# piljoong-jeong/nerf_meets_mlx

Hardware: AMD Instinct MI355X
Metric: train+render rays/sec on Lego 800x800 (synthetic), coarse+fine 64+128 (higher is better)
Workload: dtype split16 (fp16x2 render / bf16x2 train MFMA operands ~ 22 / 16 significand bits; fp32 accumulate)

## Files before the change

### include/nerf_hip.h

```cpp
#ifndef NERF_HIP_H
#define NERF_HIP_H

#include <stddef.h>
#include <stdint.h>

#ifdef __cplusplus
extern "C" {
#endif

#define NERF_ABI_VERSION 3

#define NERF_OK 0
#define NERF_E_NULL (-1)
#define NERF_E_SHAPE (-2)
#define NERF_E_UNSUPPORTED (-3)
#define NERF_E_HIP (-4)
#define NERF_E_RCCL (-5)

int nerf_abi_version(void);
const char* nerf_last_error(void);

#define NERF_RAY_STRIDE 11

int nerf_pixel_permutation(int64_t* out_idx, int64_t n, int64_t domain, uint64_t seed, uint64_t offset,
                           void* stream);

int nerf_ray_gen(const int64_t* pixel_idx, int64_t n, int H, int W, const double* K_host, const float* c2w_host,
                 float near, float far, float* rays, int64_t* coords, void* stream);

int nerf_sample_batch(int64_t n, int H, int W, uint64_t seed, uint64_t offset, const double* K_host, const float* c2w_host,
                      float near, float far, const float* image, float* rays, float* target, int64_t* pixel_idx,
                      void* stream);

int nerf_sample_batch_rgba(int64_t n, int H, int W, uint64_t seed, uint64_t offset, const double* K_host, const float* c2w_host,
                           float near, float far, const float* image, float* rays, float* target, int64_t* pixel_idx,
                           void* stream);

int nerf_gather_rows(const float* src, int64_t n_src, const int64_t* idx, int64_t n, int channels, float* out,
                     void* stream);

int nerf_ndc_rays(float* rays, int64_t n, int H, int W, float focal, float near, void* stream);

int nerf_sample_coarse(const float* rays, int64_t B, int n, int lindisp, float perturb, const float* t_rand,
                       float* z, void* stream);

int nerf_add_noise_z(const float* z_in, const float* t_rand, int64_t B, int n, float strength, float* z_out,
                     void* stream);

int nerf_importance_sample(const float* z, const float* weights, const float* u, int64_t B, int n, int N, float eps,
                           float* z_new, float* z_merged, float* cdf, int64_t* inds, void* stream);

int nerf_encode_freq(const float* x, int64_t M, int D, int n_freqs, int freq_mode, float* out, void* stream);

int nerf_encode_sinusoidal(const float* x, int64_t M, int D, int n_freqs, const float* freqs_host,
                           int include_input, float* out, void* stream);

int nerf_sh_encode(const float* dirs, int64_t M, int degree, float* out, void* stream);

int nerf_hashgrid_forward(const float* x, int64_t M, const float* tables, int L, int log2_T, int F,
                          const int* resolutions_host, float* out, void* stream);
int nerf_hashgrid_backward(const float* x, int64_t M, const float* d_out, int L, int log2_T, int F,
                           const int* resolutions_host, float* d_tables, void* stream);

int nerf_ngp_encode(const float* rays, const float* z, int64_t B, int n, const float* tables, int L, int log2_T,
                    int F, const int* resolutions_host, int sh_degree, float pos_scale, float pos_offset, float* x_out,
                    float* pts_out, void* stream);
int nerf_hashgrid_backward_rays(const float* rays, const float* z, int64_t B, int n, const float* d_out, int L,
                                int log2_T, int F, const int* resolutions_host, float pos_scale, float pos_offset,
                                float* d_tables, void* stream);

int nerf_hashgrid_backward_ex(const float* x, int64_t M, const float* d_out, int L, int log2_T, int F,
                              const int* resolutions_host, int level_lo, int level_hi, int fixed_point, void* d_tables,
                              void* stream);
int nerf_hashgrid_backward_rays_ex(const float* rays, const float* z, int64_t B, int n, const float* d_out, int L,
                                   int log2_T, int F, const int* resolutions_host, float pos_scale, float pos_offset,
                                   int level_lo, int level_hi, int fixed_point, void* d_tables, void* stream);

int nerf_hashgrid_forward_lw(const float* x, int64_t M, const float* tables, int L, int log2_T, int F,
                             const int* resolutions_host, const float* level_weights_host, float* out, void* stream);
int nerf_ngp_encode_lw(const float* rays, const float* z, int64_t B, int n, const float* tables, int L, int log2_T,
                       int F, const int* resolutions_host, const float* level_weights_host, int sh_degree,
                       float pos_scale, float pos_offset, float* x_out, float* pts_out, void* stream);
int nerf_hashgrid_backward_ex_lw(const float* x, int64_t M, const float* d_out, int L, int log2_T, int F,
                                 const int* resolutions_host, const float* level_weights_host, int level_lo,
                                 int level_hi, int fixed_point, void* d_tables, void* stream);
int nerf_hashgrid_backward_rays_ex_lw(const float* rays, const float* z, int64_t B, int n, const float* d_out, int L,
                                      int log2_T, int F, const int* resolutions_host, const float* level_weights_host,
                                      float pos_scale, float pos_offset, int level_lo, int level_hi, int fixed_point,
                                      void* d_tables, void* stream);

int nerf_composite_forward(const float* raw, const float* z, const float* rays, int64_t B, int n,
                           float raw_noise_std, const float* noise, int white_bkgd, float* rgb, float* disp,
                           float* acc, float* weights, float* depth, void* stream);

int nerf_composite_backward(const float* raw, const float* z, const float* rays, int64_t B, int n,
                            float raw_noise_std, const float* noise, int white_bkgd, const float* d_rgb,
                            const float* d_acc, const float* d_depth, float* d_raw, void* stream);

int nerf_mse_loss_grad(const float* pred, const float* target, int64_t count, float grad_scale, float* loss_out,
                       float* d_pred, void* stream);

int nerf_composite_mse_backward(const float* raw, const float* z, const float* rays, int64_t B, int n, int white_bkgd,
                                const float* target, float grad_scale, float* loss_out, float* rgb, float* d_raw,
                                void* stream);

int nerf_ssim_sums(const float* pred, const float* gt, int N, int C, int H, int W, const float* window_host,
                   int w_size, float c1, float c2, double* sums, void* stream);

typedef struct nerf_mlp_arch {
  int n_layers;
  int width;
  int in_pos;
  int in_dir;
  int skip_layer;
  int use_viewdirs;
  int out_ch;
  int precision;
} nerf_mlp_arch;

int64_t nerf_mlp_param_count(const nerf_mlp_arch* arch);
int64_t nerf_mlp_packed_bytes(const nerf_mlp_arch* arch);
int nerf_mlp_pack(const nerf_mlp_arch* arch, const float* params, void* packed, void* stream);

int64_t nerf_mlp_acts_bytes(const nerf_mlp_arch* arch, int64_t M);
int64_t nerf_mlp_dz_bytes(const nerf_mlp_arch* arch, int64_t M);

int nerf_mlp_forward(const nerf_mlp_arch* arch, const void* packed, const float* x, int64_t M, float* out,
                     void* stream);
int nerf_mlp_forward_train(const nerf_mlp_arch* arch, const void* packed, const float* x, int64_t M, float* out,
                           void* acts, void* stream);

int nerf_query_fused(const nerf_mlp_arch* arch, const void* packed, const float* rays, const float* z, int64_t B,
                     int n, int freq_mode, float* raw, void* acts, void* stream);

int nerf_mlp_backward(const nerf_mlp_arch* arch, const void* packed, const void* acts, const float* d_raw,
                      int64_t M, void* dz, float* grads, void* stream);
int nerf_mlp_backward_inputs(const nerf_mlp_arch* arch, const void* packed, const void* acts, const float* d_raw,
                             int64_t M, void* dz, float* grads, float* d_x, void* stream);

int nerf_mlp_debug_width(const nerf_mlp_arch* arch, int kind, int layer);
int nerf_mlp_debug_read(const nerf_mlp_arch* arch, const void* store, int kind, int layer, int64_t M, float* out,
                        void* stream);

int nerf_ngp_query_fused(const nerf_mlp_arch* arch, const void* packed, const float* rays, const float* z, int64_t B,
                         int n, const float* tables, int L, int log2_T, int F, const int* resolutions_host,
                         int sh_degree, float pos_scale, float pos_offset, float* raw, void* acts, void* stream);
int nerf_ngp_query_fused_h(const nerf_mlp_arch* arch, const void* packed, const float* rays, const float* z, int64_t B,
                           int n, const float* tables, const void* tables_half, int L, int log2_T, int F,
                           const int* resolutions_host, int sh_degree, float pos_scale, float pos_offset, float* raw,
                           void* acts, void* stream);
int nerf_ngp_query_fused_lw(const nerf_mlp_arch* arch, const void* packed, const float* rays, const float* z, int64_t B,
                            int n, const float* tables, const void* tables_half, int L, int log2_T, int F,
                            const int* resolutions_host, const float* level_weights_host, int sh_degree, float pos_scale,
                            float pos_offset, float* raw, void* acts, void* stream);


int nerf_occ_points(int log2_res, int64_t cell0, int64_t count, uint64_t seed, uint64_t update, float pos_scale,
                    float pos_offset, float* rays_out, float* z_out, void* stream);
int nerf_occ_merge(float* density, const float* raw, int64_t count, float decay, void* stream);
int64_t nerf_occ_finalize_workspace_bytes(int log2_res);
int nerf_occ_finalize(const float* density, int log2_res, float thr_cap, void* workspace, float* thr_out, uint32_t* bits,
                      void* stream);
int64_t nerf_occ_cull_workspace_bytes(int64_t B, int n);
int nerf_occ_cull(const float* rays, const float* z, int64_t B, int n, const uint32_t* bits, int log2_res, float pos_scale,
                  float pos_offset, void* workspace, int64_t* idx_out, int64_t* count_out, float* rays_out, float* z_out,
                  float* raw_fill, void* stream);
int nerf_scatter_rows(const float* src, const int64_t* idx, int64_t n, int channels, float* dst, int64_t n_dst, void* stream);

#define NERF_MARCH_MAX_STEPS 1024
int64_t nerf_occ_march_workspace_bytes(int64_t B);
int nerf_occ_march_count(const float* rays, int64_t B, const float* jitter, float jitter_const, const uint32_t* bits, int log2_res,
                         float pos_scale, float pos_offset, float step_world, int march_steps, void* workspace, int64_t* offsets,
                         void* stream);
int nerf_occ_march_write(const float* rays, int64_t B, const float* jitter, float jitter_const, const uint32_t* bits, int log2_res,
                         float pos_scale, float pos_offset, float step_world, int march_steps, void* workspace, int64_t* offsets,
                         float* rows_out, float* z_out, void* stream);
#define NERF_OCC_RELU 0
#define NERF_OCC_EXP 1
int nerf_occ_merge_ex(float* density, const float* raw, int64_t count, float decay, int activation, void* stream);

int nerf_composite_packed_forward(const float* raw, const float* z, const int64_t* offsets, int64_t B, int64_t K, float step_world,
                                  int white_bkgd, float* rgb, float* acc, float* depth, void* stream);
int nerf_composite_packed_mse_backward(const float* raw, const int64_t* offsets, int64_t B, int64_t K, float step_world,
                                       int white_bkgd, const float* target, float grad_scale, float* loss_out, float* rgb,
                                       float* d_raw, void* stream);

int nerf_composite_packed_distortion(const float* raw, const float* z, const int64_t* offsets, const float* rays, int64_t B,
                                     int64_t K, float step_world, int march_steps, int white_bkgd, float* rgb, float* acc,
                                     float* depth, float* dist, void* stream);
int nerf_composite_packed_mse_dist_backward(const float* raw, const float* z, const int64_t* offsets, const float* rays, int64_t B,
                                            int64_t K, float step_world, int march_steps, int white_bkgd, const float* target,
                                            float grad_scale, float dist_weight, float* loss_out, float* dist_out, float* rgb,
                                            float* d_raw, void* stream);

int nerf_composite_packed_forward_bg(const float* raw, const float* z, const int64_t* offsets, int64_t B, int64_t K, float step_world,
                                     const float* bg, int bg_stride, float* rgb, float* acc, float* depth, void* stream);
int nerf_composite_packed_distortion_bg(const float* raw, const float* z, const int64_t* offsets, const float* rays, int64_t B,
                                        int64_t K, float step_world, int march_steps, const float* bg, int bg_stride, float* rgb,
                                        float* acc, float* depth, float* dist, void* stream);
int nerf_composite_packed_mse_backward_bg(const float* raw, const int64_t* offsets, int64_t B, int64_t K, float step_world,
                                          const float* target_rgba, const float* bg, float grad_scale, float* loss_out, float* rgb,
                                          float* d_raw, void* stream);
int nerf_composite_packed_mse_dist_backward_bg(const float* raw, const float* z, const int64_t* offsets, const float* rays, int64_t B,
                                               int64_t K, float step_world, int march_steps, const float* target_rgba,
                                               const float* bg, float grad_scale, float dist_weight, float* loss_out,
                                               float* dist_out, float* rgb, float* d_raw, void* stream);

#define NERF_ERT_TERMINATED 1
int64_t nerf_ert_march_workspace_bytes(int64_t B);
int nerf_ert_init(int64_t B, int32_t* istate, float* fstate, int32_t* live, void* stream);
int nerf_ert_march_count(const float* rays, int64_t B, const float* jitter, float jitter_const, const uint32_t* bits, int log2_res,
                         float pos_scale, float pos_offset, float step_world, int march_steps, const int32_t* live, int64_t A,
                         const int32_t* istate, int max_new, void* workspace, int64_t* totals, void* stream);
int nerf_ert_march_write(const float* rays, int64_t B, const float* jitter, float jitter_const, const uint32_t* bits, int log2_res,
                         float pos_scale, float pos_offset, float step_world, int march_steps, const int32_t* live, int64_t A,
                         int32_t* istate, int max_new, void* workspace, int64_t* offsets, int32_t* live_out, float* rows_out,
                         float* z_out, void* stream);
int nerf_ert_fold(const float* raw, const float* z, const int64_t* offsets, const int32_t* live, int64_t A, int64_t B, int64_t K,
                  float step_world, float min_transmittance, int32_t* istate, float* fstate, void* stream);
int nerf_ert_finish(const int32_t* istate, const float* fstate, int64_t B, int white_bkgd, float* rgb, float* acc, float* depth,
                    int32_t* samples, void* stream);
int nerf_ert_finish_bg(const int32_t* istate, const float* fstate, int64_t B, const float* bg, int bg_stride, float* rgb, float* acc,
                       float* depth, int32_t* samples, void* stream);

#define NERF_MESH_MAX_RES 512
int64_t nerf_mesh_workspace_bytes(int res);
int nerf_mesh_points(int res, const float* lo_host, const float* hi_host, int64_t p0, int64_t count, float* rays_out, float* z_out,
                     void* stream);
int nerf_mesh_count(const float* vol, int res, float iso, void* workspace, int64_t* totals, void* stream);
int nerf_mesh_write_vertices(const float* vol, int res, float iso, const float* lo_host, const float* hi_host, void* workspace,
                             int64_t V, float* verts, float* normals, float* color_rows, void* stream);
int nerf_mesh_write_faces(const float* vol, int res, float iso, void* workspace, int64_t F, int32_t* faces, void* stream);

int64_t nerf_ccl_workspace_bytes(int res);
int nerf_ccl_label(const float* vol, int res, float iso, void* workspace, int32_t* labels, void* stream);
int nerf_ccl_sizes(const int32_t* labels, int res, int32_t* sizes, int64_t* stats, void* stream);
int nerf_ccl_filter(const float* vol, const int32_t* labels, const int32_t* sizes, const int64_t* stats, int res, float iso,
                    int64_t min_voxels, int largest_only, float* out, void* stream);

#define NERF_MORPH_MAX_RADIUS 16
int64_t nerf_morph_workspace_bytes(int res);
int nerf_morph_erode(const float* vol, int res, float iso, int radius, void* workspace, float* core, int64_t* stats2, void* stream);
int nerf_morph_reconstruct(const float* vol, const float* kept, int res, float iso, int radius, void* workspace, float* out,
                           int64_t* stats2, void* stream);

#define NERF_TSDF_MAX_VIEWS 16
typedef struct nerf_tsdf_view {
  float c2w[12];
  float fx, fy, cx, cy;
} nerf_tsdf_view;
int nerf_tsdf_reset(float* D, float* Wt, uint8_t* flags, int res, void* stream);
int nerf_tsdf_integrate(float* D, float* Wt, uint8_t* flags, int res, const float* lo_host, const float* hi_host,
                        const nerf_tsdf_view* views_host, int n, int H, int W, const float* depth, const float* acc, float trunc,
                        float acc_min, float far, int carve, void* stream);
int nerf_tsdf_volume(const float* D, const float* Wt, const uint8_t* flags, int res, int min_views, float* vol_out, void* stream);

int64_t nerf_render_workspace_bytes(int64_t B, int n, int N);
int nerf_render_rays_fused(const nerf_mlp_arch* arch, const void* packed_coarse, const void* packed_fine,
                           const float* rays, int64_t B, int n, int N, const float* u, int freq_mode, int white_bkgd,
                           void* workspace, float* rgb, float* disp, float* acc, float* rgb_coarse, float* disp_coarse,
                           float* acc_coarse, float* z_vals, float* weights, void* stream);

#define NERF_COMM_ID_BYTES 128
int nerf_comm_unique_id(char* id_out_host);
int nerf_comm_init(void** comm_out, int nranks, int rank, const char* id_host);
int nerf_allreduce_grads(void* comm, float* grads, int64_t count, void* stream);
int nerf_comm_destroy(void* comm);

#define NERF_OPTION_UNKNOWN (-2147483647 - 1)
int nerf_set_option(const char* key, int value);
int nerf_get_option(const char* key);

int nerf_adam_step(float* params, const float* grads, float* m, float* v, int64_t count, float lr, float beta1,
                   float beta2, float eps, int bias_correction, int step, float grad_scale, void* stream);
int nerf_adam_step_ex(float* params, void* grads, float* m, float* v, int64_t count, float lr, float beta1, float beta2,
                      float eps, int bias_correction, int step, float grad_scale, int grads_fixed_point, int zero_grads,
                      void* stream);
int nerf_adam_step_shadow(float* params, void* grads, float* m, float* v, int64_t count, float lr, float beta1, float beta2,
                          float eps, int bias_correction, int step, float grad_scale, int grads_fixed_point, int zero_grads,
                          void* params_half, void* stream);

#ifdef __cplusplus
}
#endif
#endif
```

### nerf_meets_mlx_amd/_native.py

```python
import ctypes as C
import os

import torch

_HERE = os.path.dirname(os.path.abspath(__file__))
LIB_PATH = os.environ.get("NERF_HIP_LIB", os.path.join(_HERE, "libnerf_hip.so"))

_P, _I64, _I, _F, _U64 = C.c_void_p, C.c_int64, C.c_int, C.c_float, C.c_uint64
SIGNATURES = {
    "nerf_abi_version": (_I, []),
    "nerf_last_error": (C.c_char_p, []),
    "nerf_pixel_permutation": (_I, [_P, _I64, _I64, _U64, _U64, _P]),
    "nerf_ray_gen": (_I, [_P, _I64, _I, _I, C.POINTER(C.c_double), C.POINTER(C.c_float), _F, _F, _P, _P, _P]),
    "nerf_sample_batch": (_I, [_I64, _I, _I, _U64, _U64, C.POINTER(C.c_double), C.POINTER(C.c_float), _F, _F, _P, _P, _P, _P, _P]),
    "nerf_sample_batch_rgba": (_I, [_I64, _I, _I, _U64, _U64, C.POINTER(C.c_double), C.POINTER(C.c_float), _F, _F, _P, _P, _P, _P, _P]),
    "nerf_gather_rows": (_I, [_P, _I64, _P, _I64, _I, _P, _P]),
    "nerf_ndc_rays": (_I, [_P, _I64, _I, _I, _F, _F, _P]),
    "nerf_sample_coarse": (_I, [_P, _I64, _I, _I, _F, _P, _P, _P]),
    "nerf_add_noise_z": (_I, [_P, _P, _I64, _I, _F, _P, _P]),
    "nerf_importance_sample": (_I, [_P, _P, _P, _I64, _I, _I, _F, _P, _P, _P, _P, _P]),
    "nerf_encode_freq": (_I, [_P, _I64, _I, _I, _I, _P, _P]),
    "nerf_encode_sinusoidal": (_I, [_P, _I64, _I, _I, C.POINTER(C.c_float), _I, _P, _P]),
    "nerf_sh_encode": (_I, [_P, _I64, _I, _P, _P]),
    "nerf_hashgrid_forward": (_I, [_P, _I64, _P, _I, _I, _I, C.POINTER(C.c_int), _P, _P]),
    "nerf_hashgrid_backward": (_I, [_P, _I64, _P, _I, _I, _I, C.POINTER(C.c_int), _P, _P]),
    "nerf_ngp_encode": (_I, [_P, _P, _I64, _I, _P, _I, _I, _I, C.POINTER(C.c_int), _I, C.c_float, C.c_float, _P, _P, _P]),
    "nerf_ngp_query_fused": (_I, [_P, _P, _P, _P, _I64, _I, _P, _I, _I, _I, C.POINTER(C.c_int), _I, C.c_float, C.c_float, _P, _P, _P]),
    "nerf_ngp_query_fused_h": (_I, [_P, _P, _P, _P, _I64, _I, _P, _P, _I, _I, _I, C.POINTER(C.c_int), _I, C.c_float, C.c_float, _P, _P, _P]),
    "nerf_hashgrid_backward_rays": (_I, [_P, _P, _I64, _I, _P, _I, _I, _I, C.POINTER(C.c_int), C.c_float, C.c_float, _P, _P]),
    "nerf_hashgrid_backward_ex": (_I, [_P, _I64, _P, _I, _I, _I, C.POINTER(C.c_int), _I, _I, _I, _P, _P]),
    "nerf_hashgrid_backward_rays_ex": (_I, [_P, _P, _I64, _I, _P, _I, _I, _I, C.POINTER(C.c_int), C.c_float, C.c_float, _I, _I, _I, _P, _P]),
    "nerf_hashgrid_forward_lw": (_I, [_P, _I64, _P, _I, _I, _I, C.POINTER(C.c_int), C.POINTER(C.c_float), _P, _P]),
    "nerf_ngp_encode_lw": (_I, [_P, _P, _I64, _I, _P, _I, _I, _I, C.POINTER(C.c_int), C.POINTER(C.c_float), _I, C.c_float, C.c_float, _P, _P, _P]),
    "nerf_ngp_query_fused_lw": (_I, [_P, _P, _P, _P, _I64, _I, _P, _P, _I, _I, _I, C.POINTER(C.c_int), C.POINTER(C.c_float), _I, C.c_float, C.c_float, _P, _P, _P]),
    "nerf_hashgrid_backward_ex_lw": (_I, [_P, _I64, _P, _I, _I, _I, C.POINTER(C.c_int), C.POINTER(C.c_float), _I, _I, _I, _P, _P]),
    "nerf_hashgrid_backward_rays_ex_lw": (_I, [_P, _P, _I64, _I, _P, _I, _I, _I, C.POINTER(C.c_int), C.POINTER(C.c_float), C.c_float, C.c_float, _I, _I, _I, _P, _P]),
    "nerf_composite_forward": (_I, [_P, _P, _P, _I64, _I, _F, _P, _I, _P, _P, _P, _P, _P, _P]),
    "nerf_composite_backward": (_I, [_P, _P, _P, _I64, _I, _F, _P, _I, _P, _P, _P, _P, _P]),
    "nerf_mse_loss_grad": (_I, [_P, _P, _I64, _F, _P, _P, _P]),
    "nerf_composite_mse_backward": (_I, [_P, _P, _P, _I64, _I, _I, _P, _F, _P, _P, _P, _P]),
    "nerf_ssim_sums": (_I, [_P, _P, _I, _I, _I, _I, C.POINTER(C.c_float), _I, _F, _F, _P, _P]),
    "nerf_mlp_param_count": (_I64, [_P]),
    "nerf_mlp_packed_bytes": (_I64, [_P]),
    "nerf_mlp_pack": (_I, [_P, _P, _P, _P]),
    "nerf_mlp_acts_bytes": (_I64, [_P, _I64]),
    "nerf_mlp_dz_bytes": (_I64, [_P, _I64]),
    "nerf_mlp_forward": (_I, [_P, _P, _P, _I64, _P, _P]),
    "nerf_mlp_forward_train": (_I, [_P, _P, _P, _I64, _P, _P, _P]),
    "nerf_query_fused": (_I, [_P, _P, _P, _P, _I64, _I, _I, _P, _P, _P]),
    "nerf_mlp_backward": (_I, [_P, _P, _P, _P, _I64, _P, _P, _P]),
    "nerf_mlp_backward_inputs": (_I, [_P, _P, _P, _P, _I64, _P, _P, _P, _P]),
    "nerf_mlp_debug_width": (_I, [_P, _I, _I]),
    "nerf_mlp_debug_read": (_I, [_P, _P, _I, _I, _I64, _P, _P]),
    "nerf_render_workspace_bytes": (_I64, [_I64, _I, _I]),
    "nerf_render_rays_fused": (_I, [_P, _P, _P, _P, _I64, _I, _I, _P, _I, _I, _P, _P, _P, _P, _P, _P, _P, _P, _P, _P]),
    "nerf_comm_unique_id": (_I, [C.c_char_p]),
    "nerf_comm_init": (_I, [C.POINTER(C.c_void_p), _I, _I, C.c_char_p]),
    "nerf_allreduce_grads": (_I, [_P, _P, _I64, _P]),
    "nerf_comm_destroy": (_I, [_P]),
    "nerf_set_option": (_I, [C.c_char_p, _I]),
    "nerf_get_option": (_I, [C.c_char_p]),
    "nerf_adam_step": (_I, [_P, _P, _P, _P, _I64, _F, _F, _F, _F, _I, _I, _F, _P]),
    "nerf_adam_step_ex": (_I, [_P, _P, _P, _P, _I64, _F, _F, _F, _F, _I, _I, _F, _I, _I, _P]),
    "nerf_adam_step_shadow": (_I, [_P, _P, _P, _P, _I64, _F, _F, _F, _F, _I, _I, _F, _I, _I, _P, _P]),
    "nerf_occ_points": (_I, [_I, _I64, _I64, _U64, _U64, _F, _F, _P, _P, _P]),
    "nerf_occ_merge": (_I, [_P, _P, _I64, _F, _P]),
    "nerf_occ_finalize_workspace_bytes": (_I64, [_I]),
    "nerf_occ_finalize": (_I, [_P, _I, _F, _P, _P, _P, _P]),
    "nerf_occ_cull_workspace_bytes": (_I64, [_I64, _I]),
    "nerf_occ_cull": (_I, [_P, _P, _I64, _I, _P, _I, _F, _F, _P, _P, _P, _P, _P, _P, _P]),
    "nerf_scatter_rows": (_I, [_P, _P, _I64, _I, _P, _I64, _P]),
    "nerf_occ_merge_ex": (_I, [_P, _P, _I64, _F, _I, _P]),
    "nerf_occ_march_workspace_bytes": (_I64, [_I64]),
    "nerf_occ_march_count": (_I, [_P, _I64, _P, _F, _P, _I, _F, _F, _F, _I, _P, _P, _P]),
    "nerf_occ_march_write": (_I, [_P, _I64, _P, _F, _P, _I, _F, _F, _F, _I, _P, _P, _P, _P, _P]),
    "nerf_composite_packed_forward": (_I, [_P, _P, _P, _I64, _I64, _F, _I, _P, _P, _P, _P]),
    "nerf_composite_packed_mse_backward": (_I, [_P, _P, _I64, _I64, _F, _I, _P, _F, _P, _P, _P, _P]),
    "nerf_composite_packed_distortion": (_I, [_P, _P, _P, _P, _I64, _I64, _F, _I, _I, _P, _P, _P, _P, _P]),
    "nerf_composite_packed_mse_dist_backward": (_I, [_P, _P, _P, _P, _I64, _I64, _F, _I, _I, _P, _F, _F, _P, _P, _P, _P, _P]),
    "nerf_composite_packed_forward_bg": (_I, [_P, _P, _P, _I64, _I64, _F, _P, _I, _P, _P, _P, _P]),
    "nerf_composite_packed_distortion_bg": (_I, [_P, _P, _P, _P, _I64, _I64, _F, _I, _P, _I, _P, _P, _P, _P, _P]),
    "nerf_composite_packed_mse_backward_bg": (_I, [_P, _P, _I64, _I64, _F, _P, _P, _F, _P, _P, _P, _P]),
    "nerf_composite_packed_mse_dist_backward_bg": (_I, [_P, _P, _P, _P, _I64, _I64, _F, _I, _P, _P, _F, _F, _P, _P, _P, _P, _P]),
    "nerf_ert_march_workspace_bytes": (_I64, [_I64]),
    "nerf_ert_init": (_I, [_I64, _P, _P, _P, _P]),
    "nerf_ert_march_count": (_I, [_P, _I64, _P, _F, _P, _I, _F, _F, _F, _I, _P, _I64, _P, _I, _P, _P, _P]),
    "nerf_ert_march_write": (_I, [_P, _I64, _P, _F, _P, _I, _F, _F, _F, _I, _P, _I64, _P, _I, _P, _P, _P, _P, _P, _P]),
    "nerf_ert_fold": (_I, [_P, _P, _P, _P, _I64, _I64, _I64, _F, _F, _P, _P, _P]),
    "nerf_ert_finish": (_I, [_P, _P, _I64, _I, _P, _P, _P, _P, _P]),
    "nerf_ert_finish_bg": (_I, [_P, _P, _I64, _P, _I, _P, _P, _P, _P, _P]),
    "nerf_mesh_workspace_bytes": (_I64, [_I]),
    "nerf_mesh_points": (_I, [_I, C.POINTER(C.c_float), C.POINTER(C.c_float), _I64, _I64, _P, _P, _P]),
    "nerf_mesh_count": (_I, [_P, _I, _F, _P, _P, _P]),
    "nerf_mesh_write_vertices": (_I, [_P, _I, _F, C.POINTER(C.c_float), C.POINTER(C.c_float), _P, _I64, _P, _P, _P, _P]),
    "nerf_mesh_write_faces": (_I, [_P, _I, _F, _P, _I64, _P, _P]),
    "nerf_ccl_workspace_bytes": (_I64, [_I]),
    "nerf_ccl_label": (_I, [_P, _I, _F, _P, _P, _P]),
    "nerf_ccl_sizes": (_I, [_P, _I, _P, _P, _P]),
    "nerf_ccl_filter": (_I, [_P, _P, _P, _P, _I, _F, _I64, _I, _P, _P]),
    "nerf_morph_workspace_bytes": (_I64, [_I]),
    "nerf_morph_erode": (_I, [_P, _I, _F, _I, _P, _P, _P, _P]),
    "nerf_morph_reconstruct": (_I, [_P, _P, _I, _F, _I, _P, _P, _P, _P]),
    "nerf_tsdf_reset": (_I, [_P, _P, _P, _I, _P]),
    "nerf_tsdf_integrate": (_I, [_P, _P, _P, _I, C.POINTER(C.c_float), C.POINTER(C.c_float), C.POINTER(C.c_float), _I, _I, _I, _P, _P,
                                _F, _F, _F, _I, _P]),
    "nerf_tsdf_volume": (_I, [_P, _P, _P, _I, _I, _P, _P]),
}


class MlpArch(C.Structure):
    _fields_ = [("n_layers", _I), ("width", _I), ("in_pos", _I), ("in_dir", _I), ("skip_layer", _I),
                ("use_viewdirs", _I), ("out_ch", _I), ("precision", _I)]


class NerfHipError(RuntimeError):
    pass


_lib = None


def lib():
    global _lib
    if _lib is None:
        if not os.path.exists(LIB_PATH):
            raise NerfHipError(
                f"{LIB_PATH} not found: build it with `python -c 'import __graft_entry__ as g; g.build()'` "
                "(hipcc --offload-arch=gfx950).  There is no CPU fallback.")
        L = C.CDLL(LIB_PATH)
        for name, (res, args) in SIGNATURES.items():
            fn = getattr(L, name)
            fn.restype, fn.argtypes = res, args
        _lib = L
    return _lib


def check(rc: int):
    if rc != 0:
        msg = lib().nerf_last_error().decode(errors="replace")
        if rc in (-1, -2, -3):
            raise ValueError(f"libnerf_hip error {rc}: {msg}")
        raise NerfHipError(f"libnerf_hip error {rc}: {msg}")


def ptr(t):
    if t is None:
        return None
    if not t.is_cuda:
        raise ValueError("libnerf_hip kernels need tensors on the ROCm device (there is no CPU path)")
    if not t.is_contiguous():
        raise ValueError("libnerf_hip kernels need contiguous tensors")
    return C.c_void_p(t.data_ptr())


def stream():
    return C.c_void_p(torch.cuda.current_stream().cuda_stream)


def f32(t, device=None):
    if not torch.is_tensor(t):
        t = torch.as_tensor(t)
    if device is not None:
        t = t.to(device)
    return t.to(torch.float32).contiguous()
```

### nerf_meets_mlx_amd/csrc/dw_split.h

```cpp
#pragma once
#include <stdint.h>

namespace nerf {

constexpr int DW_SPLIT_MAX_JOBS = 16;
struct DwCost { int nf, kf; };

inline int dw_split(const DwCost* jobs, int nj, int bias, int target_wgs, int64_t max_splits, int* splits) {
  int64_t units[DW_SPLIT_MAX_JOBS], total_units = 0;
  for (int j = 0; j < nj; ++j) {
    units[j] = jobs[j].nf + jobs[j].kf + bias;
    total_units += units[j];
  }
  int nw = 0;
  double frac[DW_SPLIT_MAX_JOBS];
  for (int j = 0; j < DW_SPLIT_MAX_JOBS; ++j) splits[j] = 0;
  for (int j = 0; j < nj; ++j) {
    const double share = (double)units[j] * target_wgs / (double)total_units;
    int64_t sp = (int64_t)share;
    frac[j] = share - (double)sp;
    if (sp < 1) { sp = 1; frac[j] = 0.0; }
    if (sp > max_splits) { sp = max_splits; frac[j] = 0.0; }
    splits[j] = (int)sp;
    nw += (int)sp;
  }
  while (nw < target_wgs) {
    int best = -1;
    for (int j = 0; j < nj; ++j)
      if (splits[j] < max_splits && (best < 0 || frac[j] > frac[best])) best = j;
    if (best < 0 || frac[best] <= 0.0) break;
    splits[best] += 1; frac[best] = 0.0; nw += 1;
  }
  while (nw > target_wgs) {
    int big = 0;
    for (int j = 1; j < nj; ++j) if (splits[j] > splits[big]) big = j;
    if (splits[big] <= 1) break;
    splits[big] -= 1; nw -= 1;
  }
  return nw;
}

}
```

### nerf_meets_mlx_amd/csrc/mlp.hip

```cpp
#include "common.h"
#include "mlp_ring.h"
#include "mlp_layout.h"
#include "mlp_frag.h"
#include "mlp_arch2.h"
#include "hash_common.h"
#include "mlp_params.h"
#include "mlp_model.h"
#include "dw_split.h"
#include <limits.h>
#include <string.h>


namespace nerf {

extern int g_hash_combine_max_res;




constexpr int PACK_THREADS = (L::F_TOTAL + L::B_PADDED) * 64 + L::BI_TOTAL;
__device__ __forceinline__ void pack_part(int tid, const float* __restrict__ p, bf16x8* __restrict__ wf,
                                          bf16x8* __restrict__ wb, float* __restrict__ bias) {
  const int nf = L::F_TOTAL * 64, nb = L::B_PADDED * 64;
  if (tid < nf + nb) {
// ... 781 lines not shown
  const int wv = __builtin_amdgcn_readfirstlane(threadIdx.x >> 6);
  const int64_t ntiles = (a.M + 31) >> 5;
  const int64_t nsuper = (ntiles + NW - 1) / NW;
  RingW<(L::B_TOTAL + CHUNK - 1) / CHUNK, L::B_TOTAL, 4, NW, CHUNK> ws;
  ws.wsrc = reinterpret_cast<const char*>(a.wb);
  ws.lane16 = 16 * lane;
  ws.lds0 = __builtin_amdgcn_readfirstlane(lds_addr_of(ring_smem));
  ws.wv = wv;
  ws.start(lane);
  PassQueue pq;
  pq.init(a.queue, ws.lds0 + decltype(ws)::BIAS_OFF);
  for (int64_t sp = blockIdx.x; sp < nsuper;) {
    int ln = lane;
    asm volatile("" : "+v"(ln));
    ws.new_pass();
    bwd_tiles<1>(a, ws, sp * NW + wv, ntiles, ln, &pq);
    sp = pq.next(sp);
  }
  ws.drain();
  pq.leave();
}


constexpr int DW_FRAG_STRIDE = 1152;
constexpr int DW_STAGE_BYTES = 32 * DW_FRAG_STRIDE;
constexpr int DW_STAGES = 4;
constexpr int DW_LDS_BYTES = DW_STAGES * DW_STAGE_BYTES + 1024;

__device__ __forceinline__ bf16x8 tr_frag(const char* lds_frag, int u, int hq, int i16) {
  const int q = i16 >> 2, p = i16 & 3;
  const char* base = lds_frag + 16 * (p & 1) + 8 * (p >> 1) + 32 * (16 * u + 8 * hq + q);
  const s16x4 lo = __builtin_amdgcn_ds_read_tr16_b64_v4i16((__attribute__((address_space(3))) s16x4*)(base));
  const s16x4 hi = __builtin_amdgcn_ds_read_tr16_b64_v4i16((__attribute__((address_space(3))) s16x4*)(base + 128));
  union { struct { s16x4 a, b; } s; bf16x8 v; } cvt;
  cvt.s.a = lo; cvt.s.b = hi;
  return cvt.v;
}

#ifndef NERF_DW_WAVES
#define NERF_DW_WAVES 16
#endif
constexpr int DW_WAVES = NERF_DW_WAVES;
constexpr int DW_NPW = 32 / DW_WAVES;
__global__ void __launch_bounds__(64 * DW_WAVES) mlp_dw_kernel(DwArgs a) {
  char* smem = ring_smem;
  int bj = blockIdx.x, job_id = 0;
  while (bj >= a.splits[job_id]) { bj -= a.splits[job_id]; ++job_id; }
  const DwJob jb = a.jobs[job_id];
  const int tile_lo = (int)((int64_t)a.ntiles * bj / a.splits[job_id]);
  const int tile_hi = (int)((int64_t)a.ntiles * (bj + 1) / a.splits[job_id]);
  const int tid = threadIdx.x, lane = tid & 63;
  const int wv = __builtin_amdgcn_readfirstlane(tid >> 6);
  const int n_tiles = (jb.nf + 1) >> 1, k_tiles = (jb.kf + 1) >> 1;
  const bool col_major = DW_WAVES == 16 && k_tiles <= 2;
  const int wr = col_major ? (wv & 3) : (wv >> 2), wc = col_major ? (wv >> 2) : (wv & 3);
  const int nf_pad = n_tiles * 2;
  const int nfk = jb.nf + jb.kf;
  const bool active = (wr * DW_NPW < n_tiles) && (wc * 2 < k_tiles);
  f32x16 acc[DW_NPW][2];
#pragma unroll
  for (int i = 0; i < DW_NPW; ++i)
#pragma unroll
    for (int k = 0; k < 2; ++k)
#pragma unroll
      for (int e = 0; e < 16; ++e) acc[i][k][e] = 0.0f;
  float bsum[DW_NPW];
#pragma unroll
  for (int i = 0; i < DW_NPW; ++i) bsum[i] = 0.0f;
  const int g16 = lane >> 4, i16 = lane & 15, hq = g16 >> 1, fsel = g16 & 1;
  const bf16x8* dzp = reinterpret_cast<const bf16x8*>(a.dz) + lane;
  const bf16x8* acp = reinterpret_cast<const bf16x8*>(a.acts) + lane;
  const unsigned lds0 = __builtin_amdgcn_readfirstlane(lds_addr_of(smem));
  const unsigned sink = lds0 + DW_STAGES * DW_STAGE_BYTES;

  if (jb.nf & 1) {
    for (int c = tid; c < DW_STAGES * 64; c += 64 * DW_WAVES) {
      bf16x8 zv;
#pragma unroll
      for (int j = 0; j < 8; ++j) zv[j] = (__bf16)0.0f;
      *reinterpret_cast<bf16x8*>(smem + (c >> 6) * DW_STAGE_BYTES + jb.nf * DW_FRAG_STRIDE + (c & 63) * 16) = zv;
    }
  }
  auto issue = [&](int tile, int stage) {
    const unsigned st = lds0 + __builtin_amdgcn_readfirstlane(stage) * DW_STAGE_BYTES;
#pragma unroll
    for (int k = 0; k < DW_NPW; ++k) {
      const int i = wv + DW_WAVES * k;
      if (i < jb.nf) dma_frag_nt(dzp + (int64_t)tile * a.zstride + (jb.dz_slot + i) * 64, st + i * DW_FRAG_STRIDE);
      else if (i < nfk) dma_frag_nt(acp + (int64_t)tile * a.astride + (jb.act_slot + (i - jb.nf)) * 64,
                                 st + (nf_pad + i - jb.nf) * DW_FRAG_STRIDE);
      else dma_frag(dzp + (int64_t)tile * a.zstride + jb.dz_slot * 64, sink);
    }
  };
  __syncthreads();
#pragma unroll
  for (int s_ = 0; s_ < DW_STAGES - 1; ++s_)
    if (tile_lo + s_ < tile_hi) issue(tile_lo + s_, s_);

  for (int tile = tile_lo; tile < tile_hi; ++tile) {
    const int rem = tile_hi - 1 - tile;
    if (DW_NPW == 4) {
      if (rem >= 2) asm volatile("s_waitcnt vmcnt(8) lgkmcnt(0)" ::: "memory");
      else if (rem == 1) asm volatile("s_waitcnt vmcnt(4) lgkmcnt(0)" ::: "memory");
      else asm volatile("s_waitcnt vmcnt(0) lgkmcnt(0)" ::: "memory");
    } else {
      if (rem >= 2) asm volatile("s_waitcnt vmcnt(4) lgkmcnt(0)" ::: "memory");
      else if (rem == 1) asm volatile("s_waitcnt vmcnt(2) lgkmcnt(0)" ::: "memory");
      else asm volatile("s_waitcnt vmcnt(0) lgkmcnt(0)" ::: "memory");
    }
    __builtin_amdgcn_s_barrier();
    if (tile + DW_STAGES - 1 < tile_hi) issue(tile + DW_STAGES - 1, (tile - tile_lo + DW_STAGES - 1) % DW_STAGES);
    const char* st = smem + ((tile - tile_lo) % DW_STAGES) * DW_STAGE_BYTES;
#if NERF_ABLATE == 4
    if (false) {
#else
    if (active) {
#endif
#pragma unroll
      for (int u = 0; u < 2; ++u) {
        bf16x8 bfr[2];
#pragma unroll
        for (int k = 0; k < 2; ++k) {
          const int kt = wc * 2 + k;
          const int f = nf_pad + (kt < k_tiles ? 2 * kt : 0) + fsel;
          bfr[k] = tr_frag(st + f * DW_FRAG_STRIDE, u, hq, i16);
        }
#pragma unroll
        for (int i = 0; i < DW_NPW; ++i) {
          const int nt = wr * DW_NPW + i;
          const int f = (nt < n_tiles ? 2 * nt : 0) + fsel;
          const bf16x8 afr = tr_frag(st + f * DW_FRAG_STRIDE, u, hq, i16);
#if NERF_ABLATE != 5
          if (wc == 0) {
            typedef __bf16 bf16x2_t __attribute__((ext_vector_type(2)));
            const bf16x2_t ones = {(__bf16)1.0f, (__bf16)1.0f};
#pragma unroll
            for (int j = 0; j < 8; j += 2) {
              const bf16x2_t pr = {afr[j], afr[j + 1]};
              bsum[i] = __builtin_amdgcn_fdot2_f32_bf16(pr, ones, bsum[i], false);
            }
          }
#endif
#pragma unroll
          for (int k = 0; k < 2; ++k) acc[i][k] = __builtin_amdgcn_mfma_f32_32x32x16_bf16(afr, bfr[k], acc[i][k], 0, 0, 0);
        }
      }
    }
  }
  if (!active) return;
#if NERF_ABLATE == 6
  if (a.ntiles > 0) return;
#endif
  const int rr = lane & 31, hh = lane >> 5;
  float* slot = a.partial + (size_t)blockIdx.x * DW_SLOT_FLOATS;
#pragma unroll
  for (int i = 0; i < DW_NPW; ++i) {
    const int nt = wr * DW_NPW + i;
    if (nt >= n_tiles) continue;
#pragma unroll
    for (int k = 0; k < 2; ++k) {
      const int kt = wc * 2 + k;
      if (kt >= k_tiles) continue;
      float* tile = slot + (8 * nt + kt) * 1024;
#pragma unroll
      for (int e = 0; e < 16; ++e) tile[((e & 3) + 8 * (e >> 2) + 4 * hh) * 32 + rr] = acc[i][k][e];
    }
    if (wc == 0 && jb.b_off >= 0) {
      const float tot = bsum[i] + __shfl_xor(bsum[i], 32, 64);
      if (hh == 0) slot[64 * 1024 + 32 * nt + rr] = tot;
    }
  }
}

__global__ void __launch_bounds__(256) mlp_dw_reduce_kernel(DwArgs a) {
  const int j = blockIdx.y;
  const DwJob jb = a.jobs[j];
  int first = 0;
  for (int q = 0; q < j; ++q) first += a.splits[q];
  const int S = a.splits[j];
  const int nw = jb.n_valid * jb.k_valid, nb = jb.b_off >= 0 ? jb.n_valid : 0;
  const float* base = a.partial + (size_t)first * DW_SLOT_FLOATS;
  for (int t = blockIdx.x * 256 + threadIdx.x; t < nw + nb; t += gridDim.x * 256) {
    const float* src;
    float* dst;
    if (t < nw) {
      const int n = t / jb.k_valid, k = t - n * jb.k_valid;
      src = base + (8 * (n >> 5) + (k >> 5)) * 1024 + (n & 31) * 32 + (k & 31);
      dst = a.grads + jb.w_off + (int64_t)n * jb.ldw + jb.col0 + k;
    } else {
      src = base + 64 * 1024 + (t - nw);
      dst = a.grads + jb.b_off + (t - nw);
    }
    float sum = 0.0f;
    int sidx = 0;
    for (; sidx + 8 <= S; sidx += 8) {
      float v[8];
#pragma unroll
      for (int q = 0; q < 8; ++q) v[q] = __builtin_nontemporal_load(src + (size_t)(sidx + q) * DW_SLOT_FLOATS);
#pragma unroll
      for (int q = 0; q < 8; ++q) sum += v[q];
    }
    for (; sidx < S; ++sidx) sum += __builtin_nontemporal_load(src + (size_t)sidx * DW_SLOT_FLOATS);
    *dst = sum;
  }
}



__global__ void __launch_bounds__(256) pack_img_kernel(const float* __restrict__ p, bf16x8* __restrict__ wf,
                                                       bf16x8* __restrict__ wb, float* __restrict__ bias, int out_ch) {
  const int tid = blockIdx.x * 256 + threadIdx.x;
  const int nf = LI::F_TOTAL * 64, nb = LI::B_PADDED * 64;
  if (tid < nf + nb) {
    const bool fw = tid < nf;
    const int t = fw ? tid : tid - nf;
    const int f = t >> 6, lane = t & 63, r = lane & 31, h = lane >> 5;
    bf16x8 v;
#pragma unroll
    for (int j = 0; j < 8; ++j)
      v[j] = (__bf16)(fw ? fwd_src_img(p, f, r, h, j, out_ch) : (f < LI::B_TOTAL ? bwd_src_img(p, f, r, h, j, out_ch) : 0.0f));
    (fw ? wf : wb)[t] = v;
  } else if (tid < nf + nb + LI::BI_TOTAL) {
    const int s = tid - nf - nb;
    bias[s] = s < 2048 ? p[LI::pb(s >> 8) + (s & 255)] : ((s - LI::BI_OUT) < out_ch ? p[LI::P_WO + out_ch * 256 + (s - LI::BI_OUT)] : 0.0f);
  }
}

struct ImgArgs {
  const bf16x8* wf; const bf16x8* wb; const float* bias;
  const float* x;
  const float* d_out;
  int64_t M; int out_ch;
  float* out;
  void* acts; void* dz;
  int64_t astride, zstride;
};

template <bool STORE, class WS>
__device__ __forceinline__ void fwd_tiles_img(const ImgArgs& a, WS& ws, int64_t tile0, int64_t ntiles, int lane) {
  constexpr int ST = 1;
  const int r = lane & 31, h = lane >> 5;
  int64_t tile = tile0 < ntiles ? tile0 : ntiles - 1;
  int64_t m = tile * 32 + r; if (m >= a.M) m = a.M - 1;
  bf16x8 xin[ST][3];
#pragma unroll
  for (int ks = 0; ks < 3; ++ks) xin[0][ks] = row_frag(a.x + m * LI::CIN, ks, h, LI::CIN);
  int bad = nonfinite_flags<32>(nonfinite_bits(xin[0][0]) | nonfinite_bits(xin[0][1]) | nonfinite_bits(xin[0][2]), 0u);
  asm volatile("" : "+v"(bad));
  if (STORE) { store_frags<3>(a.acts, tile0, a.astride, LI::A_X, xin[0], r, h); ws.note_stores(3); }
  bf16x8 ha[ST][16], hb[ST][16];
  u32x4 mk[ST];
#define IMG_LAYER(KS, FB, BS, IN, OUT, LYR)                                                        \
  do { mk[0] = u32x4{0u, 0u, 0u, 0u};                                                              \
       layer_fwd<ST, KS, 8, true, STORE>(ws, FB, BS, IN, OUT, mk, lane);                           \
       if (STORE) { store_frags<16>(a.acts, tile0, a.astride, LI::A_H0 + 16 * (LYR), OUT[0], r, h); \
                    *reinterpret_cast<u32x4*>(frag_ptr(a.acts, tile0, a.astride, LI::A_MASK + (LYR), r, h)) = mk[0]; ws.note_stores(17); } } while (0)
  IMG_LAYER(3, LI::F_L0, 0, xin, ha, 0);
  IMG_LAYER(16, LI::F_L1 + 0 * 128, 256, ha, hb, 1);
  IMG_LAYER(16, LI::F_L1 + 1 * 128, 512, hb, ha, 2);
  IMG_LAYER(16, LI::F_L1 + 2 * 128, 768, ha, hb, 3);
  IMG_LAYER(16, LI::F_L1 + 3 * 128, 1024, hb, ha, 4);
  {
    bf16x8 cat[ST][19];
    if (STORE) {
#pragma unroll
      for (int k = 0; k < 3; ++k) xin[0][k] = *frag_ptr(a.acts, tile0, a.astride, LI::A_X + k, r, h);
    }
#pragma unroll
    for (int k = 0; k < 3; ++k) cat[0][k] = xin[0][k];
#pragma unroll
    for (int k = 0; k < 16; ++k) cat[0][3 + k] = ha[0][k];
    IMG_LAYER(19, LI::F_L5, 1280, cat, hb, 5);
  }
  IMG_LAYER(16, LI::F_L6, 1536, hb, ha, 6);
  IMG_LAYER(16, LI::F_L7, 1792, ha, hb, 7);
#undef IMG_LAYER
  f32x16 acc;
  acc_init_bias(acc, ws, LI::BI_OUT, h);
#pragma unroll
  for (int ks = 0; ks < 16; ++ks) {
    const bf16x8 wo = next_frag(ws, LI::F_OUT + ks, lane);
    acc = __builtin_amdgcn_mfma_f32_32x32x16_bf16(wo, hb[0][ks], acc, 0, 0, 0);
  }
  const int64_t mo = tile0 * 32 + r;
  if (h == 0 && tile0 < ntiles && mo < a.M) {
#pragma unroll
    for (int c = 0; c < 4; ++c)
      if (c < a.out_ch) a.out[mo * a.out_ch + c] = bad ? __builtin_nanf("") : acc[c];
  }
}

template <bool STORE>
__global__ void __launch_bounds__(512, 2) mlp_img_fwd_ring_kernel(ImgArgs a) {
  const int lane = threadIdx.x & 63;
  const int wv = __builtin_amdgcn_readfirstlane(threadIdx.x >> 6);
  const int64_t ntiles = (a.M + 31) >> 5, nsuper = (ntiles + 7) >> 3;
  RingW<LI::F_CHUNKS, LI::F_TOTAL, (STORE ? 2 : 4)> ws;
  ws.wsrc = reinterpret_cast<const char*>(a.wf);
  ws.lane16 = 16 * lane;
  ws.lds0 = __builtin_amdgcn_readfirstlane(lds_addr_of(ring_smem));
  ws.wv = wv;
  ws.start(lane);
  ring_load_bias(a.bias, LI::BI_TOTAL);
  __syncthreads();
  for (int64_t sp = blockIdx.x; sp < nsuper; sp += gridDim.x) {
    int ln = lane;
    asm volatile("" : "+v"(ln));
    ws.new_pass();
    fwd_tiles_img<STORE>(a, ws, sp * 8 + wv, ntiles, ln);
  }
  ws.drain();
}

__global__ void __launch_bounds__(512, 2) mlp_img_bwd_ring_kernel(ImgArgs a) {
  constexpr int ST = 1;
  const int lane0 = threadIdx.x & 63;
  const int wv = __builtin_amdgcn_readfirstlane(threadIdx.x >> 6);
  const int64_t ntiles = (a.M + 31) >> 5, nsuper = (ntiles + 7) >> 3;
  RingW<LI::B_CHUNKS, LI::B_TOTAL> ws;
  ws.wsrc = reinterpret_cast<const char*>(a.wb);
  ws.lane16 = 16 * lane0;
  ws.lds0 = __builtin_amdgcn_readfirstlane(lds_addr_of(ring_smem));
  ws.wv = wv;
  ws.start(lane0);
  for (int64_t sp = blockIdx.x; sp < nsuper; sp += gridDim.x) {
    int lane = lane0;
    asm volatile("" : "+v"(lane));
    ws.new_pass();
    const int r = lane & 31, h = lane >> 5;
    const int64_t tile0 = sp * 8 + wv;
    const int64_t tile = tile0 < ntiles ? tile0 : ntiles - 1;
    const int64_t m = tile * 32 + r;
    bf16x8 zo[ST][1];
#pragma unroll
    for (int j = 0; j < 8; ++j) zo[0][0][j] = (__bf16)0.0f;
    if (tile0 < ntiles && m < a.M && h == 0) {
#pragma unroll
      for (int c = 0; c < 4; ++c)
        if (c < a.out_ch) zo[0][0][c] = (__bf16)a.d_out[m * a.out_ch + c];
    }
    u32x4 mk[8][ST];
#pragma unroll
    for (int l = 0; l < 8; ++l)
      mk[l][0] = *reinterpret_cast<const u32x4*>(frag_ptr(a.acts, tile, a.astride, LI::A_MASK + l, r, h));
    store_frags<1>(a.dz, tile0, a.zstride, LI::Z_OUT, zo[0], r, h); ws.note_stores(1);
    bf16x8 za[ST][16], zb[ST][16];
    layer_bwd<ST, 1, 8, true>(ws, LI::B_OUT, zo, zb, mk[7], lane);
    store_frags<16>(a.dz, tile0, a.zstride, LI::Z_L0 + 112, zb[0], r, h); ws.note_stores(16);
    layer_bwd<ST, 16, 8, true>(ws, LI::B_L7 + 0 * 128, zb, za, mk[6], lane);
    store_frags<16>(a.dz, tile0, a.zstride, LI::Z_L0 + 96, za[0], r, h); ws.note_stores(16);
    layer_bwd<ST, 16, 8, true>(ws, LI::B_L7 + 1 * 128, za, zb, mk[5], lane);
    store_frags<16>(a.dz, tile0, a.zstride, LI::Z_L0 + 80, zb[0], r, h); ws.note_stores(16);
    layer_bwd<ST, 16, 8, true>(ws, LI::B_L7 + 2 * 128, zb, za, mk[4], lane);
    store_frags<16>(a.dz, tile0, a.zstride, LI::Z_L0 + 64, za[0], r, h); ws.note_stores(16);
    layer_bwd<ST, 16, 8, true>(ws, LI::B_L7 + 3 * 128, za, zb, mk[3], lane);
// ... 76 lines not shown
        const int l = 8 * ks + 4 * q + 2 * h + e;
        const Corners c = corners_of(px, py, pz, a.rt.res[l], mask);
        if (LW) {
          const float w = h ? a.lw.w[8 * ks + 4 * q + 2 + e] : a.lw.w[8 * ks + 4 * q + e];
          const FeatVec<2> fv = hash_level_lw<HALF>(a.tables + (size_t)l * a.T * 2, a.tables_h + (size_t)l * a.T, c, w);
          xin[0][ks][4 * q + 2 * e] = (__bf16)fv.v[0];
          xin[0][ks][4 * q + 2 * e + 1] = (__bf16)fv.v[1];
        } else {
          const FeatVec<2> fv = HALF ? hash_level_h(a.tables_h + (size_t)l * a.T, c) : hash_level<2>(a.tables + (size_t)l * a.T * 2, c);
          xin[0][ks][4 * q + 2 * e] = (__bf16)fv.v[0];
          xin[0][ks][4 * q + 2 * e + 1] = (__bf16)fv.v[1];
        }
      }
  float sh[16];
  sh_eval(rr[8], rr[9], rr[10], 3, sh);
#pragma unroll
  for (int j = 0; j < 8; ++j) din[0][0][j] = (__bf16)(h == 0 ? sh[8 * (j >> 2) + (j & 3)] : sh[8 * (j >> 2) + 4 + (j & 3)]);
}

template <bool STORE, bool FUSED, bool LW = false>
__global__ void __launch_bounds__(512) mlp_small_fwd_kernel(SmallArgs a) {
  constexpr int ST = 1;
  lds_load_stream(a.wf, a.bias);
  const int lane0 = threadIdx.x & 63, wv = threadIdx.x >> 6;
  const bool rmaj = FUSED && !STORE && a.ray_major;
  const int64_t ntiles = rmaj ? ((a.B + 31) >> 5) * a.n : (a.M + 31) >> 5;
  LdsW ws;
  for (int64_t tile0 = (int64_t)blockIdx.x * 8 + wv; tile0 < ntiles; tile0 += (int64_t)gridDim.x * 8) {
    int lane = lane0;
    asm volatile("" : "+v"(lane));
    const int r = lane & 31, h = lane >> 5;
    int64_t m = tile0 * 32 + r;
    bool valid = m < a.M;
    if (rmaj) {
      const int64_t rb = tile0 / a.n;
      const int depth = (int)(tile0 - rb * a.n);
      int64_t ray = rb * 32 + r;
      valid = ray < a.B;
      if (!valid) ray = a.B - 1;
      m = ray * a.n + depth;
    }
    if (m >= a.M) m = a.M - 1;
    bf16x8 xin[ST][2], din[ST][1];
    if (FUSED) {
      if (a.tables_h) ngp_row_frags<true, LW>(a, m, h, xin, din);
      else ngp_row_frags<false, LW>(a, m, h, xin, din);
    } else {
      const float* row = a.x + m * LN::CIN;
      xin[0][0] = row_frag(row, 0, h, LN::CPOS); xin[0][1] = row_frag(row, 1, h, LN::CPOS);
      din[0][0] = row_frag(row + LN::CPOS, 0, h, LN::CDIR);
    }
    int bad = nonfinite_flags<32>(nonfinite_bits(xin[0][0]) | nonfinite_bits(xin[0][1]), nonfinite_bits(din[0][0]));
    asm volatile("" : "+v"(bad));
#define SINK(slot0) FragSink<STORE>{a.acts, tile0, a.astride, slot0, r, h}
#define MASK_STORE(layer) do { if (STORE) *reinterpret_cast<u32x4*>(frag_ptr(a.acts, tile0, a.astride, LN::A_MASK + (layer), r, h)) = mk[0]; } while (0)
    if (STORE) { store_frags<2>(a.acts, tile0, a.astride, LN::A_X, xin[0], r, h); store_frags<1>(a.acts, tile0, a.astride, LN::A_DX, din[0], r, h); }
    u32x4 mk[ST];
    bf16x8 h0[ST][4], h1[ST][4], ft[ST][4];
    mk[0] = u32x4{0u, 0u, 0u, 0u};
    layer_fwd<ST, 2, 2, true, STORE>(ws, LN::F_L0, LN::BI_L0, xin, h0, mk, lane, SINK(LN::A_H0));
    MASK_STORE(0);
    mk[0] = u32x4{0u, 0u, 0u, 0u};
    layer_fwd<ST, 4, 2, true, STORE>(ws, LN::F_L1, LN::BI_L1, h0, h1, mk, lane, SINK(LN::A_H1));
    MASK_STORE(1);
    layer_fwd<ST, 4, 2, false, false>(ws, LN::F_FA, LN::BI_FEAT, h1, ft, mk, lane, SINK(LN::A_FEAT));
    float alpha;
    {
      f32x16 acc;
      acc_init_bias(acc, ws, LN::BI_ALPHA, h);
#pragma unroll
      for (int ks = 0; ks < 4; ++ks) acc = __builtin_amdgcn_mfma_f32_32x32x16_bf16(ws.frag(LN::F_FA + 8 + ks, lane), h1[0][ks], acc, 0, 0, 0);
      alpha = acc[0];
    }
    bf16x8 hd[ST][2];
    {
      bf16x8 cat[ST][5];
#pragma unroll
      for (int k = 0; k < 4; ++k) cat[0][k] = ft[0][k];
      cat[0][4] = din[0][0];
      mk[0] = u32x4{0u, 0u, 0u, 0u};
      layer_fwd<ST, 5, 1, true, STORE>(ws, LN::F_DIR, LN::BI_DIR, cat, hd, mk, lane, SINK(LN::A_HD));
      MASK_STORE(2);
    }
    {
      f32x16 acc;
      acc_init_bias(acc, ws, LN::BI_RGB, h);
#pragma unroll
      for (int ks = 0; ks < 2; ++ks) acc = __builtin_amdgcn_mfma_f32_32x32x16_bf16(ws.frag(LN::F_RGB + ks, lane), hd[0][ks], acc, 0, 0, 0);
      if (h == 0 && valid) {
        float4 o; o.x = acc[0]; o.y = acc[1]; o.z = acc[2]; o.w = alpha;
        *reinterpret_cast<float4*>(a.out + m * 4) = poison_raw(o, bad);
      }
    }
#undef SINK
#undef MASK_STORE
  }
}

__global__ void __launch_bounds__(512) mlp_small_bwd_kernel(SmallArgs a) {
  constexpr int ST = 1;
  lds_load_stream(a.wb, nullptr);
  const int lane0 = threadIdx.x & 63, wv = threadIdx.x >> 6;
  const int64_t ntiles = (a.M + 31) >> 5;
  LdsW ws;
  for (int64_t tile0 = (int64_t)blockIdx.x * 8 + wv; tile0 < ntiles; tile0 += (int64_t)gridDim.x * 8) {
    int lane = lane0;
    asm volatile("" : "+v"(lane));
    const int r = lane & 31, h = lane >> 5;
    const int64_t m = tile0 * 32 + r;
    float4 g = make_float4(0.f, 0.f, 0.f, 0.f);
    if (m < a.M && h == 0) g = *reinterpret_cast<const float4*>(a.d_raw + m * 4);
    bf16x8 zrgb[ST][1], zal[ST][1];
#pragma unroll
    for (int j = 0; j < 8; ++j) { zrgb[0][0][j] = (__bf16)0.0f; zal[0][0][j] = (__bf16)0.0f; }
    zrgb[0][0][0] = (__bf16)g.x; zrgb[0][0][1] = (__bf16)g.y; zrgb[0][0][2] = (__bf16)g.z;
    zal[0][0][0] = (__bf16)g.w;
    u32x4 mk[3][ST];
#pragma unroll
    for (int l = 0; l < 3; ++l)
      mk[l][0] = *reinterpret_cast<const u32x4*>(frag_ptr(const_cast<void*>(a.acts), tile0, a.astride, LN::A_MASK + l, r, h));
    store_frags<1>(a.dz, tile0, a.zstride, LN::Z_RGB, zrgb[0], r, h);
    store_frags<1>(a.dz, tile0, a.zstride, LN::Z_A, zal[0], r, h);
#define ZSINK(slot0) FragSink<true>{a.dz, tile0, a.zstride, slot0, r, h}
    bf16x8 zd[ST][2], zf[ST][4], z1[ST][4], z0[ST][4];
    layer_bwd<ST, 1, 1, true>(ws, LN::B_RGB, zrgb, zd, mk[2], lane, ZSINK(LN::Z_D));
    layer_bwd<ST, 2, 2, false>(ws, LN::B_DIR, zd, zf, mk[2], lane, ZSINK(LN::Z_F));
    {
      bf16x8 cat[ST][5];
#pragma unroll
      for (int k = 0; k < 4; ++k) cat[0][k] = zf[0][k];
      cat[0][4] = zal[0][0];
      layer_bwd<ST, 5, 2, true>(ws, LN::B_FA, cat, z1, mk[1], lane, ZSINK(LN::Z_L1));
    }
    layer_bwd<ST, 4, 2, true>(ws, LN::B_L1, z1, z0, mk[0], lane, ZSINK(LN::Z_L0));
#undef ZSINK
    if (a.d_x) {
      f32x16 acc;
#pragma unroll
      for (int i = 0; i < 16; ++i) acc[i] = 0.0f;
#pragma unroll
      for (int ns = 0; ns < 4; ++ns) acc = __builtin_amdgcn_mfma_f32_32x32x16_bf16(ws.frag(LN::B_L0 + ns, lane), z0[0][ns], acc, 0, 0, 0);
      if (m < a.M) {
#pragma unroll
        for (int q = 0; q < 4; ++q) {
          float4 o; o.x = acc[4 * q]; o.y = acc[4 * q + 1]; o.z = acc[4 * q + 2]; o.w = acc[4 * q + 3];
          *reinterpret_cast<float4*>(a.d_x + m * LN::CPOS + 8 * q + 4 * h) = o;
        }
      }
    }
  }
}

static int g_dw_wgs = 0;
static int g_dw_bias = -1;
static int g_bwd_stage = 0;
static int g_dw_ring_cap = 8;
static int g_dw_private = 4;
static int g_dw16_variant = 1;
static int g_dw_narrow_first = 1;
static int g_dw_job_mask = 0;
static int g_mlp_variant = 0;
static int g_ring_wgs = 0;
static int g_ngp_ray_major = 1;
int g_pass_queue = 1;
static int g_ring_split = 1;

static int cu_count() {
  constexpr int MAX_DEVICES = 64;
  static int n[MAX_DEVICES] = {};
  int dev = 0;
  if (hipGetDevice(&dev) != hipSuccess || dev < 0 || dev >= MAX_DEVICES) dev = 0;
  if (n[dev] == 0) {
    int v = 0;
    n[dev] = (hipDeviceGetAttribute(&v, hipDeviceAttributeMultiprocessorCount, dev) == hipSuccess && v > 0) ? v : 256;
  }
  return n[dev];
}
static inline int ring_wgs() { return g_ring_wgs > 0 ? g_ring_wgs : cu_count(); }
static inline unsigned ring_grid(int64_t ntiles) { return persistent_grid((ntiles + 7) / 8, ring_wgs()); }

struct Option { const char* key; int* var; bool (*rule)(int& v); const char* refusal; };
static bool opt_any(int&) { return true; }
static bool opt_flag(int& v) { v = v ? 1 : 0; return true; }
template <int LO, int HI> static bool opt_clamp(int& v) { v = v < LO ? LO : v > HI ? HI : v; return true; }
static const Option OPTIONS[] = {
    {"mlp_variant", &g_mlp_variant, opt_any, nullptr},
    {"ring_split", &g_ring_split, [](int& v) { return v == 1 || v == 2; }, "nerf_set_option: ring_split must be 1 or 2"},
    {"ring_workgroups", &g_ring_wgs, opt_clamp<0, INT_MAX>, nullptr},
    {"tile_pad16", &g_tile_pad16, opt_clamp<0, INT_MAX>, nullptr},
    {"dw_workgroups", &g_dw_wgs, opt_clamp<0, INT_MAX>, nullptr},
    {"dw_unit_bias", &g_dw_bias, opt_clamp<-1, INT_MAX>, nullptr},
    {"bwd_stage", &g_bwd_stage, opt_any, nullptr},
    {"dw_job_mask", &g_dw_job_mask, opt_any, nullptr},
    {"hash_combine_max_res", &g_hash_combine_max_res, opt_clamp<0, INT_MAX>, nullptr},
    {"ngp_ray_major", &g_ngp_ray_major, opt_flag, nullptr},
    {"dw22_variant", &s16::g_dw_variant, opt_flag, nullptr},
    {"dw16_variant", &g_dw16_variant, opt_clamp<0, 3>, nullptr},
    {"dw_private_tiles", &g_dw_private, opt_clamp<0, 4>, nullptr},
    {"dw_ring_cap", &g_dw_ring_cap, opt_clamp<2, 16>, nullptr},
    {"pass_queue", &g_pass_queue, opt_flag, nullptr},
    {"dw_narrow_first", &g_dw_narrow_first, opt_flag, nullptr},
    {"f22_tiles", &f22::g_tiles, [](int& v) { return v == 0 || v == 2 || v == 3; }, "nerf_set_option: f22_tiles must be 0 (automatic), 2 or 3"},
};

}

using namespace nerf;

extern "C" int nerf_set_option(const char* key, int value) {
  NERF_REQUIRE(key, NERF_E_NULL, "nerf_set_option: key is NULL");
  NERF_REQUIRE(strcmp(key, "mlp_precision") != 0, NERF_E_UNSUPPORTED,
               "nerf_set_option: \"mlp_precision\" is gone (ABI 3): set nerf_mlp_arch.precision of the model instead");
  for (const Option& o : OPTIONS) {
    if (strcmp(key, o.key)) continue;
    if (!o.rule(value)) return fail(NERF_E_UNSUPPORTED, "%s", o.refusal);
    *o.var = value;
    return NERF_OK;
  }
  return fail(NERF_E_UNSUPPORTED, "nerf_set_option: unknown key '%s'", key);
}

extern "C" int nerf_get_option(const char* key) {
  if (!key) return NERF_OPTION_UNKNOWN;
  for (const Option& o : OPTIONS)
    if (!strcmp(key, o.key)) return *o.var;
  return NERF_OPTION_UNKNOWN;
}

extern "C" int64_t nerf_mlp_param_count(const nerf_mlp_arch* arch) { return resolve(arch).params; }
extern "C" int64_t nerf_mlp_packed_bytes(const nerf_mlp_arch* arch) { return resolve(arch).packed_bytes; }
extern "C" int64_t nerf_mlp_acts_bytes(const nerf_mlp_arch* arch, int64_t M) { return resolve(arch).acts_bytes(M); }
extern "C" int64_t nerf_mlp_dz_bytes(const nerf_mlp_arch* arch, int64_t M) { return resolve(arch).dz_bytes(M); }

#define NERF_ARCH_MSG ": HIP kernels exist for (8x256, skip 4) with in=63+27 view head, or in=40 / no view head / out_ch<=4, and for (2x64, no skip) with in=32+16 view head"
#define NERF_RESOLVE(who)        \
  const Model m = resolve(arch); \
  NERF_REQUIRE(m.ok, NERF_E_UNSUPPORTED, who NERF_ARCH_MSG)

extern "C" int nerf_mlp_pack(const nerf_mlp_arch* arch, const float* params, void* packed, void* stream) {
  NERF_RESOLVE("nerf_mlp_pack");
  NERF_REQUIRE(params && packed, NERF_E_NULL, "nerf_mlp_pack: params/packed is NULL");
  auto s = as_stream(stream);
  bf16x8* wf = m.stream<bf16x8>(packed, S_FWD);
  bf16x8* wb = m.stream<bf16x8>(packed, S_BWD);
  float* bias = m.stream<float>(packed, S_BIAS);
  int rc;
  if (m.shape == Shape::Small) {
    const int tot = (LN::F_PADDED + LN::B_PADDED) * 64 + LN::BI_TOTAL;
    rc = launch<pack_small_kernel>("nerf_mlp_pack (2x64 model)", dim3((tot + 255) / 256), dim3(256), 0, s, params, wf, wb, bias);
    if (!rc && m.split()) rc = s16x::small_pack(params, m.stream<void>(packed, S_S16), s);
  } else if (m.shape == Shape::Image) {
    const int tot = (LI::F_TOTAL + LI::B_PADDED) * 64 + LI::BI_TOTAL;
    rc = launch<pack_img_kernel>("nerf_mlp_pack (image model)", dim3((tot + 255) / 256), dim3(256), 0, s, params, wf, wb, bias, m.out_ch);
    if (!rc && m.split()) rc = s16x::img_pack(params, m.out_ch, m.stream<void>(packed, S_S16), s);
    if (!rc && m.prec == Prec::F32) rc = f32::pack(params, m.stream<void>(packed, S_F32), m.out_ch, s);
  } else {
    rc = launch<pack_kernel>("nerf_mlp_pack", dim3(PACK_BLOCKS + PACK16_BLOCKS), dim3(256), 0, s, params, wf, wb, bias,
                             m.stream<bf16x8>(packed, S_FWD16));
    if (!rc && m.prec == Prec::F32) rc = f32::pack(params, m.stream<void>(packed, S_F32), 0, s);
    if (!rc && m.split()) rc = f22::pack(params, m.stream<void>(packed, S_F22), s);
    if (!rc && m.split()) rc = s16::pack(params, m.stream<void>(packed, S_S16), s);
  }
  return rc;
}

template <int MODE>
static int launch_fwd(const Model& m, const void* packed, const float* x, const float* rays, const float* z, int64_t M, int n,
                      int freq_mode, float* out, void* acts, void* stream) {
  FwdArgs a;
  a.queue = nullptr;
  a.wf = m.stream<bf16x8>(packed, S_FWD);
  a.bias = m.stream<float>(packed, S_BIAS);
  a.x = x; a.rays = rays; a.z = z; a.M = M; a.n = n; a.out = out; a.acts = acts; a.astride = m.astride();
  fill_freqs(a.fr.pos, a.fr.dir, freq_mode);
  const int64_t ntiles = (M + 31) / 32;
  auto s = as_stream(stream);
  const int variant = (g_mlp_variant == 0) ? (MODE == 1 ? (acts ? 3 : 4) : 1) : g_mlp_variant;
  if ((variant == 4 || variant == 5) && MODE == 1 && !acts) {
    const dim3 g(persistent_grid((M + 255) / 256, ring_wgs()));
    FwdArgs a16 = a;
    a16.queue = passq_slot();
    a16.wf = m.stream<bf16x8>(packed, S_FWD16);
    const char* what = "mlp forward (ring, 16x16x32)";
    if (variant == 4) return launch<mlp_fwd_ring16_kernel<8, 2>, mlp_fwd_ring16_kernel<4, 4>>(what, g, dim3(512), RING16_LDS_BYTES, s, a16);
    return launch<mlp_fwd_ring16_kernel<4, 4>, mlp_fwd_ring16_kernel<8, 2>>(what, g, dim3(256), RING16_LDS_BYTES, s, a16);
  }
  if (variant >= 3 && MODE == 1) {
    a.queue = passq_slot();
    if (acts && g_ring_split == 2) {
      return launch<mlp_fwd_ring_kernel<1, true, SPLIT_NW, SPLIT_CHUNK>>(
          "mlp forward (ring, 2 workgroups per CU)", dim3(persistent_grid((ntiles + SPLIT_NW - 1) / SPLIT_NW, 2 * (int64_t)ring_wgs())),
          dim3(64 * SPLIT_NW), SPLIT_LDS_BYTES, s, a);
    }
    return with_bool(acts != nullptr, [&](auto store) {
      constexpr bool ST = decltype(store)::value;
      return launch<mlp_fwd_ring_kernel<1, ST>, mlp_fwd_ring_kernel<1, !ST>>("mlp forward (ring)", dim3(ring_grid(ntiles)), dim3(512),
                                                                              RING_LDS_BYTES, s, a);
    });
  }
  const int st = variant == 2 ? 2 : 1;
  const int64_t blocks = (ntiles + 4 * st - 1) / (4 * st);
  NERF_REQUIRE(blocks < (1ll << 31), NERF_E_SHAPE, "mlp forward: M too large");
  return with_bool(st == 1, [&](auto one) { return with_bool(acts != nullptr, [&](auto store) {
    return launch<mlp_fwd_kernel<decltype(one)::value ? 1 : 2, MODE, decltype(store)::value>>("mlp forward", dim3((unsigned)blocks), dim3(256),
                                                                                                0, s, a);
  }); });
}

static void img_args(ImgArgs& a, const Model& m, const void* packed) {
  a.wf = m.stream<bf16x8>(packed, S_FWD);
  a.wb = m.stream<bf16x8>(packed, S_BWD);
  a.bias = m.stream<float>(packed, S_BIAS);
  a.out_ch = m.out_ch; a.astride = m.astride(); a.zstride = m.zstride();
  a.x = nullptr; a.d_out = nullptr; a.out = nullptr; a.acts = nullptr; a.dz = nullptr; a.M = 0;
}

static void small_args(SmallArgs& a, const Model& m, const void* packed) {
  a.wf = m.stream<bf16x8>(packed, S_FWD);
  a.wb = m.stream<bf16x8>(packed, S_BWD);
  a.bias = m.stream<float>(packed, S_BIAS);
  a.x = nullptr; a.d_raw = nullptr; a.out = nullptr; a.d_x = nullptr; a.acts = nullptr; a.dz = nullptr; a.M = 0;
  a.astride = m.astride(); a.zstride = m.zstride();
  a.rays = nullptr; a.z = nullptr; a.n = 1; a.tables = nullptr; a.tables_h = nullptr; a.T = 0; a.pos_scale = 1.0f; a.pos_offset = 0.0f;
  a.ray_major = 0; a.B = 0;
  for (int l = 0; l < 32; ++l) a.lw.w[l] = 1.0f;
}

static int view_forward(const Model& m, const void* packed, const float* x, const float* rays, const float* z, int64_t M, int n,
                        int freq_mode, float* out, void* acts, void* stream);

extern "C" int nerf_mlp_forward_train(const nerf_mlp_arch* arch, const void* packed, const float* x, int64_t M,
                                      float* out, void* acts, void* stream) {
  NERF_RESOLVE("nerf_mlp_forward");
  if (M <= 0) return NERF_OK;
  NERF_REQUIRE(packed && x && out, NERF_E_NULL, "nerf_mlp_forward: NULL pointer");
  auto s = as_stream(stream);
  if (m.shape == Shape::Small) {
    if (m.split())
      return s16x::small_forward(m.stream<void>(packed, S_S16), m.stream<float>(packed, S_BIAS), x, M, out, acts, m.astride(),
                                 nullptr, s);
    SmallArgs a;
    small_args(a, m, packed);
    a.x = x; a.out = out; a.acts = acts; a.M = M;
    return with_bool(acts != nullptr, [&](auto store) {
      return launch<mlp_small_fwd_kernel<decltype(store)::value, false>>("mlp forward (2x64 model)", dim3(small_grid((M + 31) / 32)), dim3(512),
                                                                         LN::LDS_BYTES, s, a);
    });
  }
  if (m.shape == Shape::Image) {
    if (m.prec == Prec::F32)
      return f32::forward(m.stream<void>(packed, S_F32), x, nullptr, nullptr, M, 1, 0, out, acts, m.out_ch, s);
    if (m.split())
      return s16x::img_forward(m.stream<void>(packed, S_S16), m.stream<float>(packed, S_BIAS), x, M, m.out_ch, out, acts,
                               m.astride(), ring_wgs(), s);
    ImgArgs a;
    img_args(a, m, packed);
    a.x = x; a.out = out; a.acts = acts; a.M = M;
    return with_bool(acts != nullptr, [&](auto store) {
      constexpr bool ST = decltype(store)::value;
      return launch<mlp_img_fwd_ring_kernel<ST>, mlp_img_fwd_ring_kernel<!ST>>("mlp forward (image model)", dim3(ring_grid((M + 31) / 32)),
                                                                               dim3(512), RING_LDS_BYTES, s, a);
    });
  }
  return view_forward(m, packed, x, nullptr, nullptr, M, 1, 0, out, acts, stream);
}

static int view_forward(const Model& m, const void* packed, const float* x, const float* rays, const float* z, int64_t M, int n,
                        int freq_mode, float* out, void* acts, void* stream) {
  auto s = as_stream(stream);
  if (m.split() && !acts)
    return f22::forward(m.stream<void>(packed, S_F22), x, rays, z, M, n, freq_mode, out, ring_wgs(), s);
  if (m.split())
    return s16::forward(m.stream<void>(packed, S_S16), m.stream<float>(packed, S_BIAS), x, rays, z, M, n, freq_mode, out, acts,
                        m.astride(), ring_wgs(), s);
  if (m.prec == Prec::F32) return f32::forward(m.stream<void>(packed, S_F32), x, rays, z, M, n, freq_mode, out, acts, 0, s);
  return x ? launch_fwd<0>(m, packed, x, rays, z, M, n, freq_mode, out, acts, stream)
           : launch_fwd<1>(m, packed, x, rays, z, M, n, freq_mode, out, acts, stream);
}

extern "C" int nerf_mlp_forward(const nerf_mlp_arch* arch, const void* packed, const float* x, int64_t M, float* out,
                                void* stream) {
  return nerf_mlp_forward_train(arch, packed, x, M, out, nullptr, stream);
}

extern "C" int nerf_query_fused(const nerf_mlp_arch* arch, const void* packed, const float* rays, const float* z,
                                int64_t B, int n, int freq_mode, float* raw, void* acts, void* stream) {
  const Model m = resolve(arch);
  NERF_REQUIRE(m.ok && m.shape == Shape::View, NERF_E_UNSUPPORTED, "nerf_query_fused" NERF_ARCH_MSG);
  NERF_REQUIRE(n >= 1, NERF_E_SHAPE, "nerf_query_fused: n must be >= 1");
  if (B <= 0) return NERF_OK;
  NERF_REQUIRE(packed && rays && z && raw, NERF_E_NULL, "nerf_query_fused: NULL pointer");
  NERF_REQUIRE(freq_mode == 0 || freq_mode == 1, NERF_E_UNSUPPORTED, "nerf_query_fused: freq_mode must be 0 or 1");
  NERF_REQUIRE(B * (int64_t)n < (1ll << 31), NERF_E_SHAPE, "nerf_query_fused: B*n must be < 2^31 samples per call");
  return view_forward(m, packed, nullptr, rays, z, B * n, n, freq_mode, raw, acts, stream);
}

static int launch_dw_part(const Model& m, DwArgs& d, int nj, int64_t ntiles, const void* acts, void* dz, float* grads,
                          hipStream_t s, int kind, int slot_base, int max_wgs) {
  static_assert(DW_SPLIT_MAX_JOBS == DW_MAX_JOBS, "dw_split.h sizes its arrays for DwArgs::jobs");
  DwCost cost[DW_MAX_JOBS];
  for (int j = 0; j < nj; ++j) cost[j] = DwCost{d.jobs[j].nf, d.jobs[j].kf};
  int target_wgs = g_dw_wgs > 0 ? g_dw_wgs : cu_count();
  if (target_wgs > max_wgs) target_wgs = max_wgs;
  const int nw = dw_split(cost, nj, g_dw_bias >= 0 ? g_dw_bias : m.split() ? 2 : 128, target_wgs, (ntiles + 3) / 4, d.splits);
  NERF_REQUIRE(slot_base + nw <= DW_MAX_WGS, NERF_E_SHAPE, "nerf_mlp_backward: dw_workgroups must be <= %d", DW_MAX_WGS);
  bool all_tiny = true;
  for (int j = 0; j < nj; ++j) all_tiny = all_tiny && ((d.jobs[j].nf + 1) / 2) * ((d.jobs[j].kf + 1) / 2) <= 4;
  d.ntiles = (int)ntiles; d.astride = m.astride(); d.zstride = m.zstride();
  d.acts = acts; d.dz = dz; d.grads = grads;
  d.a_lo = m.info->a_lo; d.z_lo = m.info->z_lo; d.ring_cap = g_dw_ring_cap; d.private_max_tiles = g_dw_private;
  d.partial = m.dw_partial(dz, ntiles) + (size_t)slot_base * DW_SLOT_FLOATS;
  int rc;
  if (kind >= 2) {
    rc = launch_dw_wide_kernel(d, nw, kind == 2, s);
  } else if (kind == 1) {
    rc = s16::launch_dw_kernel(d, nw, true, s);
  } else if (g_dw16_variant == 3 || (g_dw16_variant == 1 && all_tiny)) {
    rc = s16::launch_dw_kernel(d, nw, false, s);
  } else {
    rc = launch<mlp_dw_kernel>("mlp dW", dim3(nw), dim3(64 * DW_WAVES), DW_LDS_BYTES, s, d);
  }
  if (rc) return rc;
  return launch<mlp_dw_reduce_kernel>("mlp dW reduce", dim3(257, nj), dim3(256), 0, s, d);
}

static int launch_dw(const Model& m, DwArgs& d, int nj, int64_t ntiles, const void* acts, void* dz, float* grads, hipStream_t s) {
  if (g_dw_job_mask) {
    hipError_t e = hipMemsetAsync(grads, 0, sizeof(float) * m.params, s);
    if (e != hipSuccess) return fail(NERF_E_HIP, "nerf_mlp_backward: memset: %s", hipGetErrorString(e));
  }
  const bool split_bf16 = m.split();
  if ((split_bf16 ? s16::g_dw_variant : g_dw16_variant) == 0)
    return launch_dw_part(m, d, nj, ntiles, acts, dz, grads, s, split_bf16 ? 1 : 0, 0, DW_MAX_WGS);
  DwArgs wide = d, rest = d;
  int nwide = 0, nrest = 0;
  for (int j = 0; j < nj; ++j) {
    if (d.jobs[j].nf == 16 && d.jobs[j].kf == 16) wide.jobs[nwide++] = d.jobs[j];
    else rest.jobs[nrest++] = d.jobs[j];
  }
  const int half = DW_MAX_WGS / 2;
  for (int turn = 0; turn < 2; ++turn) {
    const bool do_wide = (turn == 0) != (g_dw_narrow_first != 0);
    if (do_wide && nwide) {
      const int rc = launch_dw_part(m, wide, nwide, ntiles, acts, dz, grads, s, split_bf16 ? 2 : 3, half, half);
      if (rc) return rc;
    }
    if (!do_wide && nrest) {
      const int rc = launch_dw_part(m, rest, nrest, ntiles, acts, dz, grads, s, split_bf16 ? 1 : 0, 0, half);
      if (rc) return rc;
    }
  }
  return NERF_OK;
}

static int view_backward_chain(const Model& m, const void* packed, const void* acts, const float* d_raw, int64_t M, void* dz,
                               hipStream_t s) {
  const int64_t ntiles = (M + 31) / 32;
  if (m.split()) {
    if (g_bwd_stage != 2) {
      const int rcs = s16::backward_chain(m.stream<void>(packed, S_S16), acts, d_raw, M, dz, m.astride(), m.zstride(), ring_wgs(), s);
      if (rcs) return rcs;
    }
    return check_launch("mlp backward chain");
  }
  BwdArgs b;
  b.queue = nullptr;
  b.wb = m.stream<bf16x8>(packed, S_BWD);
  b.acts = acts; b.d_raw = d_raw; b.M = M; b.dz = dz; b.astride = m.astride(); b.zstride = m.zstride();
  const int variant = g_mlp_variant == 0 ? 3 : g_mlp_variant;
  const char* what = "mlp backward chain";
  if (variant >= 3) {
    b.queue = passq_slot();
    if (g_bwd_stage == 2) return check_launch(what);
    if (g_ring_split == 2)
      return launch<mlp_bwd_ring_kernel<SPLIT_NW, SPLIT_CHUNK>>(
          what, dim3(persistent_grid((ntiles + SPLIT_NW - 1) / SPLIT_NW, 2 * (int64_t)ring_wgs())), dim3(64 * SPLIT_NW), SPLIT_LDS_BYTES, s, b);
    return launch<mlp_bwd_ring_kernel<>>(what, dim3(ring_grid(ntiles)), dim3(512), RING_LDS_BYTES, s, b);
  }
  const int st = variant == 2 ? 2 : 1;
  const int64_t blocks = (ntiles + 4 * st - 1) / (4 * st);
  return with_bool(st == 1, [&](auto one) {
    return launch<mlp_bwd_kernel<decltype(one)::value ? 1 : 2>>(what, dim3((unsigned)blocks), dim3(256), 0, s, b);
  });
}

static int mlp_backward_impl(const nerf_mlp_arch* arch, const void* packed, const void* acts, const float* d_raw,
                             int64_t M, void* dz, float* grads, float* d_x, void* stream) {
  NERF_RESOLVE("nerf_mlp_backward");
  NERF_REQUIRE(!d_x || m.shape == Shape::Small, NERF_E_UNSUPPORTED,
               "nerf_mlp_backward_inputs: input gradients exist for the (2x64) model only (the 8x256 models take fixed encodings)");
  NERF_REQUIRE(packed && acts && d_raw && dz && grads, NERF_E_NULL, "nerf_mlp_backward: NULL pointer");
  NERF_REQUIRE(M > 0, NERF_E_SHAPE, "nerf_mlp_backward: M must be > 0");
  auto s = as_stream(stream);
  const int64_t ntiles = (M + 31) / 32;
  if (m.prec == Prec::F32)
    return f32::backward(m.stream<void>(packed, S_F32), acts, d_raw, M, dz, grads, m.shape == Shape::Image ? m.out_ch : 0, s);
  int rc;
  if (m.shape == Shape::Small) {
    if (m.split()) {
      rc = s16x::small_backward_chain(m.stream<void>(packed, S_S16), acts, d_raw, M, dz, d_x, m.astride(), m.zstride(), s);
    } else {
      SmallArgs a;
      small_args(a, m, packed);
      a.d_raw = d_raw; a.acts = const_cast<void*>(acts); a.dz = dz; a.M = M; a.d_x = d_x;
      rc = launch<mlp_small_bwd_kernel>("mlp backward chain (2x64 model)", dim3(small_grid(ntiles)), dim3(512), LN::LDS_BYTES, s, a);
    }
  } else if (m.shape == Shape::Image) {
    if (m.split()) {
      rc = s16x::img_backward_chain(m.stream<void>(packed, S_S16), acts, d_raw, M, m.out_ch, dz, m.astride(), m.zstride(), ring_wgs(), s);
    } else {
      ImgArgs a;
      img_args(a, m, packed);
      a.d_out = d_raw; a.acts = const_cast<void*>(acts); a.dz = dz; a.M = M;
      rc = launch<mlp_img_bwd_ring_kernel>("mlp backward chain (image model)", dim3(ring_grid(ntiles)), dim3(512), RING_LDS_BYTES, s, a);
    }
  } else {
    rc = view_backward_chain(m, packed, acts, d_raw, M, dz, s);
    if (!rc && g_bwd_stage == 1) return NERF_OK;
  }
  if (rc) return rc;
  DwArgs d;
  const int nj = m.dw_jobs(d.jobs, m.shape == Shape::View ? g_dw_job_mask : 0);
  return launch_dw(m, d, nj, ntiles, acts, dz, grads, s);
}

static int ngp_query_fused_impl(const nerf_mlp_arch* arch, const void* packed, const float* rays, const float* z,
                                int64_t B, int n, const float* tables, const void* tables_half, int L, int log2_T, int F,
                                const int* resolutions_host, const float* lw_host, int sh_degree, float pos_scale,
                                float pos_offset, float* raw, void* acts, void* stream) {
  const Model m = resolve(arch);
  NERF_REQUIRE(m.ok && m.shape == Shape::Small, NERF_E_UNSUPPORTED, "nerf_ngp_query_fused: needs the (2x64, in 32+16) model");
  NERF_REQUIRE(L == 16 && F == 2 && sh_degree == 3, NERF_E_UNSUPPORTED,
               "nerf_ngp_query_fused: fused rows exist for 16 levels x 2 features + SH degree 3 (use nerf_ngp_encode + nerf_mlp_forward otherwise)");
  NERF_REQUIRE(log2_T >= 1 && log2_T <= 30, NERF_E_SHAPE, "nerf_ngp_query_fused: need 1<=log2_T<=30");
  if (B <= 0 || n <= 0) return NERF_OK;
  NERF_REQUIRE(packed && rays && z && tables && resolutions_host && raw, NERF_E_NULL, "nerf_ngp_query_fused: NULL pointer");
  const int64_t M = B * n;
  NERF_REQUIRE(M < (1ll << 31), NERF_E_SHAPE, "nerf_ngp_query_fused: B*n must be < 2^31");
  LevelTab lt;
  if (lw_host)
    NERF_REQUIRE(level_tab_fill(lt, lw_host, L), NERF_E_SHAPE, "nerf_ngp_query_fused_lw: level weights must be finite and in [0, 1]");
  if (m.split()) {
    s16x::SmallQuery q;
    q.rays = rays; q.z = z; q.n = n; q.tables = tables; q.T = 1u << log2_T; q.pos_scale = pos_scale; q.pos_offset = pos_offset;
    for (int l = 0; l < 32; ++l) q.res[l] = l < L ? (float)resolutions_host[l] : 0.0f;
    q.B = B; q.ray_major = g_ngp_ray_major;
    q.use_lw = lw_host != nullptr;
    if (lw_host) for (int l = 0; l < 32; ++l) q.lw[l] = lt.w[l];
    return s16x::small_forward(m.stream<void>(packed, S_S16), m.stream<float>(packed, S_BIAS), nullptr, M, raw, acts, m.astride(), &q,
                               as_stream(stream));
  }
  SmallArgs a;
  small_args(a, m, packed);
  a.out = raw; a.acts = acts; a.M = M; a.rays = rays; a.z = z; a.n = n; a.tables = tables; a.T = 1u << log2_T;
  a.tables_h = static_cast<const uint32_t*>(tables_half);
  a.pos_scale = pos_scale; a.pos_offset = pos_offset;
  for (int l = 0; l < 32; ++l) a.rt.res[l] = l < L ? (float)resolutions_host[l] : 0.0f;
  a.B = B;
  a.ray_major = (!acts && g_ngp_ray_major && B >= 32) ? 1 : 0;
  const dim3 g(small_grid(a.ray_major ? ((B + 31) / 32) * (int64_t)n : (M + 31) / 32));
  if (lw_host) a.lw = lt;
  return with_bool(acts != nullptr, [&](auto store) { return with_bool(lw_host != nullptr, [&](auto lw) {
    return launch<mlp_small_fwd_kernel<decltype(store)::value, true, decltype(lw)::value>>(
        lw_host ? "nerf_ngp_query_fused_lw" : "nerf_ngp_query_fused", g, dim3(512), LN::LDS_BYTES, as_stream(stream), a);
  }); });
}

extern "C" int nerf_ngp_query_fused_h(const nerf_mlp_arch* arch, const void* packed, const float* rays, const float* z,
                                      int64_t B, int n, const float* tables, const void* tables_half, int L, int log2_T, int F,
                                      const int* resolutions_host, int sh_degree, float pos_scale, float pos_offset,
                                      float* raw, void* acts, void* stream) {
  return ngp_query_fused_impl(arch, packed, rays, z, B, n, tables, tables_half, L, log2_T, F, resolutions_host, nullptr, sh_degree,
                              pos_scale, pos_offset, raw, acts, stream);
}

extern "C" int nerf_ngp_query_fused_lw(const nerf_mlp_arch* arch, const void* packed, const float* rays, const float* z,
                                       int64_t B, int n, const float* tables, const void* tables_half, int L, int log2_T, int F,
                                       const int* resolutions_host, const float* level_weights_host, int sh_degree,
                                       float pos_scale, float pos_offset, float* raw, void* acts, void* stream) {
  return ngp_query_fused_impl(arch, packed, rays, z, B, n, tables, tables_half, L, log2_T, F, resolutions_host, level_weights_host,
                              sh_degree, pos_scale, pos_offset, raw, acts, stream);
}

extern "C" int nerf_ngp_query_fused(const nerf_mlp_arch* arch, const void* packed, const float* rays, const float* z,
                                    int64_t B, int n, const float* tables, int L, int log2_T, int F,
                                    const int* resolutions_host, int sh_degree, float pos_scale, float pos_offset,
                                    float* raw, void* acts, void* stream) {
  return nerf_ngp_query_fused_h(arch, packed, rays, z, B, n, tables, nullptr, L, log2_T, F, resolutions_host, sh_degree, pos_scale,
                                pos_offset, raw, acts, stream);
}

extern "C" int nerf_mlp_backward(const nerf_mlp_arch* arch, const void* packed, const void* acts, const float* d_raw,
                                 int64_t M, void* dz, float* grads, void* stream) {
  return mlp_backward_impl(arch, packed, acts, d_raw, M, dz, grads, nullptr, stream);
}

extern "C" int nerf_mlp_backward_inputs(const nerf_mlp_arch* arch, const void* packed, const void* acts,
                                        const float* d_raw, int64_t M, void* dz, float* grads, float* d_x,
                                        void* stream) {
  NERF_REQUIRE(d_x, NERF_E_NULL, "nerf_mlp_backward_inputs: d_x is NULL");
  return mlp_backward_impl(arch, packed, acts, d_raw, M, dz, grads, d_x, stream);
}

namespace nerf {
__global__ void __launch_bounds__(256) decode_frags_kernel(const void* base, int64_t stride16, int slot0, int nfrag,
                                                           int64_t M, float* __restrict__ out, int lo_off) {
  const int64_t total = M * nfrag * 2;
  for (int64_t t = blockIdx.x * (int64_t)blockDim.x + threadIdx.x; t < total; t += (int64_t)gridDim.x * blockDim.x) {
    const int h = (int)(t & 1), ks = (int)((t >> 1) % nfrag);
    const int64_t m = t / (2 * nfrag);
    const bf16x8 v = *frag_ptr(const_cast<void*>(base), m >> 5, stride16, slot0 + ks, (int)(m & 31), h);
#pragma unroll
    for (int j = 0; j < 8; ++j) out[m * (16 * nfrag) + kperm(ks, h, j)] = (float)v[j];
    if (lo_off > 0) {
      const bf16x8 w = *frag_ptr(const_cast<void*>(base), m >> 5, stride16, slot0 + lo_off + ks, (int)(m & 31), h);
#pragma unroll
      for (int j = 0; j < 8; ++j) out[m * (16 * nfrag) + kperm(ks, h, j)] += (float)w[j];
    }
  }
}
}

extern "C" int nerf_mlp_debug_width(const nerf_mlp_arch* arch, int kind, int layer) {
  const Model m = resolve(arch);
  if (!m.ok) return -1;
  if (m.prec == Prec::F32) return f32::debug_width(kind, layer);
  const DebugSlot ds = m.debug_slot(kind, layer);
  return ds.nfrag ? 16 * ds.nfrag : -1;
}

extern "C" int nerf_mlp_debug_read(const nerf_mlp_arch* arch, const void* store, int kind, int layer, int64_t M,
                                   float* out, void* stream) {
  NERF_RESOLVE("nerf_mlp_debug_read");
  if (m.prec == Prec::F32) {
    NERF_REQUIRE(store && out, NERF_E_NULL, "nerf_mlp_debug_read: NULL pointer");
    return M <= 0 ? NERF_OK : f32::debug_read(store, kind, layer, M, out, as_stream(stream));
  }
  const DebugSlot ds = m.debug_slot(kind, layer);
  NERF_REQUIRE(ds.nfrag, NERF_E_SHAPE, "nerf_mlp_debug_read: no such (kind, layer) in this architecture's stores");
  NERF_REQUIRE(store && out, NERF_E_NULL, "nerf_mlp_debug_read: NULL pointer");
  if (M <= 0) return NERF_OK;
  const int lo_off = !m.split() ? 0 : kind == 0 ? m.info->a_lo : m.info->z_lo;
  return launch<decode_frags_kernel>("nerf_mlp_debug_read", dim3(grid_for(M * ds.nfrag * 2, 256)), dim3(256), 0, as_stream(stream), store,
                                     kind == 0 ? m.astride() : m.zstride(), ds.slot, ds.nfrag, M, out, lo_off);
}

NERF_STAMP2_EXPORT(nerf_debug_stamps2_ring16)
#ifdef NERF_CLOCK_STAMP
extern "C" int nerf_debug_stamps(unsigned long long* host_out, int nwg) {
  if (nwg > 4096) nwg = 4096;
  return hipMemcpyFromSymbol(host_out, HIP_SYMBOL(nerf::g_stamps), (size_t)nwg * 32) == hipSuccess ? 0 : -4;
}
#endif
```

### nerf_meets_mlx_amd/csrc/mlp_dww.hip

```cpp
#include "mlp_s16_dev.h"

#ifndef NERF_DWX
#define NERF_DWX 0
#endif

namespace nerf {
using s16::mfma32;

constexpr int DWW_STAGES = 4, DWW_STAGE_BYTES = 32 * 1024, DWW_LDS_BYTES = DWW_STAGES * DWW_STAGE_BYTES;
constexpr int DWW_WAVES = 4, DWW_DPW = 8;
constexpr int DWW_SLICES = 8;

struct WOps { bf16x8 ah[4], al[4], bh[4], bl[4]; };

typedef __attribute__((address_space(3))) s16x4* lds_s16x4_p;
__device__ __forceinline__ bf16x8 trw(unsigned addr) {
#if NERF_DWX & 2
  bf16x8 r; asm volatile("" : "=v"(r) : "v"(addr)); return r;
#else
  const s16x4 lo = __builtin_amdgcn_ds_read_tr16_b64_v4i16((lds_s16x4_p)(uintptr_t)addr);
  const s16x4 hi = __builtin_amdgcn_ds_read_tr16_b64_v4i16((lds_s16x4_p)(uintptr_t)(addr + 256));
  union { struct { s16x4 a, b; } s; bf16x8 v; } cvt;
  cvt.s.a = lo; cvt.s.b = hi;
  return cvt.v;
#endif
}

__device__ __forceinline__ void dma_block_nt(const char* gbase_uniform, unsigned lane_off, unsigned lds_addr) {
  asm volatile("s_mov_b32 m0, %2\n\ts_nop 0\n\tglobal_load_lds_dwordx4 %0, %1 nt"
               :: "v"(lane_off), "s"(gbase_uniform), "s"(lds_addr) : "memory", "m0");
}

template <bool B> struct BoolC { static constexpr bool value = B; };

template <bool SPLIT>
__global__ void __launch_bounds__(64 * DWW_WAVES) mlp_dww_kernel(DwArgs a) {
  constexpr int MPS = SPLIT ? 6 : 4;
  char* smem = ring_smem;
  int bj = blockIdx.x, job_id = 0;
  while (bj >= a.splits[job_id]) { bj -= a.splits[job_id]; ++job_id; }
  const DwJob jb = a.jobs[job_id];
  const int tile_lo = (int)((int64_t)a.ntiles * bj / a.splits[job_id]);
  const int tile_hi = (int)((int64_t)a.ntiles * (bj + 1) / a.splits[job_id]);
  const int tid = threadIdx.x, lane = tid & 63;
  const int wv = __builtin_amdgcn_readfirstlane(tid >> 6);
  const int wr = wv >> 1, wc = wv & 1, rot = 2 * wc;
  f32x16 acc[4][4];
#pragma unroll
  for (int i = 0; i < 4; ++i)
#pragma unroll
    for (int k = 0; k < 4; ++k)
#pragma unroll
      for (int e = 0; e < 16; ++e) acc[i][k][e] = 0.0f;
  float bsum[4] = {0.0f, 0.0f, 0.0f, 0.0f};

  const unsigned lds0 = __builtin_amdgcn_readfirstlane(lds_addr_of(smem));
  const int g16 = lane >> 4, i16 = lane & 15, hq = g16 >> 1, fsel = g16 & 1, q = i16 >> 2, p = i16 & 3;
  const unsigned lane_rd = lds0 + 64 * (8 * hq + q) + 32 * fsel + 16 * (p & 1) + 8 * (p >> 1);
  const unsigned rdA0 = lane_rd + (4 * wr + rot) * 1024, rdA1 = lane_rd + (4 * wr + (rot ^ 2)) * 1024;
  const unsigned rdB = lane_rd + (16 + 4 * wc) * 1024;
  const int src_row = lane >> 2, src_sel = (lane >> 1) & 1, src_half = lane & 1;
  unsigned lane_off[DWW_DPW];
#pragma unroll
  for (int k = 0; k < DWW_DPW; ++k) {
    const int j = wv + 4 * (k & 3), lo_part = j >> 3, t = j & 7;
    const int slot = (k < 4 ? jb.dz_slot + (SPLIT ? lo_part * a.z_lo : 0) : jb.act_slot + (SPLIT ? lo_part * a.a_lo : 0)) + 2 * t + src_sel;
    lane_off[k] = (unsigned)(slot * 1024 + 32 * src_row + 16 * src_half + (SPLIT ? 0 : 512 * lo_part));
  }
  const char* dzb = reinterpret_cast<const char*>(a.dz);
  const char* acb = reinterpret_cast<const char*>(a.acts);
  long long zstride_b = a.zstride * 16, astride_b = a.astride * 16;
  unsigned ldsw = lds0 + wv * 1024;
  asm volatile("" : "+s"(zstride_b), "+s"(astride_b), "+s"(dzb), "+s"(acb), "+s"(ldsw));

  const int ht_lo = SPLIT ? 2 * tile_lo : tile_lo, n = SPLIT ? 2 * (tile_hi - tile_lo) : tile_hi - tile_lo;
  auto issue_k = [&](int ht, int slot, int k) {
#if !(NERF_DWX & 1)
    const long long tile = SPLIT ? ht >> 1 : ht;
    const char* base = (k < 4 ? dzb + tile * zstride_b : acb + tile * astride_b) + (SPLIT ? 512 * (ht & 1) : 0);
    dma_block_nt(base, lane_off[k], ldsw + slot * DWW_STAGE_BYTES + k * 4096);
#endif
  };
  auto read_tile = [&](WOps& o, int r, unsigned so) {
    if (r < 4) o.al[r] = trw((r < 2 ? rdA0 : rdA1) + so + (r & 1) * 1024 + 8192);
    else if (r < 8) o.bh[r - 4] = trw(rdB + so + (r - 4) * 1024);
    else if (r < 12) o.ah[r - 8] = trw((r - 8 < 2 ? rdA0 : rdA1) + so + (r & 1) * 1024);
    else o.bl[r - 12] = trw(rdB + so + (r - 12) * 1024 + 8192);
  };
  auto mfma_m = [&](const WOps& o, int m) {
#if !(NERF_DWX & 16)
    const int pt = m >> 4, i = (m >> 2) & 3, k = m & 3;
    if (SPLIT) {
      if (pt == 0) acc[i][k] = mfma32(o.al[i], o.bh[k], acc[i][k]);
      else if (pt == 1) acc[i][k] = mfma32(o.ah[i], o.bl[k], acc[i][k]);
      else acc[i][k] = mfma32(o.ah[i], o.bh[k], acc[i][k]);
    } else {
      if (pt == 0) acc[i][k] = mfma32(o.ah[i], o.bh[k], acc[i][k]);
      else acc[i][k] = mfma32(o.al[i], o.bl[k], acc[i][k]);
    }
#else
    asm volatile("" :: "v"(o.al[m & 3]), "v"(o.ah[m & 3]), "v"(o.bh[m & 3]), "v"(o.bl[m & 3]));
#endif
  };
  auto dot_d = [&](const WOps& o, int d) {
#if !(NERF_DWX & 8)
    const int t = d >> 3, part = (d >> 2) & 1, w = d & 3;
    const bf16x8& v = part ? o.al[t] : o.ah[t];
    const bf16x2 ones = {(__bf16)1.0f, (__bf16)1.0f};
    const bf16x2 pr = {v[2 * w], v[2 * w + 1]};
    bsum[2 * t + part] = __builtin_amdgcn_fdot2_f32_bf16(pr, ones, bsum[2 * t + part], false);
#endif
  };
  constexpr int RD0[DWW_SLICES + 1] = {0, 0, 3, 6, 9, 12, 14, 16, 16};
  constexpr int DM0[DWW_SLICES + 1] = {0, 0, 2, 3, 4, 5, 6, 7, 8};

  auto step = [&](WOps& use, WOps& ld, int j, int slot, auto full_c) {
    constexpr bool FULL = decltype(full_c)::value;
    const bool more = FULL || j + 1 < n, iss = FULL || j + 4 < n;
    __builtin_amdgcn_s_waitcnt(0xC07F);
#pragma unroll
    for (int m = 0; m < MPS; ++m) mfma_m(use, m);
    dot_d(use, 0); dot_d(use, 1);
    __builtin_amdgcn_sched_barrier(0);
    if (FULL) asm volatile("s_waitcnt vmcnt(16)" ::: "memory");
    else {
      const int younger = (n - 1 < j + 3 ? n - 1 : j + 3) - (j + 1);
      if (younger >= 2) asm volatile("s_waitcnt vmcnt(16)" ::: "memory");
      else if (younger == 1) asm volatile("s_waitcnt vmcnt(8)" ::: "memory");
      else asm volatile("s_waitcnt vmcnt(0)" ::: "memory");
    }
#if !(NERF_DWX & 4)
    __builtin_amdgcn_s_barrier();
#endif
    const unsigned so = (unsigned)(((slot + 1) & 3) * DWW_STAGE_BYTES);
#pragma unroll
    for (int s = 1; s < DWW_SLICES; ++s) {
      if (iss) {
#pragma unroll
        for (int k = DM0[s]; k < DM0[s + 1]; ++k) issue_k(ht_lo + j + 4, slot, k);
      }
      if (more) {
#pragma unroll
        for (int r = RD0[s]; r < RD0[s + 1]; ++r) read_tile(ld, r, so);
      }
#pragma unroll
      for (int m = MPS * s; m < MPS * (s + 1); ++m) mfma_m(use, m);
      dot_d(use, 2 * s); dot_d(use, 2 * s + 1);
      __builtin_amdgcn_sched_barrier(0);
    }
  };

  WOps x, y;
  if (n > 0) {
#pragma unroll
    for (int s_ = 0; s_ < DWW_STAGES; ++s_)
      if (s_ < n) {
#pragma unroll
        for (int k = 0; k < DWW_DPW; ++k) issue_k(ht_lo + s_, s_, k);
      }
    if (n >= 4) asm volatile("s_waitcnt vmcnt(24)" ::: "memory");
    else asm volatile("s_waitcnt vmcnt(0)" ::: "memory");
    __builtin_amdgcn_s_barrier();
#pragma unroll
    for (int r = 0; r < 16; ++r) read_tile(x, r, 0u);
  }
  int j = 0;
  for (; j + 5 < n; j += 2) {
    step(x, y, j, j & 3, BoolC<true>());
    step(y, x, j + 1, (j + 1) & 3, BoolC<true>());
  }
  for (; j < n; j += 2) {
    step(x, y, j, j & 3, BoolC<false>());
    if (j + 1 < n) step(y, x, j + 1, (j + 1) & 3, BoolC<false>());
  }

  const int rr = lane & 31, hh = lane >> 5;
  float* slot = a.partial + (size_t)blockIdx.x * DW_SLOT_FLOATS;
#pragma unroll
  for (int i = 0; i < 4; ++i) {
    const int nt = 4 * wr + ((i + rot) & 3);
#pragma unroll
    for (int k = 0; k < 4; ++k) {
      float* tile = slot + (8 * nt + 4 * wc + k) * 1024;
#pragma unroll
      for (int e = 0; e < 16; ++e) tile[((e & 3) + 8 * (e >> 2) + 4 * hh) * 32 + rr] = acc[i][k][e];
    }
  }
  if (jb.b_off >= 0) {
#pragma unroll
    for (int t = 0; t < 2; ++t) {
      const float v = bsum[2 * t + 1] + bsum[2 * t];
      const float tot = v + __shfl_xor(v, 32, 64);
      if (hh == 0) slot[64 * 1024 + 32 * (4 * wr + rot + t) + rr] = tot;
    }
  }
}

int launch_dw_wide_kernel(const DwArgs& d, int workgroups, bool split_bf16, hipStream_t s) {
  return with_bool(split_bf16, [&](auto split) {
    return launch<mlp_dww_kernel<decltype(split)::value>>(split_bf16 ? "mlp dW (split bf16, 256 x 256 jobs)" : "mlp dW (bf16, 256 x 256 jobs)",
                                                          dim3(workgroups), dim3(64 * DWW_WAVES), DWW_LDS_BYTES, s, d);
  });
}

}
```

### nerf_meets_mlx_amd/csrc/mlp_frag.h

```cpp
#pragma once
#include "mlp_layout.h"

namespace nerf {

struct Chan { int kind, dim, band; };
__host__ __device__ constexpr Chan chan_of(int c, int limit) {
  if (c < 3) return Chan{0, c, 0};
  if (c >= limit) return Chan{3, 0, 0};
  return Chan{((c - 3) % 6) >= 3 ? 2 : 1, (c - 3) % 3, (c - 3) / 6};
}

__device__ inline float fwd_src(const float* __restrict__ p, int f, int r, int h, int j) {
  int nt, ks;
  if (f < L::F_L1) {
    nt = f / 4; ks = f % 4;
    const int kk = kperm(ks, h, j);
    return kk < 63 ? p[L::P_W0 + (32 * nt + r) * 63 + kk] : 0.0f;
  }
  if (f < L::F_L5) {
    const int l = 1 + (f - L::F_L1) / 128, g = (f - L::F_L1) % 128;
    nt = g / 16; ks = g % 16;
    return p[L::pw(l) + (32 * nt + r) * 256 + kperm(ks, h, j)];
  }
  if (f < L::F_L6) {
// ... 21 lines not shown
    const int kk = kperm(ks, h, j), n = 32 * nt + r;
    if (kk < 256) return p[L::P_WD + n * 283 + kk];
    return (kk - 256) < 27 ? p[L::P_WD + n * 283 + kk] : 0.0f;
  }
  ks = f - L::F_RGB;
  return r < 3 ? p[L::P_WR + r * 128 + kperm(ks, h, j)] : 0.0f;
}

__device__ inline float bwd_src(const float* __restrict__ p, int f, int r, int h, int j) {
  if (f < L::B_DIR) {
    const int nn = kperm(0, h, j);
    return nn < 3 ? p[L::P_WR + nn * 128 + 32 * f + r] : 0.0f;
  }
  if (f < L::B_FA) {
    const int g = f - L::B_DIR, kt = g / 8, ns = g % 8;
    return p[L::P_WD + kperm(ns, h, j) * 283 + 32 * kt + r];
  }
  if (f < L::B_L7) {
    const int g = f - L::B_FA, kt = g / 17, ns = g % 17;
    const int nn = kperm(ns, h, j);
    if (ns < 16) return p[L::P_WF + nn * 256 + 32 * kt + r];
    return nn == 256 ? p[L::P_WA + 32 * kt + r] : 0.0f;
  }
  const int g = f - L::B_L7, li = g / 128, q = g % 128, kt = q / 16, ns = q % 16;
  const int l = 7 - li, nn = kperm(ns, h, j), row = 32 * kt + r;
  if (l == 5) return p[L::P_W5 + nn * 319 + 63 + row];
  return p[L::pw(l) + nn * 256 + row];
}

__device__ __forceinline__ bf16x8* frag_ptr(void* base, int64_t tile, int64_t stride16, int slot, int r, int h) {
  char* tb = reinterpret_cast<char*>(base) + tile * stride16 * 16;
  return reinterpret_cast<bf16x8*>(tb + slot * 1024 + (unsigned)(32 * r + 16 * h));
}

#ifndef NERF_NT_STORES
#define NERF_NT_STORES 1
#endif
constexpr bool g_nt_stores = NERF_NT_STORES != 0;

__device__ __forceinline__ void store_frag(void* base, int64_t tile, int64_t stride16, int slot, const bf16x8& v,
                                           int r, int h) {
#if NERF_ABLATE == 7
  asm volatile("" :: "v"(v));
  return;
#endif
#if NERF_ABLATE == 8
  tile = tile & 7;
#endif
  if (g_nt_stores) __builtin_nontemporal_store(v, frag_ptr(base, tile, stride16, slot, r, h));
  else *frag_ptr(base, tile, stride16, slot, r, h) = v;
}
template <int COUNT>
__device__ __forceinline__ void store_frags(void* base, int64_t tile, int64_t stride16, int slot0,
                                            const bf16x8 (&frags)[COUNT], int r, int h) {
#pragma unroll
  for (int k = 0; k < COUNT; ++k) store_frag(base, tile, stride16, slot0 + k, frags[k], r, h);
}
struct NoSink {
  __device__ __forceinline__ void put(int, int, const bf16x8&) const {}
};
template <bool ON>
struct FragSink {
  void* base; int64_t tile0, stride16; int slot0, r, h;
  __device__ __forceinline__ void put(int t, int idx, const bf16x8& v) const {
    if (ON) store_frag(base, tile0 + t, stride16, slot0 + idx, v, r, h);
  }
};

template <class WS>
__device__ __forceinline__ void acc_init_bias(f32x16& acc, WS& ws, int slot_tile, int h) {
#pragma unroll
  for (int g = 0; g < 4; ++g) {
    const float4 b = ws.bias4(slot_tile + 8 * g + 4 * h);
    acc[4 * g + 0] = b.x; acc[4 * g + 1] = b.y; acc[4 * g + 2] = b.z; acc[4 * g + 3] = b.w;
  }
}

typedef unsigned int u32x4 __attribute__((ext_vector_type(4)));

typedef short s16x2 __attribute__((ext_vector_type(2)));
typedef __bf16 bf16x2 __attribute__((ext_vector_type(2)));
typedef float f32x2 __attribute__((ext_vector_type(2)));
__device__ __forceinline__ bf16x2 pack2(float a, float b) {
  const f32x2 v = {a, b};
  return __builtin_convertvector(v, bf16x2);
}
__device__ __forceinline__ bf16x2 relu_pack(float a, float b) {
  s16x2 q = __builtin_bit_cast(s16x2, pack2(a, b));
  const s16x2 zero = {0, 0};
  q = __builtin_elementwise_max(q, zero);
  return __builtin_bit_cast(bf16x2, q);
}
__device__ __forceinline__ unsigned nonfinite_bits(const bf16x8& f) {
  const u32x4 w = __builtin_bit_cast(u32x4, f);
  unsigned b = 0;
#pragma unroll
  for (int i = 0; i < 4; ++i) b |= (w[i] & 0x7F807F80u) + 0x00800080u;
  return b & 0x80008000u;
}
template <int XOR_MASKS>
__device__ __forceinline__ int nonfinite_flags(unsigned pos_bits, unsigned dir_bits) {
  const unsigned long long mp = __ballot(pos_bits != 0u), md = __ballot(dir_bits != 0u);
  const int lane = (int)__lane_id();
  int f = 0;
#pragma unroll
  for (int x = 0; x < 64; x += 16)
    if ((x & ~XOR_MASKS) == 0) f |= (int)((mp >> (lane ^ x)) & 1ull) | ((int)((md >> (lane ^ x)) & 1ull) << 1);
  return f;
}
__device__ __forceinline__ float4 poison_raw(float4 o, int flags) {
  const float qnan = __builtin_nanf("");
  if (flags) { o.x = qnan; o.y = qnan; o.z = qnan; }
  if (flags & 1) o.w = qnan;
  return o;
}

__device__ __forceinline__ unsigned nonzero_bits(bf16x2 p) {
  unsigned r;
  asm("v_pk_min_u16 %0, %1, 1 op_sel_hi:[1,0]" : "=v"(r) : "v"(__builtin_bit_cast(unsigned, p)));
  return r;
}
template <int B>
__device__ __forceinline__ bf16x2 keep_where(bf16x2 p, unsigned w) {
  unsigned sel, r;
  asm("v_pk_lshrrev_b16 %0, %2, %1 op_sel_hi:[0,1]" : "=v"(sel) : "v"(w), "n"(B));
  sel &= 0x00010001u;
  asm("v_pk_mul_lo_u16 %0, %1, %2" : "=v"(r) : "v"(__builtin_bit_cast(unsigned, p)), "v"(sel));
  return __builtin_bit_cast(bf16x2, r);
}

template <bool RELU, bool MASKOUT>
__device__ __forceinline__ void finish_quarter(const f32x16& acc, int q, int nt, bf16x8& lo, bf16x8& hi, u32x4& mask) {
  unsigned w = 0;
#pragma unroll
  for (int p = 0; p < 2; ++p) {
    const int i = 4 * q + 2 * p, k = 2 * q + p;
    const bf16x2 pr = RELU ? relu_pack(acc[i], acc[i + 1]) : pack2(acc[i], acc[i + 1]);
    if (MASKOUT) w |= nonzero_bits(pr) << k;
    if (i < 8) { lo[i] = pr[0]; lo[i + 1] = pr[1]; } else { hi[i - 8] = pr[0]; hi[i - 7] = pr[1]; }
  }
  if (MASKOUT) mask[nt >> 1] |= w << (8 * (nt & 1));
}

__host__ __device__ constexpr int quarter_pos(int ks_count, int q) {
  return ks_count >= 8 ? (q * ks_count) / 4 + 1 : (q < ks_count ? q : ks_count - 1);
}

struct DwJob {
  int dz_slot, nf;
  int act_slot, kf;
  int w_off, ldw, col0;
  int n_valid, k_valid;
  int b_off;
};
constexpr int DW_MAX_JOBS = 16;
struct DwArgs {
  DwJob jobs[DW_MAX_JOBS];
  int splits[DW_MAX_JOBS];
  int ntiles;
  int64_t astride, zstride;
  const void* acts;
  const void* dz;
  float* grads;
  float* partial;
  int ring_cap;
  int private_max_tiles;
  int a_lo, z_lo;
};
constexpr int DW_SLOT_FLOATS = 64 * 1024 + 256;
constexpr int DW_MAX_WGS = 512;
constexpr int64_t DW_PARTIAL_BYTES = (int64_t)DW_MAX_WGS * DW_SLOT_FLOATS * 4;
int launch_dw_wide_kernel(const DwArgs& d, int workgroups, bool split_bf16, hipStream_t s);

}
```

### nerf_meets_mlx_amd/csrc/mlp_model.h

```cpp
#pragma once
#include "mlp_arch2.h"
#include "mlp_frag.h"
#include "mlp32.h"
#include "mlp22.h"
#include "mlp_s16.h"
#include "mlp_s16x.h"

namespace nerf {

inline int g_tile_pad16 = 0;

enum class Shape { View, Image, Small };
enum class Prec { Bf16, F32, Split };
enum Stream { S_FWD, S_BWD, S_BIAS, S_FWD16, S_F32, S_F22, S_S16, S_COUNT };

struct DebugSlot { int slot, nfrag; };
#define NERF_HIDDEN8(b) {b, 16}, {b + 16, 16}, {b + 32, 16}, {b + 48, 16}, {b + 64, 16}, {b + 80, 16}, {b + 96, 16}, {b + 112, 16}

constexpr DwJob view_pos(int l) { return {L::Z_L0 + 16 * l, 16, L::A_H0 + 16 * (l - 1), 16, L::pw(l), 256, 0, 256, 256, L::pb(l)}; }
constexpr DwJob img_pos(int l) { return {LI::Z_L0 + 16 * l, 16, LI::A_H0 + 16 * (l - 1), 16, LI::pw(l), 256, 0, 256, 256, LI::pb(l)}; }
constexpr DwJob VIEW_JOBS[] = {
    {L::Z_L0, 16, L::A_PE, 4, L::P_W0, 63, 0, 256, 63, L::P_B0},
    view_pos(1), view_pos(2), view_pos(3), view_pos(4),
    {L::Z_L0 + 80, 16, L::A_H0 + 64, 16, L::P_W5, 319, 63, 256, 256, L::P_B5},
    {L::Z_L0 + 80, 16, L::A_PE, 4, L::P_W5, 319, 0, 256, 63, -1},
    view_pos(6), view_pos(7),
    {L::Z_F, 16, L::A_H0 + 112, 16, L::P_WF, 256, 0, 256, 256, L::P_BF},
    {L::Z_A, 1, L::A_H0 + 112, 16, L::P_WA, 256, 0, 1, 256, L::P_BA},
    {L::Z_D, 8, L::A_FEAT, 16, L::P_WD, 283, 0, 128, 256, L::P_BD},
    {L::Z_D, 8, L::A_DPE, 2, L::P_WD, 283, 256, 128, 27, -1},
    {L::Z_RGB, 1, L::A_HD, 8, L::P_WR, 128, 0, 3, 128, L::P_BR},
};
constexpr DwJob IMG_JOBS[] = {
    {LI::Z_L0, 16, LI::A_X, 3, LI::P_W0, 40, 0, 256, 40, LI::P_B0},
    img_pos(1), img_pos(2), img_pos(3), img_pos(4),
    {LI::Z_L0 + 80, 16, LI::A_H0 + 64, 16, LI::P_W5, 296, 40, 256, 256, LI::P_B5},
    {LI::Z_L0 + 80, 16, LI::A_X, 3, LI::P_W5, 296, 0, 256, 40, -1},
    img_pos(6), img_pos(7),
    {LI::Z_OUT, 1, LI::A_H0 + 112, 16, LI::P_WO, 256, 0, 0, 256, 0},
};
constexpr DwJob SMALL_JOBS[] = {
    {LN::Z_L0, 4, LN::A_X, 2, LN::P_W0, 32, 0, 64, 32, LN::P_B0},
    {LN::Z_L1, 4, LN::A_H0, 4, LN::P_W1, 64, 0, 64, 64, LN::P_B1},
    {LN::Z_F, 4, LN::A_H1, 4, LN::P_WF, 64, 0, 64, 64, LN::P_BF},
    {LN::Z_A, 1, LN::A_H1, 4, LN::P_WA, 64, 0, 1, 64, LN::P_BA},
    {LN::Z_D, 2, LN::A_FEAT, 4, LN::P_WD, 80, 0, 32, 64, LN::P_BD},
    {LN::Z_D, 2, LN::A_DX, 1, LN::P_WD, 80, 64, 32, 16, -1},
    {LN::Z_RGB, 1, LN::A_HD, 2, LN::P_WR, 32, 0, 3, 32, LN::P_BR},
};

struct ShapeInfo {
  int64_t params;
  int f_frags, b_frags, bias_floats;
  int f16_frags;
  int64_t split_bytes;
  int a_slots[2], z_slots[2];
  int a_lo, z_lo;
  const DwJob* jobs; int njobs;
  DebugSlot debug[2][12];
};
constexpr ShapeInfo SHAPES[3] = {
    {L::P_TOTAL, L::F_TOTAL, L::B_PADDED, L::BI_TOTAL, L::F16_PADDED, s16::PACKED_BYTES,
     {L::A_SLOTS, s16::A_SLOTS}, {L::Z_SLOTS, s16::Z_SLOTS}, s16::A_LO, s16::Z_LO, VIEW_JOBS, sizeof(VIEW_JOBS) / sizeof(DwJob),
     {{NERF_HIDDEN8(L::A_H0), {L::A_FEAT, 16}, {L::A_HD, 8}, {L::A_PE, 4}, {L::A_DPE, 2}},
      {NERF_HIDDEN8(L::Z_L0), {L::Z_F, 16}, {L::Z_D, 8}, {L::Z_A, 1}, {L::Z_RGB, 1}}}},
    {LI::P_WO, LI::F_TOTAL, LI::B_PADDED, LI::BI_TOTAL, 0, s16x::IMG_PACKED_BYTES,
     {LI::A_SLOTS, s16x::IMG_A_SLOTS}, {LI::Z_SLOTS, s16x::IMG_Z_SLOTS}, s16x::IMG_A_LO, s16x::IMG_Z_LO, IMG_JOBS, sizeof(IMG_JOBS) / sizeof(DwJob),
     {{NERF_HIDDEN8(LI::A_H0), {0, 0}, {0, 0}, {LI::A_X, 3}, {0, 0}},
      {NERF_HIDDEN8(LI::Z_L0), {LI::Z_OUT, 1}, {0, 0}, {0, 0}, {0, 0}}}},
    {LN::P_TOTAL, LN::F_PADDED, LN::B_PADDED, LN::BI_TOTAL, 0, s16x::SM_PACKED_BYTES,
     {LN::A_SLOTS, s16x::SM_A_SLOTS}, {LN::Z_SLOTS, s16x::SM_Z_SLOTS}, s16x::SM_A_LO, s16x::SM_Z_LO, SMALL_JOBS, sizeof(SMALL_JOBS) / sizeof(DwJob),
     {{{LN::A_H0, 4}, {LN::A_H1, 4}, {0, 0}, {0, 0}, {0, 0}, {0, 0}, {0, 0}, {0, 0}, {LN::A_FEAT, 4}, {LN::A_HD, 2}, {LN::A_X, 2}, {LN::A_DX, 1}},
      {{LN::Z_L0, 4}, {LN::Z_L1, 4}, {0, 0}, {0, 0}, {0, 0}, {0, 0}, {0, 0}, {0, 0}, {LN::Z_F, 4}, {LN::Z_D, 2}, {LN::Z_A, 1}, {LN::Z_RGB, 1}}}},
};
#undef NERF_HIDDEN8

inline int64_t padded_tiles(int64_t M) { return (((M + 31) / 32) + 7) / 8 * 8; }

struct Model {
  bool ok = false;
  Shape shape; Prec prec; int out_ch;
  const ShapeInfo* info;
  int64_t params, packed_bytes;
  int64_t off[S_COUNT];
  int a_slots, z_slots;

  bool split() const { return prec == Prec::Split; }
  template <class T> const T* stream(const void* packed, Stream s) const { return reinterpret_cast<const T*>(static_cast<const char*>(packed) + off[s]); }
  template <class T> T* stream(void* packed, Stream s) const { return reinterpret_cast<T*>(static_cast<char*>(packed) + off[s]); }
  int64_t astride() const { return (int64_t)a_slots * 64 + g_tile_pad16; }
  int64_t zstride() const { return (int64_t)z_slots * 64 + g_tile_pad16; }
  int64_t acts_bytes(int64_t M) const { return !ok || M < 0 ? -1 : prec == Prec::F32 ? f32::acts_bytes(M) : padded_tiles(M) * astride() * 16; }
  int64_t dz_bytes(int64_t M) const {
    return !ok || M < 0 ? -1 : prec == Prec::F32 ? f32::dz_bytes(M) : padded_tiles(M) * zstride() * 16 + DW_PARTIAL_BYTES;
  }
  float* dw_partial(void* dz, int64_t ntiles) const { return reinterpret_cast<float*>(static_cast<char*>(dz) + padded_tiles(ntiles * 32) * zstride() * 16); }
  int dw_jobs(DwJob* dst, int mask) const {
    int nj = 0;
    for (int j = 0; j < info->njobs; ++j) {
      if (mask && !((mask >> j) & 1)) continue;
      dst[nj] = info->jobs[j];
      if (shape == Shape::Image && j == info->njobs - 1) { dst[nj].n_valid = out_ch; dst[nj].b_off = LI::P_WO + out_ch * 256; }
      ++nj;
    }
    return nj;
  }
  DebugSlot debug_slot(int kind, int layer) const {
    return (layer < 0 || layer > 11 || (kind != 0 && kind != 1)) ? DebugSlot{0, 0} : info->debug[kind][layer];
  }
};

inline Model resolve(const nerf_mlp_arch* a) {
  Model m{};
  m.params = m.packed_bytes = -1;
  if (!a) return m;
  if (a->precision != 0 && a->precision != 16 && a->precision != 32 && a->precision != 22) return m;
  m.prec = a->precision == 32 ? Prec::F32 : a->precision == 22 ? Prec::Split : Prec::Bf16;
  if (m.prec == Prec::F32 && !(a->n_layers == 8 && a->width == 256)) return m;
  if (a->n_layers == 2 && a->width == 64 && a->skip_layer < 0 && a->use_viewdirs == 1 && a->in_pos == 32 && a->in_dir == 16) m.shape = Shape::Small;
  else if (a->n_layers != 8 || a->width != 256 || a->skip_layer != 4) return m;
  else if (a->use_viewdirs == 1 && a->in_pos == 63 && a->in_dir == 27) m.shape = Shape::View;
  else if (a->use_viewdirs == 0 && a->in_pos == 40 && a->out_ch >= 1 && a->out_ch <= 4) m.shape = Shape::Image;
  else return m;
  const ShapeInfo& s = SHAPES[(int)m.shape];
  m.info = &s;
  m.out_ch = a->out_ch;
  m.params = s.params + (m.shape == Shape::Image ? (int64_t)a->out_ch * 257 : 0);
  m.a_slots = s.a_slots[m.split()]; m.z_slots = s.z_slots[m.split()];
  for (int i = 0; i < S_COUNT; ++i) m.off[i] = -1;
  int64_t end = 0;
  auto put = [&](Stream st, int64_t bytes) { m.off[st] = end; end += bytes; };
  put(S_FWD, (int64_t)s.f_frags * 1024);
  put(S_BWD, (int64_t)s.b_frags * 1024);
  put(S_BIAS, (int64_t)s.bias_floats * 4);
  if (s.f16_frags) put(S_FWD16, (int64_t)s.f16_frags * 1024);
  if (m.prec == Prec::F32) put(S_F32, f32::PACKED_BYTES);
  if (m.split() && m.shape == Shape::View) put(S_F22, f22::PACKED_BYTES);
  if (m.split()) put(S_S16, s.split_bytes);
  m.packed_bytes = end;
  m.ok = true;
  return m;
}

}
```

### nerf_meets_mlx_amd/csrc/mlp_s16.hip

```cpp
#include "mlp_s16_dev.h"
#include "mlp_s16.h"

#ifndef NERF_S16_RELOAD_PE
#define NERF_S16_RELOAD_PE 0
#endif

namespace nerf {
namespace s16 {

constexpr int F_CHUNKS = F_FRAGS / RING_CHUNK;
constexpr int B_CHUNKS = B_PADDED / RING_CHUNK;
static_assert(F_CHUNKS * RING_CHUNK == F_FRAGS && B_CHUNKS * RING_CHUNK == B_PADDED, "whole ring chunks");
static_assert(F_FRAGS == 2 * L::F_TOTAL && B_FRAGS == 2 * L::B_TOTAL, "pair streams");
static_assert(A_LO == L::A_MASK && A_MASK == 2 * L::A_MASK && A_SLOTS == A_MASK + 9, "activation slots");
static_assert(Z_LO == L::Z_SLOTS && Z_SLOTS == 2 * L::Z_SLOTS, "dZ slots");
constexpr int NW = 4;

typedef RingW<F_CHUNKS, F_FRAGS, 4, NW, RING_CHUNK, RING_STAGES, true> FwdRing;
typedef RingW<B_CHUNKS, B_FRAGS, 4, NW, RING_CHUNK, RING_STAGES, true> BwdRing;


constexpr int PACK_PAIRS = L::F_TOTAL + B_PADDED / 2;
__global__ void __launch_bounds__(256) pack_s16_kernel(const float* __restrict__ p, bf16x8* __restrict__ wf,
                                                       bf16x8* __restrict__ wb) {
// ... 237 lines not shown
  ws.lane16 = 16 * lane;
  ws.lds0 = __builtin_amdgcn_readfirstlane(lds_addr_of(ring_smem));
  ws.wv = wv;
  ws.start(lane);
  PassQueue pq;
  pq.init(a.queue, ws.lds0 + BwdRing::BIAS_OFF);
  for (int64_t sp = blockIdx.x; sp < nsuper;) {
    int ln = lane;
    asm volatile("" : "+v"(ln));
    ws.new_pass();
    bwd_tiles(a, ws, sp * NW + wv, ntiles, ln, pq);
    sp = pq.next(sp);
  }
  ws.drain();
  pq.leave();
}

#ifndef NERF_DWX
#define NERF_DWX 0
#endif
#if NERF_DWX & 4
#define DW_BARRIER() do {} while (0)
#else
#define DW_BARRIER() __builtin_amdgcn_s_barrier()
#endif
constexpr int DW_WAVES = 16, DW_NPW = 2;

__device__ __forceinline__ bf16x8 tr_pair(const char* blk, int hq, int fsel, int i16) {
  const int q = i16 >> 2, p = i16 & 3;
  const char* base = blk + 64 * (8 * hq + q) + 32 * fsel + 16 * (p & 1) + 8 * (p >> 1);
#if NERF_DWX & 2
  bf16x8 r; asm volatile("" : "=v"(r) : "v"(base)); return r;
#endif
  const s16x4 lo = __builtin_amdgcn_ds_read_tr16_b64_v4i16((__attribute__((address_space(3))) s16x4*)(base));
  const s16x4 hi = __builtin_amdgcn_ds_read_tr16_b64_v4i16((__attribute__((address_space(3))) s16x4*)(base + 256));
  union { struct { s16x4 a, b; } s; bf16x8 v; } cvt;
  cvt.s.a = lo; cvt.s.b = hi;
  return cvt.v;
}

constexpr int DW_LDS_BYTES = 160 * 1024;

constexpr int DWP_WAVE_BYTES = 10 * 1024;
template <int NT, int KT, bool SPLIT>
__device__ __forceinline__ void dw_private(const DwArgs& a, const DwJob& jb, int tile_lo, int tile_hi, char* smem, int wv, int lane) {
  constexpr int NP = 2 * (NT + KT);
  static_assert(NP * 1024 <= DWP_WAVE_BYTES && NT * KT <= 4, "wave-private dW: one stage per wave, at most four tiles");
  f32x16 acc[NT][KT];
#pragma unroll
  for (int i = 0; i < NT; ++i)
#pragma unroll
    for (int k = 0; k < KT; ++k)
#pragma unroll
      for (int e = 0; e < 16; ++e) acc[i][k][e] = 0.0f;
  float bsum[NT];
#pragma unroll
  for (int i = 0; i < NT; ++i) bsum[i] = 0.0f;
  const int g16 = lane >> 4, i16 = lane & 15, hq = g16 >> 1, fsel = g16 & 1;
  char* mine = smem + wv * DWP_WAVE_BYTES;
  const unsigned lds_mine = __builtin_amdgcn_readfirstlane(lds_addr_of(mine));
  const int src_row = lane >> 2, src_sel = (lane >> 1) & 1, src_half = lane & 1;
  const char* dzb = reinterpret_cast<const char*>(a.dz);
  const char* acb = reinterpret_cast<const char*>(a.acts);
  long long zstride_b = a.zstride * 16, astride_b = a.astride * 16;
  int z_lo = a.z_lo, a_lo = a.a_lo, dz_slot = jb.dz_slot, act_slot = jb.act_slot, nf = jb.nf, kf = jb.kf;
  asm volatile("" : "+s"(zstride_b), "+s"(astride_b), "+s"(z_lo), "+s"(a_lo), "+s"(dz_slot), "+s"(act_slot), "+s"(nf), "+s"(kf));
  const int ht_hi = SPLIT ? 2 * tile_hi : tile_hi;
  for (int ht = (SPLIT ? 2 * tile_lo : tile_lo) + wv; ht < ht_hi; ht += DW_WAVES) {
    asm volatile("s_waitcnt lgkmcnt(0)" ::: "memory");
#if !(NERF_DWX & 1)
    const int64_t tile = SPLIT ? ht >> 1 : ht;
    const unsigned row_off0 = (unsigned)(32 * ((SPLIT ? 16 * (ht & 1) : 0) + src_row) + 16 * src_half);
#pragma unroll
    for (int i = 0; i < NP; ++i) {
      const bool is_z = i < 2 * NT;
      const int j = is_z ? i : i - 2 * NT, nt_ = is_z ? NT : KT;
      const int lo_part = j >= nt_ ? 1 : 0, t = lo_part ? j - nt_ : j;
      const int nfr = is_z ? nf : kf;
      int fr = 2 * t + src_sel; if (fr >= nfr) fr = nfr - 1;
      const int slot = (is_z ? dz_slot + (SPLIT ? lo_part * z_lo : 0) : act_slot + (SPLIT ? lo_part * a_lo : 0)) + fr;
      const unsigned row_off = row_off0 + (SPLIT ? 0 : 512 * lo_part);
      dma_frag_nt((is_z ? dzb + tile * zstride_b : acb + tile * astride_b) + (int64_t)slot * 1024 + row_off, lds_mine + i * 1024);
    }
#endif
    asm volatile("s_waitcnt vmcnt(0)" ::: "memory");
    bf16x8 bh[KT], bl[KT];
#pragma unroll
    for (int k = 0; k < KT; ++k) {
      bh[k] = tr_pair(mine + (2 * NT + k) * 1024, hq, fsel, i16);
      bl[k] = tr_pair(mine + (2 * NT + KT + k) * 1024, hq, fsel, i16);
    }
#pragma unroll
    for (int i = 0; i < NT; ++i) {
      const bf16x8 ah = tr_pair(mine + i * 1024, hq, fsel, i16);
      const bf16x8 al = tr_pair(mine + (NT + i) * 1024, hq, fsel, i16);
#if !(NERF_DWX & 8)
      const bf16x2 ones = {(__bf16)1.0f, (__bf16)1.0f};
#pragma unroll
      for (int j = 0; j < 8; j += 2) {
        const bf16x2 ph = {ah[j], ah[j + 1]}, pl = {al[j], al[j + 1]};
        bsum[i] = __builtin_amdgcn_fdot2_f32_bf16(pl, ones, bsum[i], false);
        bsum[i] = __builtin_amdgcn_fdot2_f32_bf16(ph, ones, bsum[i], false);
      }
#endif
#if NERF_DWX & 16
      asm volatile("" :: "v"(ah), "v"(al), "v"(bh[0]), "v"(bl[0]));
#else
#pragma unroll
      for (int k = 0; k < KT; ++k) {
        if (SPLIT) {
          acc[i][k] = mfma32(al, bh[k], acc[i][k]);
          acc[i][k] = mfma32(ah, bl[k], acc[i][k]);
          acc[i][k] = mfma32(ah, bh[k], acc[i][k]);
        } else {
          acc[i][k] = mfma32(ah, bh[k], acc[i][k]);
          acc[i][k] = mfma32(al, bl[k], acc[i][k]);
        }
      }
#endif
    }
  }
  asm volatile("s_waitcnt vmcnt(0) lgkmcnt(0)" ::: "memory");
  float* xl = reinterpret_cast<float*>(smem);
  constexpr int GIVER_FLOATS = (NT * KT * 16 + NT) * 64;
#pragma unroll 1
  for (int h = DW_WAVES / 2; h >= 1; h >>= 1) {
    __builtin_amdgcn_s_barrier();
    if (wv >= h && wv < 2 * h) {
      float* dst = xl + (size_t)(wv - h) * GIVER_FLOATS + lane;
#pragma unroll
      for (int i = 0; i < NT; ++i) {
#pragma unroll
        for (int k = 0; k < KT; ++k)
#pragma unroll
          for (int e = 0; e < 16; ++e) dst[((i * KT + k) * 16 + e) * 64] = acc[i][k][e];
        dst[(NT * KT * 16 + i) * 64] = bsum[i];
      }
    }
    __builtin_amdgcn_s_barrier();
    if (wv < h) {
      const float* src = xl + (size_t)wv * GIVER_FLOATS + lane;
#pragma unroll
      for (int i = 0; i < NT; ++i) {
#pragma unroll
        for (int k = 0; k < KT; ++k)
#pragma unroll
          for (int e = 0; e < 16; ++e) acc[i][k][e] += src[((i * KT + k) * 16 + e) * 64];
        bsum[i] += src[(NT * KT * 16 + i) * 64];
      }
    }
  }
  if (wv != 0) return;
  const int rr = lane & 31, hh = lane >> 5;
  float* slot = a.partial + (size_t)blockIdx.x * DW_SLOT_FLOATS;
#pragma unroll
  for (int i = 0; i < NT; ++i) {
#pragma unroll
    for (int k = 0; k < KT; ++k) {
      float* tile = slot + (8 * i + k) * 1024;
#pragma unroll
      for (int e = 0; e < 16; ++e) tile[((e & 3) + 8 * (e >> 2) + 4 * hh) * 32 + rr] = acc[i][k][e];
    }
    if (jb.b_off >= 0) {
      const float tot = bsum[i] + __shfl_xor(bsum[i], 32, 64);
      if (hh == 0) slot[64 * 1024 + 32 * i + rr] = tot;
    }
  }
}

template <bool SPLIT>
__global__ void __launch_bounds__(64 * DW_WAVES) s16_dw_kernel(DwArgs a) {
  char* smem = ring_smem;
  int bj = blockIdx.x, job_id = 0;
  while (bj >= a.splits[job_id]) { bj -= a.splits[job_id]; ++job_id; }
  const DwJob jb = a.jobs[job_id];
  const int tile_lo = (int)((int64_t)a.ntiles * bj / a.splits[job_id]);
  const int tile_hi = (int)((int64_t)a.ntiles * (bj + 1) / a.splits[job_id]);
  const int tid = threadIdx.x, lane = tid & 63;
  const int wv = __builtin_amdgcn_readfirstlane(tid >> 6);
  const int n_tiles = (jb.nf + 1) >> 1, k_tiles = (jb.kf + 1) >> 1;
  const bool col_major = k_tiles <= 2;
  const int wr = col_major ? (wv & 3) : (wv >> 2), wc = col_major ? (wv >> 2) : (wv & 3);
  const int npairs = 2 * (n_tiles + k_tiles);
  if (a.private_max_tiles >= n_tiles * k_tiles && npairs * 1024 <= DWP_WAVE_BYTES) {
    switch (8 * n_tiles + k_tiles) {
      case 8 * 1 + 1: dw_private<1, 1, SPLIT>(a, jb, tile_lo, tile_hi, smem, wv, lane); return;
      case 8 * 1 + 2: dw_private<1, 2, SPLIT>(a, jb, tile_lo, tile_hi, smem, wv, lane); return;
      case 8 * 1 + 3: dw_private<1, 3, SPLIT>(a, jb, tile_lo, tile_hi, smem, wv, lane); return;
      case 8 * 1 + 4: dw_private<1, 4, SPLIT>(a, jb, tile_lo, tile_hi, smem, wv, lane); return;
      case 8 * 2 + 1: dw_private<2, 1, SPLIT>(a, jb, tile_lo, tile_hi, smem, wv, lane); return;
      case 8 * 2 + 2: dw_private<2, 2, SPLIT>(a, jb, tile_lo, tile_hi, smem, wv, lane); return;
      case 8 * 3 + 1: dw_private<3, 1, SPLIT>(a, jb, tile_lo, tile_hi, smem, wv, lane); return;
      case 8 * 4 + 1: dw_private<4, 1, SPLIT>(a, jb, tile_lo, tile_hi, smem, wv, lane); return;
      default: break;
    }
  }
  const bool active = (wr * DW_NPW < n_tiles) && (wc * 2 < k_tiles);
  const int kc = (k_tiles + 1) >> 1;
  int stride = npairs * 1024, ns = DW_LDS_BYTES / stride;
  if (ns > a.ring_cap) ns = a.ring_cap;
  const int cnt_w = (wv < npairs ? 1 : 0) + (wv + DW_WAVES < npairs ? 1 : 0);
  f32x16 acc[DW_NPW][2];
#pragma unroll
  for (int i = 0; i < DW_NPW; ++i)
#pragma unroll
    for (int k = 0; k < 2; ++k)
#pragma unroll
      for (int e = 0; e < 16; ++e) acc[i][k][e] = 0.0f;
  float bsum[2 * DW_NPW];
  bool own[2 * DW_NPW];
#pragma unroll
  for (int c = 0; c < 2 * DW_NPW; ++c) { bsum[c] = 0.0f; own[c] = (c % kc) == wc && !(NERF_DWX & 8); }
  const int g16 = lane >> 4, i16 = lane & 15, hq = g16 >> 1, fsel = g16 & 1;
  const unsigned lds0 = __builtin_amdgcn_readfirstlane(lds_addr_of(smem));
  const int src_row = lane >> 2, src_sel = (lane >> 1) & 1, src_half = lane & 1;
  const char* dzb = reinterpret_cast<const char*>(a.dz);
  const char* acb = reinterpret_cast<const char*>(a.acts);
  long long zstride_b = a.zstride * 16, astride_b = a.astride * 16;
  int z_lo = a.z_lo, a_lo = a.a_lo, dz_slot = jb.dz_slot, act_slot = jb.act_slot, nf = jb.nf, kf = jb.kf;
  asm volatile("" : "+s"(zstride_b), "+s"(astride_b), "+s"(z_lo), "+s"(a_lo), "+s"(dz_slot), "+s"(act_slot), "+s"(nf), "+s"(kf),
               "+s"(stride), "+s"(ns));

  auto issue = [&](int ht, int slot) {
#if NERF_DWX & 1
    return;
#endif
    const unsigned st = lds0 + __builtin_amdgcn_readfirstlane(slot) * stride;
    const int64_t tile = SPLIT ? ht >> 1 : ht;
    const unsigned row_off0 = (unsigned)(32 * ((SPLIT ? 16 * (ht & 1) : 0) + src_row) + 16 * src_half);
#pragma unroll
    for (int k = 0; k < DW_NPW; ++k) {
      const int i = wv + DW_WAVES * k;
      if (i < npairs) {
        const bool is_z = i < 2 * n_tiles;
        const int j = is_z ? i : i - 2 * n_tiles;
        const int nt_ = is_z ? n_tiles : k_tiles;
        const int lo_part = j >= nt_ ? 1 : 0;
        const int t = lo_part ? j - nt_ : j;
        const int nfr = is_z ? nf : kf;
        int fr = 2 * t + src_sel; if (fr >= nfr) fr = nfr - 1;
        const int slot_ = (is_z ? dz_slot + (SPLIT ? lo_part * z_lo : 0) : act_slot + (SPLIT ? lo_part * a_lo : 0)) + fr;
        const unsigned row_off = row_off0 + (SPLIT ? 0 : 512 * lo_part);
        const char* src = (is_z ? dzb + tile * zstride_b : acb + tile * astride_b) + (int64_t)slot_ * 1024 + row_off;
        dma_frag_nt(src, st + i * 1024);
      }
    }
  };
  auto process = [&](const char* st) {
    if (active) {
      bf16x8 bh[2], bl[2];
#pragma unroll
      for (int k = 0; k < 2; ++k) {
        const int kt = wc * 2 + k;
        const int b = 2 * n_tiles + (kt < k_tiles ? kt : 0);
        bh[k] = tr_pair(st + b * 1024, hq, fsel, i16);
        bl[k] = tr_pair(st + (b + k_tiles) * 1024, hq, fsel, i16);
      }
#pragma unroll
      for (int i = 0; i < DW_NPW; ++i) {
        const int nt = wr * DW_NPW + i;
        const int b = nt < n_tiles ? nt : 0;
        const bf16x8 ah = tr_pair(st + b * 1024, hq, fsel, i16);
        const bf16x8 al = tr_pair(st + (b + n_tiles) * 1024, hq, fsel, i16);
        const bf16x2 ones = {(__bf16)1.0f, (__bf16)1.0f};
        if (own[2 * i]) {
          asm volatile("" ::: "memory");
#pragma unroll
          for (int j = 0; j < 8; j += 2) { const bf16x2 q = {ah[j], ah[j + 1]}; bsum[2 * i] = __builtin_amdgcn_fdot2_f32_bf16(q, ones, bsum[2 * i], false); }
        }
        if (own[2 * i + 1]) {
          asm volatile("" ::: "memory");
#pragma unroll
          for (int j = 0; j < 8; j += 2) { const bf16x2 q = {al[j], al[j + 1]}; bsum[2 * i + 1] = __builtin_amdgcn_fdot2_f32_bf16(q, ones, bsum[2 * i + 1], false); }
        }
#if NERF_DWX & 16
        asm volatile("" :: "v"(ah), "v"(al), "v"(bh[0]), "v"(bl[0]), "v"(bh[1]), "v"(bl[1]));
#else
#pragma unroll
        for (int k = 0; k < 2; ++k) {
          if (SPLIT) {
            acc[i][k] = mfma32(al, bh[k], acc[i][k]);
            acc[i][k] = mfma32(ah, bl[k], acc[i][k]);
            acc[i][k] = mfma32(ah, bh[k], acc[i][k]);
          } else {
            acc[i][k] = mfma32(ah, bh[k], acc[i][k]);
            acc[i][k] = mfma32(al, bl[k], acc[i][k]);
          }
        }
#endif
      }
    }
  };
  auto wait_landed = [&](int younger) {
    switch (younger * cnt_w) {
#define NERF_VM_CASE(N) case N: asm volatile("s_waitcnt vmcnt(" #N ") lgkmcnt(0)" ::: "memory"); break;
      NERF_VM_CASE(0) NERF_VM_CASE(1) NERF_VM_CASE(2) NERF_VM_CASE(3) NERF_VM_CASE(4) NERF_VM_CASE(5) NERF_VM_CASE(6) NERF_VM_CASE(7)
      NERF_VM_CASE(8) NERF_VM_CASE(9) NERF_VM_CASE(10) NERF_VM_CASE(11) NERF_VM_CASE(12) NERF_VM_CASE(13) NERF_VM_CASE(14)
      NERF_VM_CASE(16) NERF_VM_CASE(18) NERF_VM_CASE(20) NERF_VM_CASE(22) NERF_VM_CASE(24) NERF_VM_CASE(26) NERF_VM_CASE(28)
#undef NERF_VM_CASE
      default: asm volatile("s_waitcnt vmcnt(0) lgkmcnt(0)" ::: "memory"); break;
    }
  };
  const int ht_lo = SPLIT ? 2 * tile_lo : tile_lo, n = SPLIT ? 2 * (tile_hi - tile_lo) : tile_hi - tile_lo;
  int issued = 0, slot_i = 0, slot_p = 0;
  for (; issued < ns && issued < n; ++issued) { issue(ht_lo + issued, slot_i); slot_i = slot_i + 1 == ns ? 0 : slot_i + 1; }
  for (int p = 0; p < n; p += 2) {
    wait_landed(issued - (p + 2 < n ? p + 2 : n));
    DW_BARRIER();
#pragma unroll
    for (int k = 0; k < 2; ++k)
      if (issued < n && issued - ns < p) { issue(ht_lo + issued, slot_i); slot_i = slot_i + 1 == ns ? 0 : slot_i + 1; ++issued; }
    process(smem + slot_p * stride); slot_p = slot_p + 1 == ns ? 0 : slot_p + 1;
    if (SPLIT || p + 1 < n) { process(smem + slot_p * stride); slot_p = slot_p + 1 == ns ? 0 : slot_p + 1; }
  }
  asm volatile("s_waitcnt lgkmcnt(0)" ::: "memory");
  __builtin_amdgcn_s_barrier();
  float* xb = reinterpret_cast<float*>(smem);
#pragma unroll
  for (int c = 0; c < 2 * DW_NPW; ++c)
    if (own[c] && active) xb[(wr * 2 * DW_NPW + c) * 64 + lane] = bsum[c];
  __builtin_amdgcn_s_barrier();
  if (!active) return;
  const int rr = lane & 31, hh = lane >> 5;
  float* slot = a.partial + (size_t)blockIdx.x * DW_SLOT_FLOATS;
#pragma unroll
  for (int i = 0; i < DW_NPW; ++i) {
    const int nt = wr * DW_NPW + i;
    if (nt >= n_tiles) continue;
#pragma unroll
    for (int k = 0; k < 2; ++k) {
      const int kt = wc * 2 + k;
      if (kt >= k_tiles) continue;
      float* tile = slot + (8 * nt + kt) * 1024;
#pragma unroll
      for (int e = 0; e < 16; ++e) tile[((e & 3) + 8 * (e >> 2) + 4 * hh) * 32 + rr] = acc[i][k][e];
    }
    if (wc == 0 && jb.b_off >= 0) {
      const float lo = xb[(wr * 2 * DW_NPW + 2 * i + 1) * 64 + lane], hi = xb[(wr * 2 * DW_NPW + 2 * i) * 64 + lane];
      const float t = lo + hi;
      const float tot = t + __shfl_xor(t, 32, 64);
      if (hh == 0) slot[64 * 1024 + 32 * nt + rr] = tot;
    }
  }
}


int pack(const float* params, void* packed_s16, hipStream_t s) {
  char* base = static_cast<char*>(packed_s16);
  return launch<pack_s16_kernel>("nerf_mlp_pack (split-bf16 image)", dim3((PACK_PAIRS * 64 + 255) / 256), dim3(256), 0, s, params,
                                 reinterpret_cast<bf16x8*>(base), reinterpret_cast<bf16x8*>(base + (size_t)F_FRAGS * 1024));
}

int forward(const void* packed_s16, const float* bias_slots, const float* x, const float* rays, const float* z, int64_t M,
            int n, int freq_mode, float* out, void* acts, int64_t astride16, int persistent_wgs, hipStream_t s) {
  FwdArgs a;
  a.queue = passq_slot();
  a.wf = reinterpret_cast<const bf16x8*>(packed_s16);
  a.bias = bias_slots;
  a.x = x; a.rays = rays; a.z = z; a.M = M; a.n = n; a.out = out; a.acts = acts; a.astride = astride16;
  fill_freqs(a.fr.pos, a.fr.dir, freq_mode);
  const int64_t nsuper = ((M + 31) / 32 + NW - 1) / NW;
  return with_bool(x != nullptr, [&](auto rows) {
    return launch<s16_fwd_kernel<decltype(rows)::value ? 0 : 1>>("mlp training forward (split bf16)", dim3(persistent_grid(nsuper, persistent_wgs)),
                                                                  dim3(64 * NW), FwdRing::LDS_BYTES, s, a);
  });
}

int backward_chain(const void* packed_s16, const void* acts, const float* d_raw, int64_t M, void* dz, int64_t astride16,
                   int64_t zstride16, int persistent_wgs, hipStream_t s) {
  BwdArgs b;
  b.queue = passq_slot();
  b.wb = reinterpret_cast<const bf16x8*>(static_cast<const char*>(packed_s16) + (size_t)F_FRAGS * 1024);
  b.acts = acts; b.d_raw = d_raw; b.M = M; b.dz = dz; b.astride = astride16; b.zstride = zstride16;
  const int64_t nsuper = ((M + 31) / 32 + NW - 1) / NW;
  return launch<s16_bwd_kernel>("mlp backward chain (split bf16)", dim3(persistent_grid(nsuper, persistent_wgs)), dim3(64 * NW),
                                BwdRing::LDS_BYTES, s, b);
}

int g_dw_variant = 1;

int launch_dw_kernel(const DwArgs& d, int workgroups, bool split_bf16, hipStream_t s) {
  return with_bool(split_bf16, [&](auto split) {
    return launch<s16_dw_kernel<decltype(split)::value>>(split_bf16 ? "mlp dW (split bf16)" : "mlp dW (bf16)", dim3(workgroups), dim3(64 * DW_WAVES),
                                                         DW_LDS_BYTES, s, d);
  });
}

}
}
```

Before: 1.209 million.

## Merge weight-gradient jobs sharing dZ or activation fragments into wider compute jobs

Adds merged dW job tables in which logical weight-gradient GEMMs that share dZ fragments, or that read two activation ranges, run as one compute job. This lets each streamed dZ/activation tile be reused across more outputs and cuts the number of jobs and workgroup splits. The wide dW kernel is templated to 4x5 and 5x4 tile-per-wave shapes with larger LDS stages. The partial-slot layout is packed per launch, and the reduce kernel maps each logical job back onto its place inside a merged compute tile. This adds register pressure, index arithmetic and LDS use, and raises the risk of layout bugs.

```diff
diff --git a/include/nerf_hip.h b/include/nerf_hip.h
--- a/include/nerf_hip.h
+++ b/include/nerf_hip.h
@@ -141,6 +141,8 @@
 int nerf_mlp_debug_width(const nerf_mlp_arch* arch, int kind, int layer);
 int nerf_mlp_debug_read(const nerf_mlp_arch* arch, const void* store, int kind, int layer, int64_t M, float* out,
                         void* stream);
+
+int nerf_mlp_dw_describe(const nerf_mlp_arch* arch, int merge, int* compute, int* logical, int* counts);
 
 int nerf_ngp_query_fused(const nerf_mlp_arch* arch, const void* packed, const float* rays, const float* z, int64_t B,
                          int n, const float* tables, int L, int log2_T, int F, const int* resolutions_host,
diff --git a/nerf_meets_mlx_amd/_native.py b/nerf_meets_mlx_amd/_native.py
--- a/nerf_meets_mlx_amd/_native.py
+++ b/nerf_meets_mlx_amd/_native.py
@@ -51,6 +51,7 @@
     "nerf_mlp_backward": (_I, [_P, _P, _P, _P, _I64, _P, _P, _P]),
     "nerf_mlp_backward_inputs": (_I, [_P, _P, _P, _P, _I64, _P, _P, _P, _P]),
     "nerf_mlp_debug_width": (_I, [_P, _I, _I]),
+    "nerf_mlp_dw_describe": (_I, [_P, _I, _P, _P, _P]),
     "nerf_mlp_debug_read": (_I, [_P, _P, _I, _I, _I64, _P, _P]),
     "nerf_render_workspace_bytes": (_I64, [_I64, _I, _I]),
     "nerf_render_rays_fused": (_I, [_P, _P, _P, _P, _I64, _I, _I, _P, _I, _I, _P, _P, _P, _P, _P, _P, _P, _P, _P, _P]),
diff --git a/nerf_meets_mlx_amd/csrc/dw_split.h b/nerf_meets_mlx_amd/csrc/dw_split.h
--- a/nerf_meets_mlx_amd/csrc/dw_split.h
+++ b/nerf_meets_mlx_amd/csrc/dw_split.h
@@ -5,6 +5,8 @@
 
 constexpr int DW_SPLIT_MAX_JOBS = 16;
 struct DwCost { int nf, kf; };
+
+inline DwCost dw_wide_cost(int nf, int kf) { return DwCost{2 * ((nf + 1) / 2), 2 * ((kf + 1) / 2)}; }
 
 inline int dw_split(const DwCost* jobs, int nj, int bias, int target_wgs, int64_t max_splits, int* splits) {
   int64_t units[DW_SPLIT_MAX_JOBS], total_units = 0;
diff --git a/nerf_meets_mlx_amd/csrc/mlp.hip b/nerf_meets_mlx_amd/csrc/mlp.hip
--- a/nerf_meets_mlx_amd/csrc/mlp.hip
+++ b/nerf_meets_mlx_amd/csrc/mlp.hip
@@ -957,7 +957,7 @@
   if (a.ntiles > 0) return;
 #endif
   const int rr = lane & 31, hh = lane >> 5;
-  float* slot = a.partial + (size_t)blockIdx.x * DW_SLOT_FLOATS;
+  float* slot = a.partial + (size_t)blockIdx.x * a.slot_floats;
 #pragma unroll
   for (int i = 0; i < DW_NPW; ++i) {
     const int nt = wr * DW_NPW + i;
@@ -966,34 +966,32 @@
     for (int k = 0; k < 2; ++k) {
       const int kt = wc * 2 + k;
       if (kt >= k_tiles) continue;
-      float* tile = slot + (8 * nt + kt) * 1024;
+      float* tile = slot + (jb.kts * nt + kt) * 1024;
 #pragma unroll
       for (int e = 0; e < 16; ++e) tile[((e & 3) + 8 * (e >> 2) + 4 * hh) * 32 + rr] = acc[i][k][e];
     }
     if (wc == 0 && jb.b_off >= 0) {
       const float tot = bsum[i] + __shfl_xor(bsum[i], 32, 64);
-      if (hh == 0) slot[64 * 1024 + 32 * nt + rr] = tot;
-    }
-  }
-}
-
-__global__ void __launch_bounds__(256) mlp_dw_reduce_kernel(DwArgs a) {
-  const int j = blockIdx.y;
-  const DwJob jb = a.jobs[j];
-  int first = 0;
-  for (int q = 0; q < j; ++q) first += a.splits[q];
-  const int S = a.splits[j];
+      if (hh == 0) slot[a.bias_off + 32 * nt + rr] = tot;
+    }
+  }
+}
+
+__global__ void __launch_bounds__(256) mlp_dw_reduce_kernel(DwRedArgs a) {
+  const DwRedJob jb = a.jobs[blockIdx.y];
+  const int S = jb.splits;
+  const size_t stride = (size_t)a.slot_floats;
   const int nw = jb.n_valid * jb.k_valid, nb = jb.b_off >= 0 ? jb.n_valid : 0;
-  const float* base = a.partial + (size_t)first * DW_SLOT_FLOATS;
+  const float* base = a.partial + (size_t)jb.first * stride;
   for (int t = blockIdx.x * 256 + threadIdx.x; t < nw + nb; t += gridDim.x * 256) {
     const float* src;
     float* dst;
     if (t < nw) {
       const int n = t / jb.k_valid, k = t - n * jb.k_valid;
-      src = base + (8 * (n >> 5) + (k >> 5)) * 1024 + (n & 31) * 32 + (k & 31);
+      src = base + (jb.kts * (jb.nt0 + (n >> 5)) + jb.kt0 + (k >> 5)) * 1024 + (n & 31) * 32 + (k & 31);
       dst = a.grads + jb.w_off + (int64_t)n * jb.ldw + jb.col0 + k;
     } else {
-      src = base + 64 * 1024 + (t - nw);
+      src = base + a.bias_off + 32 * jb.nt0 + (t - nw);
       dst = a.grads + jb.b_off + (t - nw);
     }
     float sum = 0.0f;
@@ -1001,11 +999,11 @@
     for (; sidx + 8 <= S; sidx += 8) {
       float v[8];
 #pragma unroll
-      for (int q = 0; q < 8; ++q) v[q] = __builtin_nontemporal_load(src + (size_t)(sidx + q) * DW_SLOT_FLOATS);
+      for (int q = 0; q < 8; ++q) v[q] = __builtin_nontemporal_load(src + (size_t)(sidx + q) * stride);
 #pragma unroll
       for (int q = 0; q < 8; ++q) sum += v[q];
     }
-    for (; sidx < S; ++sidx) sum += __builtin_nontemporal_load(src + (size_t)sidx * DW_SLOT_FLOATS);
+    for (; sidx < S; ++sidx) sum += __builtin_nontemporal_load(src + (size_t)sidx * stride);
     *dst = sum;
   }
 }
@@ -1388,6 +1386,7 @@
 }
 
 static int g_dw_wgs = 0;
+static int g_dw_merge = 1;
 static int g_dw_bias = -1;
 static int g_bwd_stage = 0;
 static int g_dw_ring_cap = 8;
@@ -1431,6 +1430,7 @@
     {"hash_combine_max_res", &g_hash_combine_max_res, opt_clamp<0, INT_MAX>, nullptr},
     {"ngp_ray_major", &g_ngp_ray_major, opt_flag, nullptr},
     {"dw22_variant", &s16::g_dw_variant, opt_flag, nullptr},
+    {"dw_merge", &g_dw_merge, opt_flag, nullptr},
     {"dw16_variant", &g_dw16_variant, opt_clamp<0, 3>, nullptr},
     {"dw_private_tiles", &g_dw_private, opt_clamp<0, 4>, nullptr},
     {"dw_ring_cap", &g_dw_ring_cap, opt_clamp<2, 16>, nullptr},
@@ -1631,33 +1631,66 @@
   return view_forward(m, packed, nullptr, rays, z, B * n, n, freq_mode, raw, acts, stream);
 }
 
-static int launch_dw_part(const Model& m, DwArgs& d, int nj, int64_t ntiles, const void* acts, void* dz, float* grads,
-                          hipStream_t s, int kind, int slot_base, int max_wgs) {
+static void dw_slot_layout(DwArgs& d, int nc, bool packed) {
+  int tiles = 64, rows = 8;
+  if (packed) {
+    tiles = rows = 0;
+    for (int j = 0; j < nc; ++j) {
+      DwJob& jb = d.jobs[j];
+      const int nt = (jb.nf + 1) / 2;
+      jb.kts = (jb.kf + 1) / 2 + (jb.kf2 + 1) / 2;
+      if (nt * jb.kts > tiles) tiles = nt * jb.kts;
+      if (nt > rows) rows = nt;
+    }
+  }
+  d.bias_off = tiles * 1024;
+  d.slot_floats = packed ? d.bias_off + 64 * ((32 * rows + 63) / 64) : DW_SLOT_FLOATS;
+}
+
+static int launch_dw_part(const Model& m, DwArgs& d, int nc, const DwJob* logical, int nl, int64_t ntiles, const void* acts, void* dz,
+                          float* grads, hipStream_t s, int kind, int64_t float_base, int max_wgs, int* reduced) {
   static_assert(DW_SPLIT_MAX_JOBS == DW_MAX_JOBS, "dw_split.h sizes its arrays for DwArgs::jobs");
   DwCost cost[DW_MAX_JOBS];
-  for (int j = 0; j < nj; ++j) cost[j] = DwCost{d.jobs[j].nf, d.jobs[j].kf};
+  for (int j = 0; j < nc; ++j) cost[j] = kind >= 2 ? dw_wide_cost(d.jobs[j].nf, d.jobs[j].kf + d.jobs[j].kf2) : DwCost{d.jobs[j].nf, d.jobs[j].kf + d.jobs[j].kf2};
   int target_wgs = g_dw_wgs > 0 ? g_dw_wgs : cu_count();
   if (target_wgs > max_wgs) target_wgs = max_wgs;
-  const int nw = dw_split(cost, nj, g_dw_bias >= 0 ? g_dw_bias : m.split() ? 2 : 128, target_wgs, (ntiles + 3) / 4, d.splits);
-  NERF_REQUIRE(slot_base + nw <= DW_MAX_WGS, NERF_E_SHAPE, "nerf_mlp_backward: dw_workgroups must be <= %d", DW_MAX_WGS);
-  bool all_tiny = true;
-  for (int j = 0; j < nj; ++j) all_tiny = all_tiny && ((d.jobs[j].nf + 1) / 2) * ((d.jobs[j].kf + 1) / 2) <= 4;
+  const int nw = dw_split(cost, nc, g_dw_bias >= 0 ? g_dw_bias : m.split() ? 2 : 128, target_wgs, (ntiles + 3) / 4, d.splits);
+  NERF_REQUIRE(float_base + (int64_t)nw * d.slot_floats <= (int64_t)DW_MAX_WGS * DW_SLOT_FLOATS, NERF_E_SHAPE,
+               "nerf_mlp_backward: dw_workgroups must be <= %d", DW_MAX_WGS);
+  bool all_tiny = true, two_ranges = false;
+  for (int j = 0; j < nc; ++j) {
+    all_tiny = all_tiny && ((d.jobs[j].nf + 1) / 2) * ((d.jobs[j].kf + 1) / 2) <= 4;
+    two_ranges = two_ranges || d.jobs[j].kf2 > 0;
+  }
   d.ntiles = (int)ntiles; d.astride = m.astride(); d.zstride = m.zstride();
   d.acts = acts; d.dz = dz; d.grads = grads;
   d.a_lo = m.info->a_lo; d.z_lo = m.info->z_lo; d.ring_cap = g_dw_ring_cap; d.private_max_tiles = g_dw_private;
-  d.partial = m.dw_partial(dz, ntiles) + (size_t)slot_base * DW_SLOT_FLOATS;
+  d.partial = m.dw_partial(dz, ntiles) + float_base;
   int rc;
   if (kind >= 2) {
     rc = launch_dw_wide_kernel(d, nw, kind == 2, s);
   } else if (kind == 1) {
     rc = s16::launch_dw_kernel(d, nw, true, s);
-  } else if (g_dw16_variant == 3 || (g_dw16_variant == 1 && all_tiny)) {
+  } else if (g_dw16_variant == 3 || (g_dw16_variant == 1 && all_tiny) || two_ranges) {
     rc = s16::launch_dw_kernel(d, nw, false, s);
   } else {
     rc = launch<mlp_dw_kernel>("mlp dW", dim3(nw), dim3(64 * DW_WAVES), DW_LDS_BYTES, s, d);
   }
   if (rc) return rc;
-  return launch<mlp_dw_reduce_kernel>("mlp dW reduce", dim3(257, nj), dim3(256), 0, s, d);
+  DwRedArgs r;
+  int nr = 0, first[DW_MAX_JOBS];
+  for (int j = 0, f = 0; j < nc; ++j) { first[j] = f; f += d.splits[j]; }
+  for (int l = 0; l < nl; ++l) {
+    int nt0, kt0;
+    const int c = dw_locate(logical[l], d.jobs, nc, &nt0, &kt0);
+    if (c < 0) continue;
+    const DwJob& lj = logical[l];
+    r.jobs[nr++] = DwRedJob{first[c], d.splits[c], d.jobs[c].kts, nt0, kt0, lj.w_off, lj.ldw, lj.col0, lj.n_valid, lj.k_valid, lj.b_off};
+  }
+  r.partial = d.partial; r.grads = grads; r.slot_floats = d.slot_floats; r.bias_off = d.bias_off;
+  *reduced += nr;
+  if (nr == 0) return NERF_OK;
+  return launch<mlp_dw_reduce_kernel>("mlp dW reduce", dim3(257, nr), dim3(256), 0, s, r);
 }
 
 static int launch_dw(const Model& m, DwArgs& d, int nj, int64_t ntiles, const void* acts, void* dz, float* grads, hipStream_t s) {
@@ -1665,27 +1698,37 @@
     hipError_t e = hipMemsetAsync(grads, 0, sizeof(float) * m.params, s);
     if (e != hipSuccess) return fail(NERF_E_HIP, "nerf_mlp_backward: memset: %s", hipGetErrorString(e));
   }
+  DwJob logical[DW_MAX_JOBS];
+  for (int j = 0; j < nj; ++j) logical[j] = d.jobs[j];
+  int reduced = 0;
   const bool split_bf16 = m.split();
-  if ((split_bf16 ? s16::g_dw_variant : g_dw16_variant) == 0)
-    return launch_dw_part(m, d, nj, ntiles, acts, dz, grads, s, split_bf16 ? 1 : 0, 0, DW_MAX_WGS);
+  if ((split_bf16 ? s16::g_dw_variant : g_dw16_variant) == 0) {
+    dw_slot_layout(d, nj, false);
+    return launch_dw_part(m, d, nj, logical, nj, ntiles, acts, dz, grads, s, split_bf16 ? 1 : 0, 0, DW_MAX_WGS, &reduced);
+  }
+  const bool merge = g_dw_merge && !g_dw_job_mask && m.info->nmjobs > 0;
+  const int nc = merge ? m.dw_merged_jobs(d.jobs) : nj;
   DwArgs wide = d, rest = d;
   int nwide = 0, nrest = 0;
-  for (int j = 0; j < nj; ++j) {
-    if (d.jobs[j].nf == 16 && d.jobs[j].kf == 16) wide.jobs[nwide++] = d.jobs[j];
+  for (int j = 0; j < nc; ++j) {
+    if (dww_shape(d.jobs[j])) wide.jobs[nwide++] = d.jobs[j];
     else rest.jobs[nrest++] = d.jobs[j];
   }
+  dw_slot_layout(wide, nwide, merge);
+  dw_slot_layout(rest, nrest, merge);
   const int half = DW_MAX_WGS / 2;
   for (int turn = 0; turn < 2; ++turn) {
     const bool do_wide = (turn == 0) != (g_dw_narrow_first != 0);
     if (do_wide && nwide) {
-      const int rc = launch_dw_part(m, wide, nwide, ntiles, acts, dz, grads, s, split_bf16 ? 2 : 3, half, half);
+      const int rc = launch_dw_part(m, wide, nwide, logical, nj, ntiles, acts, dz, grads, s, split_bf16 ? 2 : 3, (int64_t)half * rest.slot_floats, half, &reduced);
       if (rc) return rc;
     }
     if (!do_wide && nrest) {
-      const int rc = launch_dw_part(m, rest, nrest, ntiles, acts, dz, grads, s, split_bf16 ? 1 : 0, 0, half);
+      const int rc = launch_dw_part(m, rest, nrest, logical, nj, ntiles, acts, dz, grads, s, split_bf16 ? 1 : 0, 0, half, &reduced);
       if (rc) return rc;
     }
   }
+  NERF_REQUIRE(reduced == nj, NERF_E_SHAPE, "nerf_mlp_backward: %d of %d weight-gradient jobs have a compute job", reduced, nj);
   return NERF_OK;
 }
 
@@ -1857,6 +1900,39 @@
 }
 }
 
+extern "C" int nerf_mlp_dw_describe(const nerf_mlp_arch* arch, int merge, int* compute, int* logical, int* counts) {
+  NERF_RESOLVE("nerf_mlp_dw_describe");
+  NERF_REQUIRE(m.prec != Prec::F32, NERF_E_UNSUPPORTED, "nerf_mlp_dw_describe: the fp32 kernels have their own job table");
+  NERF_REQUIRE(compute && logical && counts, NERF_E_NULL, "nerf_mlp_dw_describe: NULL pointer");
+  DwArgs d, part[2];
+  DwJob lj[DW_MAX_JOBS];
+  const int nl = m.dw_jobs(lj, 0);
+  const bool merged = merge && m.info->nmjobs > 0;
+  const int nc = merged ? m.dw_merged_jobs(d.jobs) : m.dw_jobs(d.jobs, 0);
+  int np[2] = {0, 0}, where[DW_MAX_JOBS], idx[DW_MAX_JOBS];
+  for (int j = 0; j < nc; ++j) {
+    where[j] = dww_shape(d.jobs[j]) ? 1 : 0;
+    idx[j] = np[where[j]];
+    part[where[j]].jobs[np[where[j]]++] = d.jobs[j];
+  }
+  dw_slot_layout(part[0], np[0], merged);
+  dw_slot_layout(part[1], np[1], merged);
+  for (int j = 0; j < nc; ++j) {
+    const DwArgs& pa = part[where[j]];
+    const DwJob& c = pa.jobs[idx[j]];
+    const int row[10] = {c.dz_slot, c.nf, c.act_slot, c.kf, c.act_slot2, c.kf2, dww_shape(c), c.kts, pa.slot_floats, pa.bias_off};
+    for (int q = 0; q < 10; ++q) compute[10 * j + q] = row[q];
+  }
+  for (int l = 0; l < nl; ++l) {
+    int nt0 = 0, kt0 = 0;
+    const int c = dw_locate(lj[l], d.jobs, nc, &nt0, &kt0);
+    const int row[9] = {c, nt0, kt0, lj[l].w_off, lj[l].ldw, lj[l].col0, lj[l].n_valid, lj[l].k_valid, lj[l].b_off};
+    for (int q = 0; q < 9; ++q) logical[9 * l + q] = row[q];
+  }
+  counts[0] = nc; counts[1] = nl;
+  return NERF_OK;
+}
+
 extern "C" int nerf_mlp_debug_width(const nerf_mlp_arch* arch, int kind, int layer) {
   const Model m = resolve(arch);
   if (!m.ok) return -1;
diff --git a/nerf_meets_mlx_amd/csrc/mlp_dww.hip b/nerf_meets_mlx_amd/csrc/mlp_dww.hip
--- a/nerf_meets_mlx_amd/csrc/mlp_dww.hip
+++ b/nerf_meets_mlx_amd/csrc/mlp_dww.hip
@@ -7,11 +7,12 @@
 namespace nerf {
 using s16::mfma32;
 
-constexpr int DWW_STAGES = 4, DWW_STAGE_BYTES = 32 * 1024, DWW_LDS_BYTES = DWW_STAGES * DWW_STAGE_BYTES;
-constexpr int DWW_WAVES = 4, DWW_DPW = 8;
+constexpr int DWW_STAGES = 4;
+constexpr int DWW_LDS_MAX = DWW_STAGES * 36 * 1024;
+constexpr int DWW_WAVES = 4;
 constexpr int DWW_SLICES = 8;
 
-struct WOps { bf16x8 ah[4], al[4], bh[4], bl[4]; };
+template <int NI, int NK> struct WOps { bf16x8 ah[NI], al[NI], bh[NK], bl[NK]; };
 
 typedef __attribute__((address_space(3))) s16x4* lds_s16x4_p;
 __device__ __forceinline__ bf16x8 trw(unsigned addr) {
@@ -31,40 +32,64 @@
                :: "v"(lane_off), "s"(gbase_uniform), "s"(lds_addr) : "memory", "m0");
 }
 
+__device__ __forceinline__ void mfma32_v(const bf16x8& a, const bf16x8& b, f32x16& c) {
+  asm volatile("s_nop 1\n\tv_mfma_f32_32x32x16_bf16 %0, %1, %2, %0" : "+v"(c) : "v"(a), "v"(b));
+}
+__device__ __forceinline__ void mfma_v_drain() { asm volatile("s_nop 15\n\ts_nop 15" ::: "memory"); }
+
 template <bool B> struct BoolC { static constexpr bool value = B; };
-
-template <bool SPLIT>
-__global__ void __launch_bounds__(64 * DWW_WAVES) mlp_dww_kernel(DwArgs a) {
-  constexpr int MPS = SPLIT ? 6 : 4;
+template <int V> struct IntC { static constexpr int value = V; };
+
+template <bool SPLIT, int NI, int NK>
+__device__ __forceinline__ void dww_job(const DwArgs& a, const DwJob& jb, int bj, int nsplit) {
+  static_assert((NI == 4 || NI == 5) && (NK == 4 || NK == 5) && NI + NK <= 9, "4 x 4, 4 x 5 or 5 x 4 tiles per wave");
+  constexpr int NZT = NI == 5 ? 9 : 8, NHT = NK == 5 ? 10 : 8;
+  constexpr int NB = 2 * (NZT + NHT), STAGE_BYTES = NB * 1024;
+  constexpr int DPW = (NB + DWW_WAVES - 1) / DWW_WAVES;
+  constexpr bool UNEVEN = NB % DWW_WAVES != 0;
+  constexpr int NX = NK == 5 ? 4 : NI == 5 ? 2 : 0;
+  constexpr int NT = 16 + NX, MT = NT * (SPLIT ? 3 : 2);
+  constexpr int NR = 2 * (NI + NK);
+  constexpr int NBT = NI == 5 ? 3 : 2;
+  static_assert(DWW_STAGES * STAGE_BYTES <= DWW_LDS_MAX && 3 * DPW < 64, "LDS ring, vmcnt range");
   char* smem = ring_smem;
-  int bj = blockIdx.x, job_id = 0;
-  while (bj >= a.splits[job_id]) { bj -= a.splits[job_id]; ++job_id; }
-  const DwJob jb = a.jobs[job_id];
-  const int tile_lo = (int)((int64_t)a.ntiles * bj / a.splits[job_id]);
-  const int tile_hi = (int)((int64_t)a.ntiles * (bj + 1) / a.splits[job_id]);
+  const int tile_lo = (int)((int64_t)a.ntiles * bj / nsplit);
+  const int tile_hi = (int)((int64_t)a.ntiles * (bj + 1) / nsplit);
   const int tid = threadIdx.x, lane = tid & 63;
   const int wv = __builtin_amdgcn_readfirstlane(tid >> 6);
-  const int wr = wv >> 1, wc = wv & 1, rot = 2 * wc;
-  f32x16 acc[4][4];
+  const int wr = wv >> 1, wc = wv & 1, rot = 2 * wc, rotb = NI == 5 ? 2 * wr : 0;
+  const bool last_dma = !UNEVEN || wv < NB % DWW_WAVES;
+  f32x16 acc[4][4], accx[NX > 0 ? NX : 1];
 #pragma unroll
   for (int i = 0; i < 4; ++i)
 #pragma unroll
     for (int k = 0; k < 4; ++k)
 #pragma unroll
       for (int e = 0; e < 16; ++e) acc[i][k][e] = 0.0f;
-  float bsum[4] = {0.0f, 0.0f, 0.0f, 0.0f};
+#pragma unroll
+  for (int i = 0; i < NX; ++i)
+#pragma unroll
+    for (int e = 0; e < 16; ++e) accx[i][e] = 0.0f;
+  float bsum[2 * NBT];
+#pragma unroll
+  for (int i = 0; i < 2 * NBT; ++i) bsum[i] = 0.0f;
 
   const unsigned lds0 = __builtin_amdgcn_readfirstlane(lds_addr_of(smem));
   const int g16 = lane >> 4, i16 = lane & 15, hq = g16 >> 1, fsel = g16 & 1, q = i16 >> 2, p = i16 & 3;
   const unsigned lane_rd = lds0 + 64 * (8 * hq + q) + 32 * fsel + 16 * (p & 1) + 8 * (p >> 1);
-  const unsigned rdA0 = lane_rd + (4 * wr + rot) * 1024, rdA1 = lane_rd + (4 * wr + (rot ^ 2)) * 1024;
-  const unsigned rdB = lane_rd + (16 + 4 * wc) * 1024;
+  const unsigned rdA0 = lane_rd + (4 * wr + rot) * 1024, rdA1 = lane_rd + (4 * wr + (rot ^ 2)) * 1024, rdA4 = lane_rd + 8 * 1024;
+  const unsigned rdB0 = lane_rd + (2 * NZT + 4 * wc + rotb) * 1024, rdB1 = NI == 5 ? lane_rd + (2 * NZT + 4 * wc + (rotb ^ 2)) * 1024 : rdB0 + 2048;
+  const unsigned rdB4 = lane_rd + (2 * NZT + 8 + wc) * 1024;
   const int src_row = lane >> 2, src_sel = (lane >> 1) & 1, src_half = lane & 1;
-  unsigned lane_off[DWW_DPW];
-#pragma unroll
-  for (int k = 0; k < DWW_DPW; ++k) {
-    const int j = wv + 4 * (k & 3), lo_part = j >> 3, t = j & 7;
-    const int slot = (k < 4 ? jb.dz_slot + (SPLIT ? lo_part * a.z_lo : 0) : jb.act_slot + (SPLIT ? lo_part * a.a_lo : 0)) + 2 * t + src_sel;
+  unsigned lane_off[DPW];
+  const int z_lo = __builtin_amdgcn_readfirstlane(a.z_lo), a_lo = __builtin_amdgcn_readfirstlane(a.a_lo);
+#pragma unroll
+  for (int k = 0; k < DPW; ++k) {
+    const int j = (tid >> 6) + 4 * k;
+    const bool dz = j < 2 * NZT;
+    const int jo = dz ? j : j - 2 * NZT, nt = dz ? NZT : NHT, lo_part = jo >= nt ? 1 : 0, t = jo - lo_part * nt;
+    const int first = dz ? jb.dz_slot + 2 * t : t < 8 ? jb.act_slot + 2 * t : jb.act_slot2 + 2 * (t - 8);
+    const int slot = first + (SPLIT ? lo_part * (dz ? z_lo : a_lo) : 0) + src_sel;
     lane_off[k] = (unsigned)(slot * 1024 + 32 * src_row + 16 * src_half + (SPLIT ? 0 : 512 * lo_part));
   }
   const char* dzb = reinterpret_cast<const char*>(a.dz);
@@ -76,20 +101,30 @@
   const int ht_lo = SPLIT ? 2 * tile_lo : tile_lo, n = SPLIT ? 2 * (tile_hi - tile_lo) : tile_hi - tile_lo;
   auto issue_k = [&](int ht, int slot, int k) {
 #if !(NERF_DWX & 1)
+    if (UNEVEN && k == DPW - 1 && !last_dma) return;
+    const bool dz = 4 * k + 3 < 2 * NZT ? true : 4 * k >= 2 * NZT ? false : wv + 4 * k < 2 * NZT;
     const long long tile = SPLIT ? ht >> 1 : ht;
-    const char* base = (k < 4 ? dzb + tile * zstride_b : acb + tile * astride_b) + (SPLIT ? 512 * (ht & 1) : 0);
-    dma_block_nt(base, lane_off[k], ldsw + slot * DWW_STAGE_BYTES + k * 4096);
-#endif
-  };
-  auto read_tile = [&](WOps& o, int r, unsigned so) {
-    if (r < 4) o.al[r] = trw((r < 2 ? rdA0 : rdA1) + so + (r & 1) * 1024 + 8192);
-    else if (r < 8) o.bh[r - 4] = trw(rdB + so + (r - 4) * 1024);
-    else if (r < 12) o.ah[r - 8] = trw((r - 8 < 2 ? rdA0 : rdA1) + so + (r & 1) * 1024);
-    else o.bl[r - 12] = trw(rdB + so + (r - 12) * 1024 + 8192);
-  };
-  auto mfma_m = [&](const WOps& o, int m) {
+    const char* base = (dz ? dzb + tile * zstride_b : acb + tile * astride_b) + (SPLIT ? 512 * (ht & 1) : 0);
+    dma_block_nt(base, lane_off[k], ldsw + slot * STAGE_BYTES + k * 4096);
+#endif
+  };
+  auto addr_a = [&](int i) { return i < 4 ? (i < 2 ? rdA0 : rdA1) + (i & 1) * 1024 : rdA4; };
+  auto addr_b = [&](int k) { return k < 4 ? (k < 2 ? rdB0 : rdB1) + (k & 1) * 1024 : rdB4; };
+  auto read_tile = [&](WOps<NI, NK>& o, int r, unsigned so) {
+    if (r < NI) o.al[r] = trw(addr_a(r) + so + NZT * 1024);
+    else if (r < NI + NK) o.bh[r - NI] = trw(addr_b(r - NI) + so);
+    else if (r < 2 * NI + NK) o.ah[r - NI - NK] = trw(addr_a(r - NI - NK) + so);
+    else o.bl[r - 2 * NI - NK] = trw(addr_b(r - 2 * NI - NK) + so + NHT * 1024);
+  };
+  auto mfma_m = [&](const WOps<NI, NK>& o, int m) {
 #if !(NERF_DWX & 16)
-    const int pt = m >> 4, i = (m >> 2) & 3, k = m & 3;
+    const int pt = m / NT, q = m % NT, i = NK == 5 ? q / 5 : q / 4, k = NK == 5 ? q % 5 : q % 4;
+    if (i >= 4 || k >= 4) {
+      const bf16x8& av = SPLIT ? (pt == 0 ? o.al[i] : o.ah[i]) : (pt == 0 ? o.ah[i] : o.al[i]);
+      const bf16x8& bv = SPLIT ? (pt == 1 ? o.bl[k] : o.bh[k]) : (pt == 0 ? o.bh[k] : o.bl[k]);
+      mfma32_v(av, bv, accx[NK == 5 ? i : k]);
+      return;
+    }
     if (SPLIT) {
       if (pt == 0) acc[i][k] = mfma32(o.al[i], o.bh[k], acc[i][k]);
       else if (pt == 1) acc[i][k] = mfma32(o.ah[i], o.bl[k], acc[i][k]);
@@ -102,37 +137,45 @@
     asm volatile("" :: "v"(o.al[m & 3]), "v"(o.ah[m & 3]), "v"(o.bh[m & 3]), "v"(o.bl[m & 3]));
 #endif
   };
-  auto dot_d = [&](const WOps& o, int d) {
+  auto dot_d = [&](const WOps<NI, NK>& o, int d) {
 #if !(NERF_DWX & 8)
-    const int t = d >> 3, part = (d >> 2) & 1, w = d & 3;
-    const bf16x8& v = part ? o.al[t] : o.ah[t];
+    const int t = d >> 3, part = (d >> 2) & 1, w = d & 3, i = t < 2 ? t : 4;
+    const bf16x8& v = part ? o.al[i] : o.ah[i];
     const bf16x2 ones = {(__bf16)1.0f, (__bf16)1.0f};
     const bf16x2 pr = {v[2 * w], v[2 * w + 1]};
     bsum[2 * t + part] = __builtin_amdgcn_fdot2_f32_bf16(pr, ones, bsum[2 * t + part], false);
 #endif
   };
-  constexpr int RD0[DWW_SLICES + 1] = {0, 0, 3, 6, 9, 12, 14, 16, 16};
-  constexpr int DM0[DWW_SLICES + 1] = {0, 0, 2, 3, 4, 5, 6, 7, 8};
-
-  auto step = [&](WOps& use, WOps& ld, int j, int slot, auto full_c) {
+  constexpr int M0T[DWW_SLICES + 1] = {0, MT / 8, MT * 2 / 8, MT * 3 / 8, MT * 4 / 8, MT * 5 / 8, MT * 6 / 8, MT * 7 / 8, MT};
+  constexpr int RD0[DWW_SLICES + 1] = {0, 0, 3, 6, 9, 12, NR == 16 ? 14 : 15, NR, NR};
+  constexpr int DM0[DWW_SLICES + 1] = {0, 0, 2, DPW == 8 ? 3 : 4, DPW - 4, DPW - 3, DPW - 2, DPW - 1, DPW};
+  static_assert((NR == 16 || NR == 18) && (DPW == 8 || DPW == 9), "the slice tables");
+  auto wait_younger = [&](auto yc) {
+    constexpr int Y = decltype(yc)::value;
+    if (Y == 0 || !UNEVEN || last_dma) asm volatile("s_waitcnt vmcnt(%0)" :: "n"(Y * DPW) : "memory");
+    else asm volatile("s_waitcnt vmcnt(%0)" :: "n"(Y * (DPW - 1)) : "memory");
+  };
+
+  auto step = [&](WOps<NI, NK>& use, WOps<NI, NK>& ld, int j, int slot, auto full_c) {
     constexpr bool FULL = decltype(full_c)::value;
     const bool more = FULL || j + 1 < n, iss = FULL || j + 4 < n;
     __builtin_amdgcn_s_waitcnt(0xC07F);
 #pragma unroll
-    for (int m = 0; m < MPS; ++m) mfma_m(use, m);
+    for (int m = 0; m < M0T[1]; ++m) mfma_m(use, m);
     dot_d(use, 0); dot_d(use, 1);
+    if (NBT == 3) dot_d(use, 16);
     __builtin_amdgcn_sched_barrier(0);
-    if (FULL) asm volatile("s_waitcnt vmcnt(16)" ::: "memory");
+    if (FULL) wait_younger(IntC<2>());
     else {
       const int younger = (n - 1 < j + 3 ? n - 1 : j + 3) - (j + 1);
-      if (younger >= 2) asm volatile("s_waitcnt vmcnt(16)" ::: "memory");
-      else if (younger == 1) asm volatile("s_waitcnt vmcnt(8)" ::: "memory");
-      else asm volatile("s_waitcnt vmcnt(0)" ::: "memory");
+      if (younger >= 2) wait_younger(IntC<2>());
+      else if (younger == 1) wait_younger(IntC<1>());
+      else wait_younger(IntC<0>());
     }
 #if !(NERF_DWX & 4)
     __builtin_amdgcn_s_barrier();
 #endif
-    const unsigned so = (unsigned)(((slot + 1) & 3) * DWW_STAGE_BYTES);
+    const unsigned so = (unsigned)(((slot + 1) & 3) * STAGE_BYTES);
 #pragma unroll
     for (int s = 1; s < DWW_SLICES; ++s) {
       if (iss) {
@@ -144,25 +187,26 @@
         for (int r = RD0[s]; r < RD0[s + 1]; ++r) read_tile(ld, r, so);
       }
 #pragma unroll
-      for (int m = MPS * s; m < MPS * (s + 1); ++m) mfma_m(use, m);
+      for (int m = M0T[s]; m < M0T[s + 1]; ++m) mfma_m(use, m);
       dot_d(use, 2 * s); dot_d(use, 2 * s + 1);
+      if (NBT == 3) dot_d(use, 16 + s);
       __builtin_amdgcn_sched_barrier(0);
     }
   };
 
-  WOps x, y;
+  WOps<NI, NK> x, y;
   if (n > 0) {
 #pragma unroll
     for (int s_ = 0; s_ < DWW_STAGES; ++s_)
       if (s_ < n) {
 #pragma unroll
-        for (int k = 0; k < DWW_DPW; ++k) issue_k(ht_lo + s_, s_, k);
+        for (int k = 0; k < DPW; ++k) issue_k(ht_lo + s_, s_, k);
       }
-    if (n >= 4) asm volatile("s_waitcnt vmcnt(24)" ::: "memory");
-    else asm volatile("s_waitcnt vmcnt(0)" ::: "memory");
+    if (n >= 4) wait_younger(IntC<3>());
+    else wait_younger(IntC<0>());
     __builtin_amdgcn_s_barrier();
 #pragma unroll
-    for (int r = 0; r < 16; ++r) read_tile(x, r, 0u);
+    for (int r = 0; r < NR; ++r) read_tile(x, r, 0u);
   }
   int j = 0;
   for (; j + 5 < n; j += 2) {
@@ -174,32 +218,51 @@
     if (j + 1 < n) step(y, x, j + 1, (j + 1) & 3, BoolC<false>());
   }
 
+  if (NX > 0) mfma_v_drain();
   const int rr = lane & 31, hh = lane >> 5;
-  float* slot = a.partial + (size_t)blockIdx.x * DW_SLOT_FLOATS;
-#pragma unroll
-  for (int i = 0; i < 4; ++i) {
-    const int nt = 4 * wr + ((i + rot) & 3);
-#pragma unroll
-    for (int k = 0; k < 4; ++k) {
-      float* tile = slot + (8 * nt + 4 * wc + k) * 1024;
-#pragma unroll
-      for (int e = 0; e < 16; ++e) tile[((e & 3) + 8 * (e >> 2) + 4 * hh) * 32 + rr] = acc[i][k][e];
-    }
+  float* slot = a.partial + (size_t)blockIdx.x * a.slot_floats;
+#pragma unroll
+  for (int q = 0; q < NT; ++q) {
+    const int i = NK == 5 ? q / 5 : q / 4, k = NK == 5 ? q % 5 : q % 4;
+    const int nt = i < 4 ? 4 * wr + ((i + rot) & 3) : 8, kt = k < 4 ? 4 * wc + ((k + rotb) & 3) : 8 + wc;
+    const f32x16& v = i < 4 && k < 4 ? acc[i][k] : accx[NK == 5 ? i : k];
+    float* tile = slot + (jb.kts * nt + kt) * 1024;
+#pragma unroll
+    for (int e = 0; e < 16; ++e) tile[((e & 3) + 8 * (e >> 2) + 4 * hh) * 32 + rr] = v[e];
   }
   if (jb.b_off >= 0) {
 #pragma unroll
-    for (int t = 0; t < 2; ++t) {
+    for (int t = 0; t < NBT; ++t) {
+      if (t >= 2 && wv != 0) continue;
       const float v = bsum[2 * t + 1] + bsum[2 * t];
       const float tot = v + __shfl_xor(v, 32, 64);
-      if (hh == 0) slot[64 * 1024 + 32 * (4 * wr + rot + t) + rr] = tot;
-    }
-  }
+      if (hh == 0) slot[a.bias_off + 32 * (t < 2 ? 4 * wr + rot + t : 8) + rr] = tot;
+    }
+  }
+}
+
+template <bool SPLIT>
+__global__ void __launch_bounds__(64 * DWW_WAVES) mlp_dww_kernel(DwArgs a) {
+  int bj = blockIdx.x, job_id = 0;
+  while (bj >= a.splits[job_id]) { bj -= a.splits[job_id]; ++job_id; }
+  const DwJob jb = dw_job_uniform(a, job_id);
+  auto uni = [](int v) { return __builtin_amdgcn_readfirstlane(v); };
+  const int nsplit = uni(a.splits[job_id]);
+  bj = uni(bj);
+  if (jb.kf2 != 0) dww_job<SPLIT, 4, 5>(a, jb, bj, nsplit);
+  else if (jb.nf > 16) dww_job<SPLIT, 5, 4>(a, jb, bj, nsplit);
+  else dww_job<SPLIT, 4, 4>(a, jb, bj, nsplit);
 }
 
 int launch_dw_wide_kernel(const DwArgs& d, int workgroups, bool split_bf16, hipStream_t s) {
+  int stage_kib = 32;
+  for (int j = 0; j < DW_MAX_JOBS && d.splits[j] > 0; ++j) {
+    const int kib = 2 * ((d.jobs[j].nf + 1) / 2) + 2 * ((d.jobs[j].kf + d.jobs[j].kf2 + 1) / 2);
+    if (kib > stage_kib) stage_kib = kib;
+  }
   return with_bool(split_bf16, [&](auto split) {
-    return launch<mlp_dww_kernel<decltype(split)::value>>(split_bf16 ? "mlp dW (split bf16, 256 x 256 jobs)" : "mlp dW (bf16, 256 x 256 jobs)",
-                                                          dim3(workgroups), dim3(64 * DWW_WAVES), DWW_LDS_BYTES, s, d);
+    return launch<mlp_dww_kernel<decltype(split)::value>>(split_bf16 ? "mlp dW (split bf16, wide jobs)" : "mlp dW (bf16, wide jobs)",
+                                                          dim3(workgroups), dim3(64 * DWW_WAVES), Lds(DWW_STAGES * stage_kib * 1024, DWW_LDS_MAX), s, d);
   });
 }
 
diff --git a/nerf_meets_mlx_amd/csrc/mlp_frag.h b/nerf_meets_mlx_amd/csrc/mlp_frag.h
--- a/nerf_meets_mlx_amd/csrc/mlp_frag.h
+++ b/nerf_meets_mlx_amd/csrc/mlp_frag.h
@@ -197,6 +197,8 @@
   int w_off, ldw, col0;
   int n_valid, k_valid;
   int b_off;
+  int act_slot2 = 0, kf2 = 0;
+  int kts = 8;
 };
 constexpr int DW_MAX_JOBS = 16;
 struct DwArgs {
@@ -211,10 +213,35 @@
   int ring_cap;
   int private_max_tiles;
   int a_lo, z_lo;
-};
+  int slot_floats, bias_off;
+};
+struct DwRedJob {
+  int first, splits;
+  int kts, nt0, kt0;
+  int w_off, ldw, col0, n_valid, k_valid, b_off;
+};
+struct DwRedArgs {
+  DwRedJob jobs[DW_MAX_JOBS];
+  const float* partial;
+  float* grads;
+  int slot_floats, bias_off;
+};
+__device__ __forceinline__ DwJob dw_job_uniform(const DwArgs& a, int j) {
+  const DwJob& s = a.jobs[j];
+  auto u = [](int v) { return __builtin_amdgcn_readfirstlane(v); };
+  DwJob r;
+  r.dz_slot = u(s.dz_slot); r.nf = u(s.nf); r.act_slot = u(s.act_slot); r.kf = u(s.kf);
+  r.w_off = u(s.w_off); r.ldw = u(s.ldw); r.col0 = u(s.col0); r.n_valid = u(s.n_valid); r.k_valid = u(s.k_valid); r.b_off = u(s.b_off);
+  r.act_slot2 = u(s.act_slot2); r.kf2 = u(s.kf2); r.kts = u(s.kts);
+  return r;
+}
+
 constexpr int DW_SLOT_FLOATS = 64 * 1024 + 256;
 constexpr int DW_MAX_WGS = 512;
 constexpr int64_t DW_PARTIAL_BYTES = (int64_t)DW_MAX_WGS * DW_SLOT_FLOATS * 4;
 int launch_dw_wide_kernel(const DwArgs& d, int workgroups, bool split_bf16, hipStream_t s);
-
-}
+constexpr int dww_shape(const DwJob& j) {
+  return j.kf != 16 ? 0 : j.nf == 16 ? (j.kf2 == 0 ? 1 : j.kf2 == 4 ? 2 : 0) : (j.nf == 17 && j.kf2 == 0) ? 3 : 0;
+}
+
+}
diff --git a/nerf_meets_mlx_amd/csrc/mlp_model.h b/nerf_meets_mlx_amd/csrc/mlp_model.h
--- a/nerf_meets_mlx_amd/csrc/mlp_model.h
+++ b/nerf_meets_mlx_amd/csrc/mlp_model.h
@@ -39,6 +39,21 @@
     img_pos(6), img_pos(7),
     {LI::Z_OUT, 1, LI::A_H0 + 112, 16, LI::P_WO, 256, 0, 0, 256, 0},
 };
+constexpr DwJob VIEW_MJOBS[] = {
+    VIEW_JOBS[0], view_pos(1), view_pos(2), view_pos(3), view_pos(4),
+    {L::Z_L0 + 80, 16, L::A_H0 + 64, 16, L::P_W5, 319, 63, 256, 256, L::P_B5, L::A_PE, 4},
+    view_pos(6), view_pos(7),
+    {L::Z_F, 17, L::A_H0 + 112, 16, L::P_WF, 256, 0, 256, 256, L::P_BF},
+    {L::Z_D, 8, L::A_FEAT, 16, L::P_WD, 283, 0, 128, 256, L::P_BD, L::A_DPE, 2},
+    VIEW_JOBS[13],
+};
+static_assert(L::Z_A == L::Z_F + 16 && L::Z_A + 1 < L::Z_SLOTS, "feature + alpha: 17 adjacent dZ fragments, the 18th inside the tile's store");
+static_assert(VIEW_MJOBS[9].kf2 == 2 && VIEW_MJOBS[9].nf <= 8, "dir0 merged: the 2 x 8 wave grid of s16_dw_kernel covers at most 4 n-tiles");
+constexpr DwJob IMG_MJOBS[] = {
+    IMG_JOBS[0], img_pos(1), img_pos(2), img_pos(3), img_pos(4),
+    {LI::Z_L0 + 80, 16, LI::A_H0 + 64, 16, LI::P_W5, 296, 40, 256, 256, LI::P_B5, LI::A_X, 4},
+    img_pos(6), img_pos(7), IMG_JOBS[9],
+};
 constexpr DwJob SMALL_JOBS[] = {
     {LN::Z_L0, 4, LN::A_X, 2, LN::P_W0, 32, 0, 64, 32, LN::P_B0},
     {LN::Z_L1, 4, LN::A_H0, 4, LN::P_W1, 64, 0, 64, 64, LN::P_B1},
@@ -57,19 +72,23 @@
   int a_slots[2], z_slots[2];
   int a_lo, z_lo;
   const DwJob* jobs; int njobs;
+  const DwJob* mjobs; int nmjobs;
   DebugSlot debug[2][12];
 };
 constexpr ShapeInfo SHAPES[3] = {
     {L::P_TOTAL, L::F_TOTAL, L::B_PADDED, L::BI_TOTAL, L::F16_PADDED, s16::PACKED_BYTES,
      {L::A_SLOTS, s16::A_SLOTS}, {L::Z_SLOTS, s16::Z_SLOTS}, s16::A_LO, s16::Z_LO, VIEW_JOBS, sizeof(VIEW_JOBS) / sizeof(DwJob),
+     VIEW_MJOBS, sizeof(VIEW_MJOBS) / sizeof(DwJob),
      {{NERF_HIDDEN8(L::A_H0), {L::A_FEAT, 16}, {L::A_HD, 8}, {L::A_PE, 4}, {L::A_DPE, 2}},
       {NERF_HIDDEN8(L::Z_L0), {L::Z_F, 16}, {L::Z_D, 8}, {L::Z_A, 1}, {L::Z_RGB, 1}}}},
     {LI::P_WO, LI::F_TOTAL, LI::B_PADDED, LI::BI_TOTAL, 0, s16x::IMG_PACKED_BYTES,
      {LI::A_SLOTS, s16x::IMG_A_SLOTS}, {LI::Z_SLOTS, s16x::IMG_Z_SLOTS}, s16x::IMG_A_LO, s16x::IMG_Z_LO, IMG_JOBS, sizeof(IMG_JOBS) / sizeof(DwJob),
+     IMG_MJOBS, sizeof(IMG_MJOBS) / sizeof(DwJob),
      {{NERF_HIDDEN8(LI::A_H0), {0, 0}, {0, 0}, {LI::A_X, 3}, {0, 0}},
       {NERF_HIDDEN8(LI::Z_L0), {LI::Z_OUT, 1}, {0, 0}, {0, 0}, {0, 0}}}},
     {LN::P_TOTAL, LN::F_PADDED, LN::B_PADDED, LN::BI_TOTAL, 0, s16x::SM_PACKED_BYTES,
      {LN::A_SLOTS, s16x::SM_A_SLOTS}, {LN::Z_SLOTS, s16x::SM_Z_SLOTS}, s16x::SM_A_LO, s16x::SM_Z_LO, SMALL_JOBS, sizeof(SMALL_JOBS) / sizeof(DwJob),
+     nullptr, 0,
      {{{LN::A_H0, 4}, {LN::A_H1, 4}, {0, 0}, {0, 0}, {0, 0}, {0, 0}, {0, 0}, {0, 0}, {LN::A_FEAT, 4}, {LN::A_HD, 2}, {LN::A_X, 2}, {LN::A_DX, 1}},
       {{LN::Z_L0, 4}, {LN::Z_L1, 4}, {0, 0}, {0, 0}, {0, 0}, {0, 0}, {0, 0}, {0, 0}, {LN::Z_F, 4}, {LN::Z_D, 2}, {LN::Z_A, 1}, {LN::Z_RGB, 1}}}},
 };
@@ -105,10 +124,27 @@
     }
     return nj;
   }
+  int dw_merged_jobs(DwJob* dst) const {
+    for (int j = 0; j < info->nmjobs; ++j) {
+      dst[j] = info->mjobs[j];
+      if (shape == Shape::Image && j == info->nmjobs - 1) { dst[j].n_valid = out_ch; dst[j].b_off = LI::P_WO + out_ch * 256; }
+    }
+    return info->nmjobs;
+  }
   DebugSlot debug_slot(int kind, int layer) const {
     return (layer < 0 || layer > 11 || (kind != 0 && kind != 1)) ? DebugSlot{0, 0} : info->debug[kind][layer];
   }
 };
+
+inline int dw_locate(const DwJob& l, const DwJob* c, int nc, int* nt0, int* kt0) {
+  for (int j = 0; j < nc; ++j) {
+    const int dn = l.dz_slot - c[j].dz_slot, d1 = l.act_slot - c[j].act_slot, d2 = l.act_slot - c[j].act_slot2;
+    if (dn < 0 || (dn & 1) || dn + l.nf > c[j].nf) continue;
+    if (d1 >= 0 && !(d1 & 1) && d1 + l.kf <= c[j].kf) { *nt0 = dn / 2; *kt0 = d1 / 2; return j; }
+    if (c[j].kf2 > 0 && d2 >= 0 && !(d2 & 1) && d2 + l.kf <= c[j].kf2) { *nt0 = dn / 2; *kt0 = (c[j].kf + 1) / 2 + d2 / 2; return j; }
+  }
+  return -1;
+}
 
 inline Model resolve(const nerf_mlp_arch* a) {
   Model m{};
diff --git a/nerf_meets_mlx_amd/csrc/mlp_s16.hip b/nerf_meets_mlx_amd/csrc/mlp_s16.hip
--- a/nerf_meets_mlx_amd/csrc/mlp_s16.hip
+++ b/nerf_meets_mlx_amd/csrc/mlp_s16.hip
@@ -413,18 +413,18 @@
   }
   if (wv != 0) return;
   const int rr = lane & 31, hh = lane >> 5;
-  float* slot = a.partial + (size_t)blockIdx.x * DW_SLOT_FLOATS;
+  float* slot = a.partial + (size_t)blockIdx.x * a.slot_floats;
 #pragma unroll
   for (int i = 0; i < NT; ++i) {
 #pragma unroll
     for (int k = 0; k < KT; ++k) {
-      float* tile = slot + (8 * i + k) * 1024;
+      float* tile = slot + (jb.kts * i + k) * 1024;
 #pragma unroll
       for (int e = 0; e < 16; ++e) tile[((e & 3) + 8 * (e >> 2) + 4 * hh) * 32 + rr] = acc[i][k][e];
     }
     if (jb.b_off >= 0) {
       const float tot = bsum[i] + __shfl_xor(bsum[i], 32, 64);
-      if (hh == 0) slot[64 * 1024 + 32 * i + rr] = tot;
+      if (hh == 0) slot[a.bias_off + 32 * i + rr] = tot;
     }
   }
 }
@@ -434,14 +434,15 @@
   char* smem = ring_smem;
   int bj = blockIdx.x, job_id = 0;
   while (bj >= a.splits[job_id]) { bj -= a.splits[job_id]; ++job_id; }
-  const DwJob jb = a.jobs[job_id];
+  const DwJob jb = dw_job_uniform(a, job_id);
   const int tile_lo = (int)((int64_t)a.ntiles * bj / a.splits[job_id]);
   const int tile_hi = (int)((int64_t)a.ntiles * (bj + 1) / a.splits[job_id]);
   const int tid = threadIdx.x, lane = tid & 63;
   const int wv = __builtin_amdgcn_readfirstlane(tid >> 6);
-  const int n_tiles = (jb.nf + 1) >> 1, k_tiles = (jb.kf + 1) >> 1;
+  const int k1_tiles = (jb.kf + 1) >> 1, n_tiles = (jb.nf + 1) >> 1, k_tiles = k1_tiles + ((jb.kf2 + 1) >> 1);
   const bool col_major = k_tiles <= 2;
-  const int wr = col_major ? (wv & 3) : (wv >> 2), wc = col_major ? (wv >> 2) : (wv & 3);
+  const bool grid_2x8 = k_tiles > 8;
+  const int wr = col_major ? (wv & 3) : grid_2x8 ? (wv >> 3) : (wv >> 2), wc = col_major ? (wv >> 2) : grid_2x8 ? (wv & 7) : (wv & 3);
   const int npairs = 2 * (n_tiles + k_tiles);
   if (a.private_max_tiles >= n_tiles * k_tiles && npairs * 1024 <= DWP_WAVE_BYTES) {
     switch (8 * n_tiles + k_tiles) {
@@ -478,9 +479,9 @@
   const char* dzb = reinterpret_cast<const char*>(a.dz);
   const char* acb = reinterpret_cast<const char*>(a.acts);
   long long zstride_b = a.zstride * 16, astride_b = a.astride * 16;
-  int z_lo = a.z_lo, a_lo = a.a_lo, dz_slot = jb.dz_slot, act_slot = jb.act_slot, nf = jb.nf, kf = jb.kf;
+  int z_lo = a.z_lo, a_lo = a.a_lo, dz_slot = jb.dz_slot, act_slot = jb.act_slot, nf = jb.nf, kf = jb.kf, act_slot2 = jb.act_slot2, kf2 = jb.kf2;
   asm volatile("" : "+s"(zstride_b), "+s"(astride_b), "+s"(z_lo), "+s"(a_lo), "+s"(dz_slot), "+s"(act_slot), "+s"(nf), "+s"(kf),
-               "+s"(stride), "+s"(ns));
+               "+s"(stride), "+s"(ns), "+s"(act_slot2), "+s"(kf2));
 
   auto issue = [&](int ht, int slot) {
 #if NERF_DWX & 1
@@ -497,10 +498,12 @@
         const int j = is_z ? i : i - 2 * n_tiles;
         const int nt_ = is_z ? n_tiles : k_tiles;
         const int lo_part = j >= nt_ ? 1 : 0;
-        const int t = lo_part ? j - nt_ : j;
-        const int nfr = is_z ? nf : kf;
+        const int t_ = lo_part ? j - nt_ : j;
+        const int second = is_z ? 0 : (int)((unsigned)(k1_tiles - 1 - t_) >> 31);
+        const int t = t_ - second * k1_tiles;
+        const int nfr = is_z ? nf : kf + second * (kf2 - kf);
         int fr = 2 * t + src_sel; if (fr >= nfr) fr = nfr - 1;
-        const int slot_ = (is_z ? dz_slot + (SPLIT ? lo_part * z_lo : 0) : act_slot + (SPLIT ? lo_part * a_lo : 0)) + fr;
+        const int slot_ = (is_z ? dz_slot + (SPLIT ? lo_part * z_lo : 0) : act_slot + second * (act_slot2 - act_slot) + (SPLIT ? lo_part * a_lo : 0)) + fr;
         const unsigned row_off = row_off0 + (SPLIT ? 0 : 512 * lo_part);
         const char* src = (is_z ? dzb + tile * zstride_b : acb + tile * astride_b) + (int64_t)slot_ * 1024 + row_off;
         dma_frag_nt(src, st + i * 1024);
@@ -583,7 +586,7 @@
   __builtin_amdgcn_s_barrier();
   if (!active) return;
   const int rr = lane & 31, hh = lane >> 5;
-  float* slot = a.partial + (size_t)blockIdx.x * DW_SLOT_FLOATS;
+  float* slot = a.partial + (size_t)blockIdx.x * a.slot_floats;
 #pragma unroll
   for (int i = 0; i < DW_NPW; ++i) {
     const int nt = wr * DW_NPW + i;
@@ -592,7 +595,7 @@
     for (int k = 0; k < 2; ++k) {
       const int kt = wc * 2 + k;
       if (kt >= k_tiles) continue;
-      float* tile = slot + (8 * nt + kt) * 1024;
+      float* tile = slot + (jb.kts * nt + kt) * 1024;
 #pragma unroll
       for (int e = 0; e < 16; ++e) tile[((e & 3) + 8 * (e >> 2) + 4 * hh) * 32 + rr] = acc[i][k][e];
     }
@@ -600,7 +603,7 @@
       const float lo = xb[(wr * 2 * DW_NPW + 2 * i + 1) * 64 + lane], hi = xb[(wr * 2 * DW_NPW + 2 * i) * 64 + lane];
       const float t = lo + hi;
       const float tot = t + __shfl_xor(t, 32, 64);
-      if (hh == 0) slot[64 * 1024 + 32 * nt + rr] = tot;
+      if (hh == 0) slot[a.bias_off + 32 * nt + rr] = tot;
     }
   }
 }
```

After: 1.219 million, median of 6. Within noise of the previous version (+0.8%).
